# geometrian/simple-spectral

Hardware: AMD Instinct MI355X
Metric: Msamples/s (w*h*spp/s) cornell-srgb 512x512 (higher is better)
Workload: dtype f32

## Files before the change

include/ssx.h:

```cpp
#ifndef SSX_H
#define SSX_H

#include <stddef.h>
#include <stdint.h>

#ifdef __cplusplus
extern "C" {
#endif

#define SSX_ABI_VERSION 2

enum {
	SSX_OK = 0,
	SSX_ERR_DATA = -1,
	SSX_ERR_ARG = -2,
	SSX_ERR_SCENE = -3,
	SSX_ERR_DEVICE = -10,
	SSX_ERR_STATE = -11
};

#define SSX_MAX_DEPTH 10u
#define SSX_TILE_SIZE 8u
#define SSX_SAMPLE_WAVELENGTHS 4u
#define SSX_MAX_TEXTURES 64u
// ... 43 lines not shown
} ssx_meng_grid;

typedef struct ssx_scene_desc {
	uint32_t struct_size;
	uint32_t reserved;
	double pv_inv[16];
	float cam_pos[3];
	float lambda_min;
	float lambda_step;
	uint32_t spec_xbar, spec_ybar, spec_zbar;
	uint32_t spec_basis_r, spec_basis_g, spec_basis_b;
	const ssx_spectrum* spectra;  uint32_t n_spectra;
	const float* samples;         uint32_t n_samples;
	const ssx_material* materials; uint32_t n_materials;
	const ssx_quad* quads;        uint32_t n_quads;
	const uint32_t* lights;       uint32_t n_lights;
	const ssx_texture* textures;  uint32_t n_textures;
	float srgb_to_linear[256];
	uint32_t uplift;
	uint32_t jh_res;
	const float* jh_scale;
	const float* jh_data;
	const ssx_meng_grid* meng;
	float cam_dir[3];
	uint32_t reserved2;
} ssx_scene_desc;

typedef struct ssx_render_params {
	uint32_t struct_size;
	uint32_t width, height;
	uint32_t spp;
	uint32_t indirect_only;
	uint32_t tile_first;
	uint32_t tile_stride;
	uint32_t spp_per_launch;
	uint32_t no_explicit_light_sampling;
	uint32_t no_flat_field_correction;
	uint32_t tile_major;
	uint32_t tile_skew;
	uint64_t seed;
	uint32_t libm;
	uint32_t reserved3;
} ssx_render_params;
enum { SSX_LIBM_BUILD = 0, SSX_LIBM_GLIBC_2_35 = 1 };


typedef struct ssx_ctx ssx_ctx;

int ssx_create(int device, ssx_ctx** out);
void ssx_destroy(ssx_ctx* ctx);

int ssx_upload_scene(ssx_ctx* ctx, const ssx_scene_desc* scene);

int ssx_render_start(ssx_ctx* ctx, const ssx_render_params* params);
int ssx_render_stop(ssx_ctx* ctx);
int ssx_is_rendering(ssx_ctx* ctx);
float ssx_progress(ssx_ctx* ctx);
uint32_t ssx_done_spp(ssx_ctx* ctx);
uint32_t ssx_done_tiles(ssx_ctx* ctx);
int ssx_render_wait(ssx_ctx* ctx, float* xyza_out);

int ssx_render_device(ssx_ctx* ctx, const ssx_render_params* params, void* d_xyza_out, void* hip_stream);
int ssx_render_device_wait(ssx_ctx* ctx);

void* ssx_device_framebuffer(ssx_ctx* ctx);
int ssx_device_index(ssx_ctx* ctx);
int ssx_read_framebuffer(ssx_ctx* ctx, float* xyza_out);
int ssx_accumulate_peer(ssx_ctx* ctx, void* d_dst, int src_device, const void* d_src, uint32_t width, uint32_t height, void* hip_stream);

int ssx_reduce_rccl(ssx_ctx** ctxs, int n, uint32_t width, uint32_t height);
int ssx_rccl_probe(char* report, size_t report_size);
uint64_t ssx_rccl_groups_made(void);

const char* ssx_last_error(const ssx_ctx* ctx);

int ssx_set_timing(ssx_ctx* ctx, int enable);
int ssx_get_timing(ssx_ctx* ctx, float stage_ms[4]);

int ssx_abi_version(void);
int ssx_kernel_info(ssx_ctx* ctx, int* vgprs, int* sgprs, int* lds_bytes, int* scratch_bytes, int* max_blocks_per_cu);
int ssx_plan_info(ssx_ctx* ctx, float* frames_per_sample, int* fold_in_path_kernel);
int ssx_calibration_info(ssx_ctx* ctx, float* frames_per_sample, float* rays_left_per_sample, int* camera_rays_pretraced);
int ssx_scratch_info(ssx_ctx* ctx, uint64_t* sample_bytes, uint64_t* log_bytes);
int ssx_sums_info(ssx_ctx* ctx, uint64_t* units_parked, uint64_t* units_chained);
int ssx_units_info(ssx_ctx* ctx, uint64_t* units_enqueued);
int ssx_kernel_variant(ssx_ctx* ctx);
enum { SSX_JIT_OFF = 0, SSX_JIT_AT_UPLOAD = 1, SSX_JIT_BACKGROUND = 2 };
int ssx_set_jit(ssx_ctx* ctx, int mode);
enum { SSX_JIT_STATE_NONE = 0,
       SSX_JIT_STATE_GENERIC_MEANWHILE = 1,
       SSX_JIT_STATE_SPECIALISED = 2,
       SSX_JIT_STATE_FAILED = -1 };
int ssx_jit_status(ssx_ctx* ctx, int wait_ms, char* message, size_t message_size);
void ssx_jit_counters(uint64_t* compiled, uint64_t* disk_hits);
const char* ssx_kernel_name(ssx_ctx* ctx);


int ssx_render_continue(ssx_ctx* ctx, uint32_t spp_more);

typedef struct ssx_sums_info_t {
	uint32_t struct_size;
	uint32_t width, height;
	uint32_t done_spp;
	uint64_t seed;
	uint32_t indirect_only, no_explicit_light_sampling, no_flat_field_correction, libm;
	uint32_t rgb_mode;
	uint32_t tile_first, tile_stride, tile_skew;
	uint32_t noise_batches;
	uint32_t reserved;
	uint64_t scene_digest;
} ssx_sums_info_t;
uint64_t ssx_scene_digest(ssx_ctx* ctx);
int ssx_sums_export(ssx_ctx* ctx, ssx_sums_info_t* info, double* sums, double* noise_s2);
int ssx_sums_import(ssx_ctx* ctx, const ssx_render_params* params, const ssx_sums_info_t* info, const double* sums, const double* noise_s2);

int ssx_set_noise_estimate(ssx_ctx* ctx, int enable);
int ssx_noise_info(ssx_ctx* ctx, double* v_out, double summary[4]);


int ssx_set_spectral_bins(ssx_ctx* ctx, uint32_t bins);
typedef struct ssx_spectral_info_t {
	uint32_t struct_size;
	uint32_t width, height;
	uint32_t bins;
	uint32_t done_spp;
	uint32_t reserved;
	float lambda_min;
	float bin_width;
} ssx_spectral_info_t;
int ssx_spectral_read(ssx_ctx* ctx, ssx_spectral_info_t* info, float* mean, double* sums, uint32_t* counts);

enum {
	SSX_DBG_FMATH = 1,
	SSX_DBG_SPHTRI = 2,
	SSX_DBG_ARVO = 3,
	SSX_DBG_SAMPLE_LIGHT = 4,
	SSX_DBG_COSHEMI = 5,
	SSX_DBG_TRACE = 6,
	SSX_DBG_RAND_CHOICE = 7,
	SSX_DBG_ALBEDO = 8,
	SSX_DBG_FLUX_TO_XYZ = 9,
	SSX_DBG_RAND_1F = 10,
	SSX_DBG_GLIBC_MATH = 11,
	SSX_DBG_SPHTRI_GLIBC = 12, SSX_DBG_ARVO_GLIBC = 13, SSX_DBG_SAMPLE_LIGHT_GLIBC = 14, SSX_DBG_COSHEMI_GLIBC = 15
};
enum {
	SSX_SWEEP_RCP = 1,
	SSX_SWEEP_SQRT = 2,
	SSX_SWEEP_INVERSESQRT = 3,
	SSX_SWEEP_SIN = 4,
	SSX_SWEEP_COS = 5,
	SSX_SWEEP_ACOS = 6,
	SSX_SWEEP_DIV_PI = 7,
	SSX_SWEEP_RCP64 = 8,
	SSX_SWEEP_DIV_PAIRS = 9,
	SSX_SWEEP_ACOS_SIN = 10,
	SSX_SWEEP_SIN_PROOF = 11, SSX_SWEEP_COS_PROOF = 12, SSX_SWEEP_ACOS_PROOF = 13,
	SSX_SWEEP_GLIBC_SIN = 14, SSX_SWEEP_GLIBC_COS = 15, SSX_SWEEP_GLIBC_ACOS = 16,
	SSX_SWEEP_GLIBC_COS_LDS = 17
};
int ssx_debug_sweep(ssx_ctx* ctx, uint32_t op, uint32_t lo, uint64_t count, uint64_t result[11]);
int ssx_debug_pass1_source(const uint8_t* vid, uint32_t n_quads, const char* name, char* out, size_t out_size);
int ssx_debug_eval(ssx_ctx* ctx, uint32_t op, const void* in, uint32_t in_words, void* out, uint32_t out_words, uint32_t n);
int ssx_debug_samples(ssx_ctx* ctx, const ssx_render_params* params, float* xyza, uint64_t* rng_state, uint32_t* levels);
int ssx_debug_sample_flux(ssx_ctx* ctx, const ssx_render_params* params, float* flux, float* lambda_0);

// ... 5 lines not shown
```

simple_spectral_amd/_capi.py:

```python
import ctypes as C
import os

from . import build as _build


class SsxSpectrum(C.Structure):
    _fields_ = [("offset", C.c_uint32), ("n", C.c_uint32), ("low", C.c_float), ("high", C.c_float),
                ("delta_recip", C.c_float)]


class SsxVertex(C.Structure):
    _fields_ = [("pos", C.c_float * 3), ("st", C.c_float * 2)]


class SsxQuad(C.Structure):
    _fields_ = [("v00", SsxVertex), ("v10", SsxVertex), ("v11", SsxVertex), ("v01", SsxVertex),
                ("normal0", C.c_float * 3), ("normal1", C.c_float * 3),
                ("material", C.c_uint32), ("flags", C.c_uint32)]


class SsxMaterial(C.Structure):
    _fields_ = [("kind", C.c_uint32), ("albedo_mode", C.c_uint32), ("albedo_spectrum", C.c_uint32),
                ("albedo_texture", C.c_uint32), ("emission_spectrum", C.c_uint32)]


class SsxTexture(C.Structure):
    _fields_ = [("width", C.c_uint32), ("height", C.c_uint32), ("rgb", C.POINTER(C.c_uint8))]


class SsxMengGrid(C.Structure):
    _fields_ = [("grid_w", C.c_uint32), ("grid_h", C.c_uint32), ("n_points", C.c_uint32), ("n_samples", C.c_uint32),
                ("sample_min", C.c_float), ("sample_max", C.c_float), ("xy_to_uv", C.c_float * 6),
                ("cells", C.POINTER(C.c_int32)), ("points", C.POINTER(C.c_float))]


class SsxSceneDesc(C.Structure):
    _fields_ = [
        ("struct_size", C.c_uint32), ("reserved", C.c_uint32),
        ("pv_inv", C.c_double * 16), ("cam_pos", C.c_float * 3),
        ("lambda_min", C.c_float), ("lambda_step", C.c_float),
        ("spec_xbar", C.c_uint32), ("spec_ybar", C.c_uint32), ("spec_zbar", C.c_uint32),
        ("spec_basis_r", C.c_uint32), ("spec_basis_g", C.c_uint32), ("spec_basis_b", C.c_uint32),
        ("spectra", C.POINTER(SsxSpectrum)), ("n_spectra", C.c_uint32),
        ("samples", C.POINTER(C.c_float)), ("n_samples", C.c_uint32),
        ("materials", C.POINTER(SsxMaterial)), ("n_materials", C.c_uint32),
        ("quads", C.POINTER(SsxQuad)), ("n_quads", C.c_uint32),
        ("lights", C.POINTER(C.c_uint32)), ("n_lights", C.c_uint32),
        ("textures", C.POINTER(SsxTexture)), ("n_textures", C.c_uint32),
        ("srgb_to_linear", C.c_float * 256),
        ("uplift", C.c_uint32), ("jh_res", C.c_uint32),
        ("jh_scale", C.POINTER(C.c_float)), ("jh_data", C.POINTER(C.c_float)),
        ("meng", C.POINTER(SsxMengGrid)),
        ("cam_dir", C.c_float * 3), ("reserved2", C.c_uint32),
    ]


class SsxRenderParams(C.Structure):
    _fields_ = [("struct_size", C.c_uint32), ("width", C.c_uint32), ("height", C.c_uint32), ("spp", C.c_uint32),
                ("indirect_only", C.c_uint32), ("tile_first", C.c_uint32), ("tile_stride", C.c_uint32),
                ("spp_per_launch", C.c_uint32), ("no_explicit_light_sampling", C.c_uint32), ("no_flat_field_correction", C.c_uint32),
                ("tile_major", C.c_uint32), ("tile_skew", C.c_uint32), ("seed", C.c_uint64), ("libm", C.c_uint32), ("reserved3", C.c_uint32)]


class SsxSumsInfo(C.Structure):
    _fields_ = [("struct_size", C.c_uint32), ("width", C.c_uint32), ("height", C.c_uint32), ("done_spp", C.c_uint32), ("seed", C.c_uint64),
                ("indirect_only", C.c_uint32), ("no_explicit_light_sampling", C.c_uint32), ("no_flat_field_correction", C.c_uint32), ("libm", C.c_uint32),
                ("rgb_mode", C.c_uint32), ("tile_first", C.c_uint32), ("tile_stride", C.c_uint32), ("tile_skew", C.c_uint32),
                ("noise_batches", C.c_uint32), ("reserved", C.c_uint32), ("scene_digest", C.c_uint64)]


class SsxSpectralInfo(C.Structure):
    _fields_ = [("struct_size", C.c_uint32), ("width", C.c_uint32), ("height", C.c_uint32), ("bins", C.c_uint32), ("done_spp", C.c_uint32),
                ("reserved", C.c_uint32), ("lambda_min", C.c_float), ("bin_width", C.c_float)]


SSX_LIBM_BUILD, SSX_LIBM_GLIBC_2_35 = 0, 1
LIBM_MODES = {"build": SSX_LIBM_BUILD, "glibc-2.35": SSX_LIBM_GLIBC_2_35}


SSX_MODE_RGB, SSX_UPLIFT_OURS, SSX_UPLIFT_MENG, SSX_UPLIFT_JH = 0, 1, 2, 3
SSX_PRIM_LIGHT, SSX_PRIM_TRI = 1, 0x100
SSX_OK, SSX_ERR_DATA, SSX_ERR_ARG, SSX_ERR_SCENE, SSX_ERR_DEVICE, SSX_ERR_STATE = 0, -1, -2, -3, -10, -11
SSX_ABI_VERSION = 2
SSX_JIT_OFF, SSX_JIT_AT_UPLOAD, SSX_JIT_BACKGROUND = 0, 1, 2
SSX_JIT_STATE_NONE, SSX_JIT_STATE_GENERIC_MEANWHILE, SSX_JIT_STATE_SPECIALISED, SSX_JIT_STATE_FAILED = 0, 1, 2, -1

HIP_SYMBOLS = ["ssx_create", "ssx_destroy", "ssx_upload_scene", "ssx_render_start", "ssx_render_stop",
               "ssx_is_rendering", "ssx_progress", "ssx_render_wait", "ssx_render_device", "ssx_last_error",
               "ssx_abi_version", "ssx_kernel_info", "ssx_plan_info", "ssx_set_timing", "ssx_get_timing",
               "ssx_device_framebuffer", "ssx_device_index", "ssx_read_framebuffer", "ssx_accumulate_peer",
               "ssx_debug_eval", "ssx_debug_samples", "ssx_debug_sweep", "ssx_kernel_variant", "ssx_kernel_name", "ssx_scratch_info", "ssx_calibration_info", "ssx_set_jit", "ssx_debug_pass1_source", "ssx_done_spp", "ssx_reduce_rccl", "ssx_sums_info", "ssx_rccl_groups_made", "ssx_jit_status", "ssx_jit_counters", "ssx_done_tiles", "ssx_render_device_wait", "ssx_units_info", "ssx_rccl_probe",
               "ssx_render_continue", "ssx_scene_digest", "ssx_sums_export", "ssx_sums_import", "ssx_set_noise_estimate", "ssx_noise_info",
               "ssx_set_spectral_bins", "ssx_spectral_read", "ssx_debug_sample_flux"]
(SSX_SWEEP_RCP, SSX_SWEEP_SQRT, SSX_SWEEP_INVERSESQRT, SSX_SWEEP_SIN, SSX_SWEEP_COS, SSX_SWEEP_ACOS, SSX_SWEEP_DIV_PI,
 SSX_SWEEP_RCP64, SSX_SWEEP_DIV_PAIRS, SSX_SWEEP_ACOS_SIN, SSX_SWEEP_SIN_PROOF, SSX_SWEEP_COS_PROOF, SSX_SWEEP_ACOS_PROOF) = range(1, 14)
(SSX_DBG_FMATH, SSX_DBG_SPHTRI, SSX_DBG_ARVO, SSX_DBG_SAMPLE_LIGHT, SSX_DBG_COSHEMI, SSX_DBG_TRACE, SSX_DBG_RAND_CHOICE,
 SSX_DBG_ALBEDO, SSX_DBG_FLUX_TO_XYZ, SSX_DBG_RAND_1F) = range(1, 11)
(SSX_DBG_GLIBC_MATH, SSX_DBG_SPHTRI_GLIBC, SSX_DBG_ARVO_GLIBC, SSX_DBG_SAMPLE_LIGHT_GLIBC, SSX_DBG_COSHEMI_GLIBC) = range(11, 16)
(SSX_SWEEP_GLIBC_SIN, SSX_SWEEP_GLIBC_COS, SSX_SWEEP_GLIBC_ACOS, SSX_SWEEP_GLIBC_COS_LDS) = range(14, 18)
HOST_SYMBOLS = ["ssh_scene_create", "ssh_scene_create_ex", "ssh_scene_destroy", "ssh_scene_desc", "ssh_xyza_to_srgba", "ssh_save_image",
                "ssh_load_png_rgb8", "ssh_free", "ssh_color_values", "ssh_last_error", "ssh_checkpoint_save", "ssh_checkpoint_load", "ssh_sums_merge", "ssh_save_npy_f32"]

_hip = None
_host = None


def host_lib():
    global _host
    if _host is None:
        path = _build.HOST_LIB
        if not os.path.exists(path):
            _build.build_host()
        lib = C.CDLL(path)
        vp = C.c_void_p
        lib.ssh_last_error.restype = C.c_char_p
        lib.ssh_scene_create.argtypes = [C.c_char_p, C.c_char_p, C.c_int, vp, C.c_uint32, C.c_uint32, C.c_char_p,
                                         C.c_float, C.POINTER(vp)]
        lib.ssh_scene_create_ex.argtypes = [C.c_char_p, C.c_char_p, C.c_int, vp, C.c_uint32, C.c_uint32, C.c_char_p,
                                            C.c_float, C.c_uint32, C.c_char_p, C.c_uint32, C.POINTER(vp)]
        lib.ssh_scene_destroy.argtypes = [vp]
        lib.ssh_scene_desc.restype = C.POINTER(SsxSceneDesc)
        lib.ssh_scene_desc.argtypes = [vp]
        lib.ssh_xyza_to_srgba.argtypes = [vp, vp, vp, C.c_size_t]
        lib.ssh_save_image.argtypes = [C.c_char_p, vp, C.c_uint32, C.c_uint32]
        lib.ssh_load_png_rgb8.argtypes = [C.c_char_p, C.POINTER(C.POINTER(C.c_uint8)), C.POINTER(C.c_uint32),
                                          C.POINTER(C.c_uint32)]
        lib.ssh_free.argtypes = [vp]
        lib.ssh_color_values.argtypes = [vp, C.c_char_p, C.POINTER(C.c_float), C.c_int]
        lib.ssh_checkpoint_save.argtypes = [C.c_char_p, C.POINTER(SsxSumsInfo), C.c_char_p, C.c_char_p, vp, vp]
        lib.ssh_checkpoint_load.argtypes = [C.c_char_p, C.POINTER(SsxSumsInfo), C.c_char_p, C.c_size_t, C.c_char_p, C.c_size_t,
                                            C.POINTER(C.POINTER(C.c_double)), C.POINTER(C.POINTER(C.c_double))]
        lib.ssh_sums_merge.argtypes = [vp, vp, vp, vp, C.POINTER(SsxSumsInfo)]
        lib.ssh_save_npy_f32.argtypes = [C.c_char_p, vp, C.POINTER(C.c_uint32), C.c_uint32]
        _host = lib
    return _host


def mapped_hip_runtimes():
    out = set()
    try:
        for ln in open("/proc/self/maps"):
            f = ln.split(None, 5)
            if len(f) == 6 and "libamdhip64.so" in os.path.basename(f[5].strip()):
                out.add(os.path.realpath(f[5].strip()))
    except OSError:
        pass
    return sorted(out)


def _elf_dynamic(path):
    import struct
    try:
        with open(path, "rb") as f:
            eh = f.read(64)
            if eh[:6] != b"\x7fELF\x02\x01":
                return None, []
            shoff, = struct.unpack_from("<Q", eh, 0x28)
            shentsize, shnum = struct.unpack_from("<HH", eh, 0x3A)
            f.seek(shoff)
            sh = [struct.unpack_from("<IIQQQQIIQQ", f.read(shentsize)) for _ in range(shnum)]
            dyn = next((x for x in sh if x[1] == 6), None)
            if dyn is None:
                return None, []
            strtab = sh[dyn[6]]
            f.seek(strtab[4]); names = f.read(strtab[5])
            f.seek(dyn[4]); raw = f.read(dyn[5])
        soname, needed = None, []
        for k in range(0, len(raw) - 15, 16):
            tag, val = struct.unpack_from("<qQ", raw, k)
            if tag in (1, 14):
                name = names[val:names.index(b"\0", val)].decode()
                if tag == 14:
                    soname = name
                else:
                    needed.append(name)
        return soname, needed
    except Exception:
        return None, []


def _one_hip_runtime_before_load(path):
    if mapped_hip_runtimes():
        return
    try:
        import importlib.util
        wanted = [n for n in _elf_dynamic(path)[1] if n.startswith("libamdhip64.so")]
        spec = importlib.util.find_spec("torch")
        if wanted and spec and spec.submodule_search_locations:
            cand = os.path.join(list(spec.submodule_search_locations)[0], "lib", "libamdhip64.so")
            if os.path.exists(cand) and _elf_dynamic(cand)[0] == wanted[0]:
                C.CDLL(cand, mode=C.RTLD_GLOBAL)
    except Exception:
        pass


def _one_hip_runtime_after_load(path):
    rts = mapped_hip_runtimes()
    if len(rts) > 1:
        raise RuntimeError("two HIP runtimes are mapped into this process (%s) after loading %s: streams and device pointers cannot be "
                           "handed between them.  Import simple_spectral_amd (or torch) before whatever loaded the other one, or "
                           "point LD_LIBRARY_PATH at one of them." % (", ".join(rts), path))


def hip_lib():
    global _hip
    if _hip is None:
        path = (os.environ.get("SSX_HIP_LIB_OVERRIDE") if os.environ.get("SSX_DEBUG_ENV") == "1" else None) or _build.HIP_LIB
        if not os.path.exists(path):
            raise RuntimeError("%s is missing: run `python -m simple_spectral_amd.build` (needs hipcc). "
                               "simple_spectral_amd has no CPU or PyTorch fallback path." % path)
        _one_hip_runtime_before_load(path)
        lib = C.CDLL(path)
        _one_hip_runtime_after_load(path)
        override = path != _build.HIP_LIB
        if not override and lib.ssx_abi_version() != SSX_ABI_VERSION:
            raise RuntimeError("%s implements ABI version %d, this binding version %d (include/ssx.h): rebuild with `python -m simple_spectral_amd.build`"
                               % (path, lib.ssx_abi_version(), SSX_ABI_VERSION))
        vp = C.c_void_p
        lib.ssx_last_error.restype = C.c_char_p
        lib.ssx_last_error.argtypes = [vp]
        lib.ssx_create.argtypes = [C.c_int, C.POINTER(vp)]
        lib.ssx_destroy.argtypes = [vp]
        lib.ssx_destroy.restype = None
        lib.ssx_upload_scene.argtypes = [vp, C.POINTER(SsxSceneDesc)]
        lib.ssx_render_start.argtypes = [vp, C.POINTER(SsxRenderParams)]
        lib.ssx_render_stop.argtypes = [vp]
        lib.ssx_is_rendering.argtypes = [vp]
        lib.ssx_progress.argtypes = [vp]
        lib.ssx_progress.restype = C.c_float
        lib.ssx_render_wait.argtypes = [vp, vp]
        lib.ssx_render_device.argtypes = [vp, C.POINTER(SsxRenderParams), vp, vp]
        lib.ssx_kernel_info.argtypes = [vp] + [C.POINTER(C.c_int)] * 5
        lib.ssx_plan_info.argtypes = [vp, C.POINTER(C.c_float), C.POINTER(C.c_int)]
        lib.ssx_set_timing.argtypes = [vp, C.c_int]
        lib.ssx_get_timing.argtypes = [vp, C.POINTER(C.c_float)]
        lib.ssx_device_framebuffer.argtypes = [vp]
        lib.ssx_device_framebuffer.restype = vp
        lib.ssx_device_index.argtypes = [vp]
        lib.ssx_read_framebuffer.argtypes = [vp, vp]
        lib.ssx_accumulate_peer.argtypes = [vp, vp, C.c_int, vp, C.c_uint32, C.c_uint32, vp]
        lib.ssx_debug_eval.argtypes = [vp, C.c_uint32, vp, C.c_uint32, vp, C.c_uint32, C.c_uint32]
        lib.ssx_debug_samples.argtypes = [vp, C.POINTER(SsxRenderParams), vp, vp, vp]
        lib.ssx_debug_sweep.argtypes = [vp, C.c_uint32, C.c_uint32, C.c_uint64, C.POINTER(C.c_uint64)]
        if not override or hasattr(lib, "ssx_scratch_info"):
            lib.ssx_calibration_info.argtypes = [vp, C.POINTER(C.c_float), C.POINTER(C.c_float), C.POINTER(C.c_int)]
            lib.ssx_scratch_info.argtypes = [vp, C.POINTER(C.c_uint64), C.POINTER(C.c_uint64)]
        if not override or hasattr(lib, "ssx_set_jit"):
            lib.ssx_set_jit.argtypes = [vp, C.c_int]
            lib.ssx_done_spp.argtypes = [vp]
            lib.ssx_done_spp.restype = C.c_uint32
            lib.ssx_reduce_rccl.argtypes = [C.POINTER(vp), C.c_int, C.c_uint32, C.c_uint32]
            lib.ssx_debug_pass1_source.argtypes = [C.POINTER(C.c_uint8), C.c_uint32, C.c_char_p, C.c_char_p, C.c_size_t]
        if not override or hasattr(lib, "ssx_sums_info"):
            lib.ssx_sums_info.argtypes = [vp, C.POINTER(C.c_uint64), C.POINTER(C.c_uint64)]
        if hasattr(lib, "ssx_rccl_probe"):
            lib.ssx_rccl_probe.argtypes = [C.c_char_p, C.c_size_t]
        if hasattr(lib, "ssx_units_info"):
            lib.ssx_units_info.argtypes = [vp, C.POINTER(C.c_uint64)]
        if not override or hasattr(lib, "ssx_jit_status"):
            lib.ssx_jit_status.argtypes = [vp, C.c_int, C.c_char_p, C.c_size_t]
            lib.ssx_jit_counters.argtypes = [C.POINTER(C.c_uint64), C.POINTER(C.c_uint64)]
            lib.ssx_jit_counters.restype = None
            lib.ssx_rccl_groups_made.restype = C.c_uint64
            lib.ssx_render_device_wait.argtypes = [vp]
            lib.ssx_done_tiles.argtypes = [vp]
            lib.ssx_done_tiles.restype = C.c_uint32
        if not override or hasattr(lib, "ssx_render_continue"):
            lib.ssx_render_continue.argtypes = [vp, C.c_uint32]
            lib.ssx_scene_digest.argtypes = [vp]
            lib.ssx_scene_digest.restype = C.c_uint64
            lib.ssx_sums_export.argtypes = [vp, C.POINTER(SsxSumsInfo), vp, vp]
            lib.ssx_sums_import.argtypes = [vp, C.POINTER(SsxRenderParams), C.POINTER(SsxSumsInfo), vp, vp]
            lib.ssx_set_noise_estimate.argtypes = [vp, C.c_int]
            lib.ssx_noise_info.argtypes = [vp, vp, C.POINTER(C.c_double)]
        if not override or hasattr(lib, "ssx_set_spectral_bins"):
            lib.ssx_set_spectral_bins.argtypes = [vp, C.c_uint32]
            lib.ssx_spectral_read.argtypes = [vp, C.POINTER(SsxSpectralInfo), vp, vp, vp]
            lib.ssx_debug_sample_flux.argtypes = [vp, C.POINTER(SsxRenderParams), vp, vp]
        lib.ssx_kernel_variant.argtypes = [vp]
        lib.ssx_kernel_name.argtypes = [vp]
        lib.ssx_kernel_name.restype = C.c_char_p
        _hip = lib
    return _hip
```

simple_spectral_amd/csrc/ssx_api.hip:

```cpp
#include "ssx_kernels.hip"
#include "ssx_debug.hip"

#include "../../include/ssx.h"

#include <chrono>
#include <array>
#include <atomic>
#include <cstdarg>
#include <cstdio>
#include <cstdlib>
#include <cmath>
#include <algorithm>
#include <cstring>
#include <mutex>
#include <string>
#include <thread>
#include <vector>

#include <limits.h>
#include <set>

#include "ssx_jit.h"

namespace {

thread_local std::string g_create_error;

const char* debug_env(const char* name) {
	const char* m = getenv("SSX_DEBUG_ENV");
	if (!m || m[0] != '1' || m[1] != '\0') return nullptr;
	return getenv(name);
}
bool env_on(const char* name) { const char* e = debug_env(name); return e && e[0] != '\0' && e[0] != '0'; }

std::string fmt(const char* f, ...) {
	char buf[512];
	va_list ap; va_start(ap, f); vsnprintf(buf, sizeof buf, f, ap); va_end(ap);
	return buf;
}

struct DeviceBuffer {
	void* ptr = nullptr;
	size_t bytes = 0;
	DeviceBuffer() = default;
	DeviceBuffer(DeviceBuffer&& o) noexcept : ptr(o.ptr), bytes(o.bytes) { o.ptr = nullptr; o.bytes = 0; }
	DeviceBuffer& operator=(DeviceBuffer&& o) noexcept { std::swap(ptr, o.ptr); std::swap(bytes, o.bytes); return *this; }
	~DeviceBuffer() { release(); }
	void release() { if (ptr) (void)hipFree(ptr); ptr = nullptr; bytes = 0; }
	hipError_t reserve(size_t n) {
		if (n <= bytes) return hipSuccess;
		release();
		const hipError_t e = hipMalloc(&ptr, n);
		if (e == hipSuccess) bytes = n; else ptr = nullptr;
		return e;
	}
	template <class T> T* as() const { return static_cast<T*>(ptr); }
};

}

#include "ssx_pack.h"

struct ssx_ctx {
	int device = 0;
	int n_cus = 0;
	hipStream_t stream = nullptr;
	DeviceBuffer d_blob;
	uint32_t blob_words = 0;
	uint32_t path_blob_words = 0;
	uint32_t topology = 0;
	int jit_mode = SSX_JIT_BACKGROUND;
	const ssx_jit::Kernels* jit_kernels[ssx_jit::kVariants] = {};
	uint32_t libm = SSX_LIBM_BUILD;
	uint32_t variant = SSX_LIBM_BUILD;
	bool jit_pending = false, jit_requested = false;
	ssx_jit::VidTable jit_vid;
	DeviceBuffer d_blob_jit; uint32_t blob_jit_words = 0, path_blob_jit_words = 0;
	uint64_t generic_samples = 0;
	int jit_state = SSX_JIT_STATE_NONE; std::string jit_message;
	std::vector<DeviceBuffer> d_textures;
	DeviceBuffer d_jh_data;
	bool rgb_mode = false;
	bool fuse_resolve = true;
	float calib_frames = 0.0f;
	float calib_left = 0.0f;
	bool pre_hits = false;
	DeviceBuffer d_accum;
	DeviceBuffer d_unit_counter;
	int resident_blocks = 0;
	int gen_blocks = 0;
	uint32_t max_wave_slots = 0;
	uint32_t queue_words = SSX_QUEUE_WORDS_WIDE;
	DeviceBuffer d_samples;
	DeviceBuffer d_logs;
	DeviceBuffer d_out;
	DeviceBuffer d_peer;
	bool have_scene = false;
	bool have_cam_dir = false;

	std::thread worker;
	std::atomic<int> rendering{0};
	std::atomic<int> stop_flag{0};
	std::atomic<uint32_t> done_spp{0};
	std::atomic<uint32_t> done_tiles{0};
	uint32_t total_spp = 0;
	int worker_rc = 0;
	std::atomic<uint64_t> units_enqueued{0};
	ssx_render_params cur{};
	struct SumsState { bool continuable = false, noise_valid = false, spectral_valid = false; uint32_t noise_batches = 0; } sums;
	uint32_t k_begin = 0;
	uint64_t scene_digest = 0;
	bool noise_on = false;
	DeviceBuffer d_noise;
	DeviceBuffer d_stage;
	uint32_t spectral_bins = 0;
	DeviceBuffer d_spectral_sums, d_spectral_counts;
	std::string spectral_note;
	float lambda_min = 0.0f, lambda_step = 0.0f;

	bool timing = false;
	std::vector<hipEvent_t> ev_pool;
	size_t ev_used = 0;
	float stage_ms[4] = { 0, 0, 0, 0 };

	hipEvent_t ev_device_done = nullptr;
	bool device_pending = false;

	void* rccl_comm = nullptr; uint64_t rccl_group = 0; int rccl_rank = -1, rccl_size = 0;

	std::mutex error_mutex;
	std::string error;
	std::string error_out;
};

namespace {

void set_error(ssx_ctx* ctx, const std::string& msg) { std::lock_guard<std::mutex> g(ctx->error_mutex); ctx->error = msg; }

#define SSX_HIP(ctx, call)                                                                          \
	do {                                                                                            \
		hipError_t e_ = (call);                                                                     \
		if (e_ != hipSuccess) {                                                                     \
			set_error((ctx), fmt("%s failed: %s", #call, hipGetErrorString(e_)));                   \
			return SSX_ERR_DEVICE;                                                                  \
		}                                                                                           \
	} while (0)

int fail(ssx_ctx* ctx, int code, const std::string& msg) { set_error(ctx, msg); return code; }

int check_params(ssx_ctx* ctx, const ssx_render_params* p) {
	if (!p || p->struct_size != sizeof(ssx_render_params)) return fail(ctx, SSX_ERR_ARG, "ssx_render_params.struct_size mismatch");
	if (p->libm != SSX_LIBM_BUILD && p->libm != SSX_LIBM_GLIBC_2_35) return fail(ctx, SSX_ERR_ARG, "ssx_render_params.libm: unknown value");
	if (!ctx->have_scene) return fail(ctx, SSX_ERR_STATE, "no scene uploaded");
	if (p->width == 0 || p->height == 0 || p->spp == 0) return fail(ctx, SSX_ERR_ARG, "width, height and spp must be positive");
	if ((uint64_t)p->width * p->height > (1ull << 28)) return fail(ctx, SSX_ERR_ARG, "image too large");
	if (p->tile_stride == 0 || p->tile_first >= p->tile_stride) return fail(ctx, SSX_ERR_ARG, "need tile_first < tile_stride");
	if (p->no_flat_field_correction && !ctx->have_cam_dir) return fail(ctx, SSX_ERR_ARG, "no_flat_field_correction needs ssx_scene_desc.cam_dir (caller built against an older ssx.h)");
	return SSX_OK;
}

int take_params(ssx_ctx* ctx, const ssx_render_params* in, ssx_render_params* out) {
	if (!in) return fail(ctx, SSX_ERR_ARG, "ssx_render_params is NULL");
	memset(out, 0, sizeof *out);
	if (in->struct_size == offsetof(ssx_render_params, libm)) { memcpy(out, in, offsetof(ssx_render_params, libm)); out->struct_size = sizeof *out; }
	else memcpy(out, in, in->struct_size == sizeof *out ? sizeof *out : sizeof out->struct_size);
	return check_params(ctx, out);
}
int begin_render(ssx_ctx* ctx, const ssx_render_params* in, ssx_render_params* out, const char* busy) {
	const int rc = take_params(ctx, in, out);
	if (rc) return rc;
	return ctx->rendering.load() ? fail(ctx, SSX_ERR_STATE, busy) : SSX_OK;
}

int wait_device_pending(ssx_ctx* ctx) {
	if (ctx->device_pending) { SSX_HIP(ctx, hipEventSynchronize(ctx->ev_device_done)); ctx->device_pending = false; }
	return SSX_OK;
}

uint32_t tiles_across(uint32_t pixels) { return (pixels + 7u) / 8u; }
size_t accum_bytes(uint32_t width, uint32_t height) { return (size_t)tiles_across(width) * tiles_across(height) * 64u * 4 * sizeof(double); }
size_t image_bytes(uint32_t width, uint32_t height) { return (size_t)width * height * 4 * sizeof(float); }

SsxPixelGrid pixel_grid(const ssx_render_params* p) {
	const uint32_t tx = tiles_across(p->width);
	return SsxPixelGrid{ p->width, p->height, tx, p->tile_first, p->tile_stride, p->tile_skew % tx };
}
dim3 pixel_blocks(const ssx_render_params* p) { return dim3((p->width * p->height + 255u) / 256u); }

int clear_sums(ssx_ctx* ctx, uint32_t width, uint32_t height, hipStream_t stream) {
	SSX_HIP(ctx, hipMemsetAsync(ctx->d_accum.ptr, 0, accum_bytes(width, height), stream));
	return SSX_OK;
}
void sums_invalidate(ssx_ctx* ctx) { ctx->sums = ssx_ctx::SumsState{}; }
void sums_publish(ssx_ctx* ctx, uint32_t done_spp, int64_t noise_batches = -1) {
	if (noise_batches >= 0) { ctx->sums.noise_valid = true; ctx->sums.noise_batches = (uint32_t)noise_batches; }
	ctx->done_spp.store(done_spp); ctx->sums.continuable = true;
}

constexpr size_t kSampleBufferBudget = (size_t)16 << 30;
size_t bytes_per_sample(const ssx_ctx* ctx) { return ctx->spectral_bins ? SSX_BYTES_PER_SAMPLE_FLUX : SSX_BYTES_PER_SAMPLE; }
constexpr size_t kAuxWordsPer64Records = 5;
size_t bytes_per_64_records(const ssx_ctx* ctx) { return 64u * bytes_per_sample(ctx) + kAuxWordsPer64Records * sizeof(uint32_t); }
size_t sample_bytes(const ssx_ctx* ctx, size_t records) { return records / 64u * bytes_per_64_records(ctx); }
size_t sample_slots(const ssx_ctx* ctx) { return ctx->d_samples.bytes / bytes_per_64_records(ctx) * 64u; }
size_t log_records(const ssx_ctx* ctx) { return ctx->d_logs.bytes / SSX_LOG_BYTES_PER_RECORD; }
constexpr uint32_t kMinUnits = 3072;
constexpr uint64_t kSamplesPerSync = (uint64_t)32 << 20;

struct LaunchPlan { SsxKernelArgs args; uint32_t max_spp_per_launch; };

LaunchPlan make_plan(ssx_ctx* ctx, const ssx_render_params* p, bool ask_device = true) {
	LaunchPlan pl{};
	SsxKernelArgs& a = pl.args;
	a.blob = ctx->d_blob.as<uint32_t>(); a.blob_words = ctx->path_blob_words;
	a.width = p->width; a.height = p->height;
	a.inv_width = 1.0 / (double)p->width; a.inv_height = 1.0 / (double)p->height;
	a.tiles_x = tiles_across(p->width);
	a.n_tiles = a.tiles_x * tiles_across(p->height);
	a.tile_first = p->tile_first; a.tile_stride = p->tile_stride; a.tile_skew = p->tile_skew % a.tiles_x;
	a.indirect_only = p->indirect_only ? 1u : 0u;
	a.no_els = p->no_explicit_light_sampling ? 1u : 0u;
	a.no_flat_field = p->no_flat_field_correction ? 1u : 0u;
	a.seed = p->seed;
	a.rgb_mode = ctx->rgb_mode ? 1u : 0u;
	a.fuse_resolve = ctx->fuse_resolve ? 1u : 0u;
	a.pre_hits = ctx->pre_hits ? 1u : 0u;
	a.my_tiles = a.n_tiles > p->tile_first ? (a.n_tiles - p->tile_first + p->tile_stride - 1u) / p->tile_stride : 0u;
	size_t per_spp = (size_t)(a.my_tiles ? a.my_tiles : 1u) * 64u * bytes_per_sample(ctx);
	size_t budget = kSampleBufferBudget, free_b = 0, total_b = 0;
	if (ask_device && hipMemGetInfo(&free_b, &total_b) == hipSuccess) {
		const size_t avail = (size_t)((double)(free_b + sample_slots(ctx) * bytes_per_sample(ctx)) * 0.8);
		if (avail < budget) budget = avail;
	}
	size_t cap = budget / per_spp;
	const size_t idx_cap = (size_t)0xFFFFFFFFu / ((size_t)(a.my_tiles ? a.my_tiles : 1u) * 64u);
	if (cap > idx_cap) cap = idx_cap;
	pl.max_spp_per_launch = (uint32_t)(cap < 1 ? 1 : (cap > 65536 ? 65536 : cap));
	return pl;
}

void cap_to_allocation(const ssx_ctx* ctx, LaunchPlan& pl) {
	const size_t per_spp = (size_t)(pl.args.my_tiles ? pl.args.my_tiles : 1u) * 64u;
	const size_t fit = sample_slots(ctx) / per_spp;
	if (fit >= 1 && fit < pl.max_spp_per_launch) pl.max_spp_per_launch = (uint32_t)fit;
}

int ensure_samples(ssx_ctx* ctx, const LaunchPlan& pl, uint32_t n_k) {
	const size_t need = (size_t)pl.args.my_tiles * 64u * n_k;
	const hipError_t e = ctx->d_samples.reserve(sample_bytes(ctx, need));
	if (e == hipErrorOutOfMemory) { (void)hipGetLastError(); return fail(ctx, SSX_ERR_DEVICE, fmt("out of device memory for %zu samples in flight; lower spp_per_launch", need)); }
	SSX_HIP(ctx, e);
	return SSX_OK;
}

int ensure_logs(ssx_ctx* ctx, uint32_t unit_cohorts) {
	const size_t need = (size_t)ctx->max_wave_slots * 2u * unit_cohorts * SSX_COHORT_RECORDS, bytes = need * SSX_LOG_BYTES_PER_RECORD;
	if (bytes >= ((size_t)1 << 32)) return fail(ctx, SSX_ERR_DEVICE, "level logs beyond 4 GiB: the kernels address them with 32-bit offsets");
	if (ctx->d_logs.bytes >= bytes) return SSX_OK;
	if (ctx->d_logs.ptr) {
		const int rc = wait_device_pending(ctx);
		if (rc) return rc;
		SSX_HIP(ctx, hipStreamSynchronize(ctx->stream));
	}
	const hipError_t e = ctx->d_logs.reserve(bytes);
	if (e == hipErrorOutOfMemory) { (void)hipGetLastError(); return fail(ctx, SSX_ERR_DEVICE, fmt("out of device memory for the level logs (%zu bytes)", bytes)); }
	SSX_HIP(ctx, e);
	return SSX_OK;
}

void bind_arrays(SsxKernelArgs& a, uint8_t* base, uint64_t cap, uint8_t* logs, uint64_t log_cap, bool with_flux) {
	a.ray = reinterpret_cast<float4*>(base);                      base += cap * 16u;
	a.st = reinterpret_cast<uint4*>(base);                        base += cap * 16u;
	a.hit = reinterpret_cast<float4*>(base);                      base += cap * 16u;
	a.flux = with_flux ? reinterpret_cast<float4*>(base) : nullptr;
	a.logs = logs; a.log_cap = (uint32_t)log_cap;
}

int collect_timing(ssx_ctx* ctx) {
	for (size_t b = 0; b + 6 <= ctx->ev_used; b += 6) {
		hipEvent_t* e = &ctx->ev_pool[b];
		SSX_HIP(ctx, hipEventSynchronize(e[2]));
		SSX_HIP(ctx, hipEventSynchronize(e[5]));
		const int pairs[4][2] = { { 0, 1 }, { 1, 2 }, { 3, 4 }, { 4, 5 } };
		for (int k = 0; k < 4; ++k) {
			float ms = 0;
			SSX_HIP(ctx, hipEventElapsedTime(&ms, e[pairs[k][0]], e[pairs[k][1]]));
			ctx->stage_ms[k] += ms;
		}
	}
	ctx->ev_used = 0;
	return SSX_OK;
}

int timing_events(ssx_ctx* ctx, hipEvent_t** out) {
	if (ctx->ev_used + 6 > 6 * 64) { int r = collect_timing(ctx); if (r) return r; }
	while (ctx->ev_pool.size() < ctx->ev_used + 6) {
		hipEvent_t e;
		SSX_HIP(ctx, hipEventCreateWithFlags(&e, hipEventDisableSystemFence));
		ctx->ev_pool.push_back(e);
	}
	*out = &ctx->ev_pool[ctx->ev_used];
	ctx->ev_used += 6;
	return SSX_OK;
}

struct Batch { SsxKernelArgs a; uint32_t units; uint64_t n_rec; hipEvent_t* tev; int rc; };

uint32_t unit_spp_of(const ssx_ctx* ctx) { return ctx->calib_frames >= 2.0f ? SSX_MAX_UNIT_KS / 2u : SSX_MAX_UNIT_KS; }

Batch make_batch(ssx_ctx* ctx, const LaunchPlan& pl, uint32_t k0, uint32_t k1) {
	Batch b{};
	b.a = pl.args;
	SsxKernelArgs& a = b.a;
	const uint32_t n_k = k1 - k0;
	a.k0 = k0; a.k1 = k1;
	a.n_records = (uint64_t)a.my_tiles * n_k * 64u;
	uint32_t g = unit_spp_of(ctx);
	while (g > 1u && (uint64_t)((n_k + g - 1u) / g) * a.my_tiles < kMinUnits) g >>= 1;
	a.group_spp = g;
	if (a.group_spp > n_k) a.group_spp = n_k;
	a.unit_cohorts = (a.group_spp + SSX_COHORT_KS - 1u) / SSX_COHORT_KS;
	a.unit_grab = ctx->calib_frames >= 2.0f ? 1u : 4u;
	if (a.unit_grab < 1u || a.unit_grab > 32u || a.group_spp == 0u || a.unit_cohorts == 0u) {
		b.rc = fail(ctx, SSX_ERR_STATE, fmt("internal: launch with unit_grab = %u (1..32), group_spp = %u, unit_cohorts = %u", a.unit_grab, a.group_spp, a.unit_cohorts));
		return b;
	}
	a.n_groups = (n_k + a.group_spp - 1) / a.group_spp;
	b.units = a.my_tiles * a.n_groups;
	b.n_rec = a.n_records;
	b.rc = ensure_logs(ctx, a.unit_cohorts);
	if (b.rc == SSX_OK) bind_arrays(a, ctx->d_samples.as<uint8_t>(), a.n_records, ctx->d_logs.as<uint8_t>(), log_records(ctx), ctx->spectral_bins != 0u);
	a.accum = ctx->d_accum.as<double>();
	uint32_t* const aux = reinterpret_cast<uint32_t*>(ctx->d_samples.as<uint8_t>() + sample_slots(ctx) * bytes_per_sample(ctx));
	a.unit_state = aux;
	a.tile_mask = aux + b.units;
	if (b.rc == SSX_OK && (size_t)a.my_tiles * 4u + b.units > (sample_slots(ctx) / 64u) * kAuxWordsPer64Records) b.rc = fail(ctx, SSX_ERR_STATE, "internal: launch larger than the sample allocation");
	return b;
}

size_t path_lds_bytes(uint32_t blob_words, uint32_t queue_words) {
	size_t n = ((size_t)blob_words + SSX_LDS_PREFIX_WORDS) * 4 + 4u * ((size_t)SSX_QUEUE_ENTRIES * queue_words + SSX_WAVE_COUNTER_WORDS) * 4u;
#ifdef SSX_REGTIME
	n += 4u * SSX_NTIME * 8u;
#endif
	return n;
}
struct PathKernel { const char* name; void (*host)(SsxKernelArgs); };
#define SSX_PK(k) { #k, k }
static const PathKernel kPathKernels[ssx_jit::kVariants][3][2] = {
	{ { SSX_PK(ssx_render_kernel), SSX_PK(ssx_render_kernel_nq) }, { SSX_PK(ssx_render_kernel_cornell), SSX_PK(ssx_render_kernel_cornell_nq) },
	  { SSX_PK(ssx_render_kernel_plane), SSX_PK(ssx_render_kernel_plane_nq) } },
	{ { SSX_PK(ssx_render_kernel_glibc), SSX_PK(ssx_render_kernel_nq_glibc) }, { SSX_PK(ssx_render_kernel_cornell_glibc), SSX_PK(ssx_render_kernel_cornell_nq_glibc) },
	  { SSX_PK(ssx_render_kernel_plane_glibc), SSX_PK(ssx_render_kernel_plane_nq_glibc) } },
	{ { SSX_PK(ssx_render_kernel_flux), SSX_PK(ssx_render_kernel_nq_flux) }, { SSX_PK(ssx_render_kernel_cornell_flux), SSX_PK(ssx_render_kernel_cornell_nq_flux) },
	  { SSX_PK(ssx_render_kernel_plane_flux), SSX_PK(ssx_render_kernel_plane_nq_flux) } } };
#undef SSX_PK
static const char* const kJitKernelNames[2] = { "ssx_render_kernel_jit", "ssx_render_kernel_jit_nq" };
const PathKernel& path_kernel_of(const ssx_ctx* ctx, bool narrow) { return kPathKernels[ctx->variant][ctx->topology < 3u ? ctx->topology : 0u][narrow]; }
struct KernelRef { const void* host = nullptr; hipFunction_t mod = nullptr; };
KernelRef path_kernel_ref(const ssx_ctx* ctx, bool narrow) {
	KernelRef k;
	const ssx_jit::Kernels* jk = ctx->jit_kernels[ctx->variant];
	if (ctx->topology == 3u && jk) k.mod = narrow ? jk->path_nq : jk->path;
	else k.host = (const void*)path_kernel_of(ctx, narrow).host;
	return k;
}
int occupancy_of(ssx_ctx* ctx, const KernelRef& k, size_t lds, int* per_cu) {
	if (k.mod) SSX_HIP(ctx, hipModuleOccupancyMaxActiveBlocksPerMultiprocessor(per_cu, k.mod, 256, lds));
	else SSX_HIP(ctx, hipOccupancyMaxActiveBlocksPerMultiprocessor(per_cu, k.host, 256, lds));
	return SSX_OK;
}
int blocks_that_fit(ssx_ctx* ctx, const KernelRef& k, size_t lds, int* blocks) {
	int per_cu = 0;
	const int rc = occupancy_of(ctx, k, lds, &per_cu);
	if (rc) return rc;
	*blocks = (per_cu > 0 ? per_cu : 1) * ctx->n_cus;
	return SSX_OK;
}
int launch_kernel(ssx_ctx* ctx, const KernelRef& k, uint32_t blocks, size_t lds, hipStream_t stream, SsxKernelArgs& a) {
	if (k.mod) {
		size_t size = sizeof a;
		void* config[] = { HIP_LAUNCH_PARAM_BUFFER_POINTER, &a, HIP_LAUNCH_PARAM_BUFFER_SIZE, &size, HIP_LAUNCH_PARAM_END };
		SSX_HIP(ctx, hipModuleLaunchKernel(k.mod, blocks, 1, 1, 256, 1, 1, (unsigned)lds, stream, nullptr, config));
	} else {
		void* args[] = { &a };
		SSX_HIP(ctx, hipLaunchKernel(k.host, dim3(blocks), dim3(256), args, lds, stream));
	}
	return SSX_OK;
}
int pick_queue(ssx_ctx* ctx, uint32_t blob_words, uint32_t* queue_words, int* blocks_per_cu) {
	int wide = 0, narrow = 0, rc;
	if (path_lds_bytes(blob_words, SSX_QUEUE_WORDS_WIDE) <= 65536u)
		if ((rc = occupancy_of(ctx, path_kernel_ref(ctx, false), path_lds_bytes(blob_words, SSX_QUEUE_WORDS_WIDE), &wide))) return rc;
	if ((rc = occupancy_of(ctx, path_kernel_ref(ctx, true), path_lds_bytes(blob_words, SSX_QUEUE_WORDS_NARROW), &narrow))) return rc;
	const bool use_narrow = narrow > wide || env_on("SSX_NARROW_QUEUE");
	*queue_words = use_narrow ? SSX_QUEUE_WORDS_NARROW : SSX_QUEUE_WORDS_WIDE;
	if (blocks_per_cu) *blocks_per_cu = use_narrow ? narrow : wide;
	return SSX_OK;
}

bool fuses_generate(const ssx_ctx* ctx, const SsxKernelArgs& a) {
	const char* fuse_env = debug_env("SSX_FUSE_GEN");
	const bool tiles_fit = a.tiles_x <= 0xFFFFu && tiles_across(a.height) <= 0xFFFFu;
	return ctx->topology == 2u && !a.pre_hits && tiles_fit && !(fuse_env && fuse_env[0] == '0');
}

int enqueue_generate(ssx_ctx* ctx, const Batch& b, hipStream_t stream) {
	SsxKernelArgs ga = b.a;
	ga.blob_words = ctx->blob_words;
	if (ga.pre_hits) {
		hipLaunchKernelGGL(ssx_tile_mask_kernel, dim3((ga.my_tiles + 3u) / 4u), dim3(256), 0, stream, ga);
		SSX_HIP(ctx, hipGetLastError());
	}
	const KernelRef gen_kernel{ (const void*)ssx_generate_kernel };
	const size_t gen_lds = ((size_t)ga.blob_words + SSX_LDS_PREFIX_WORDS) * 4;
	if (ctx->gen_blocks == 0) { const int rc = blocks_that_fit(ctx, gen_kernel, gen_lds, &ctx->gen_blocks); if (rc) return rc; }
	const uint64_t want = (b.n_rec + 255u) / 256u;
	return launch_kernel(ctx, gen_kernel, (uint32_t)(want < (uint64_t)ctx->gen_blocks ? want : (uint64_t)ctx->gen_blocks), gen_lds, stream, ga);
}

int enqueue_path(ssx_ctx* ctx, Batch& b, const KernelRef& kernel, uint32_t queue_words, uint32_t blob_words, int resident_blocks, hipStream_t stream) {
	if (!ctx->d_unit_counter.ptr) {
		SSX_HIP(ctx, ctx->d_unit_counter.reserve(4 * sizeof(uint32_t)));
		SSX_HIP(ctx, hipMemsetAsync(ctx->d_unit_counter.ptr, 0, 4 * sizeof(uint32_t), stream));
	}
	b.a.blob_words = blob_words; b.a.queue_words = queue_words;
	SSX_HIP(ctx, hipMemsetAsync(ctx->d_unit_counter.ptr, 0, 2 * sizeof(uint32_t), stream));
	SSX_HIP(ctx, hipMemsetAsync(b.a.unit_state, 0, (size_t)b.units * sizeof(uint32_t), stream));
	b.a.unit_counter = ctx->d_unit_counter.as<uint32_t>();
	const uint32_t want_blocks = (b.units + 3u) / 4u;
	uint32_t blocks = want_blocks < (uint32_t)resident_blocks ? want_blocks : (uint32_t)resident_blocks;
	if (blocks * 4u > ctx->max_wave_slots) blocks = ctx->max_wave_slots / 4u;
	return launch_kernel(ctx, kernel, blocks, path_lds_bytes(blob_words, queue_words), stream, b.a);
}

int launch_batch(ssx_ctx* ctx, Batch& b, hipStream_t stream) {
	if (b.rc) return b.rc;
	int rc;
	if (ctx->timing) { if ((rc = timing_events(ctx, &b.tev))) return rc; SSX_HIP(ctx, hipEventRecord(b.tev[0], stream)); }
	b.a.fuse_gen = fuses_generate(ctx, b.a) ? 1u : 0u;
	if (!b.a.fuse_gen && (rc = enqueue_generate(ctx, b, stream))) return rc;
	if (ctx->timing) SSX_HIP(ctx, hipEventRecord(b.tev[1], stream));
	const bool plan = ctx->resident_blocks == 0;
	if (plan && (rc = pick_queue(ctx, b.a.blob_words, &ctx->queue_words, nullptr))) return rc;
	const KernelRef path_kernel = path_kernel_ref(ctx, ctx->queue_words == SSX_QUEUE_WORDS_NARROW);
	if (plan && (rc = blocks_that_fit(ctx, path_kernel, path_lds_bytes(b.a.blob_words, ctx->queue_words), &ctx->resident_blocks))) return rc;
	if ((rc = enqueue_path(ctx, b, path_kernel, ctx->queue_words, b.a.blob_words, ctx->resident_blocks, stream))) return rc;
	ctx->units_enqueued.fetch_add(b.units);
	if (ctx->timing) for (int k = 2; k < 6; ++k) SSX_HIP(ctx, hipEventRecord(b.tev[k], stream));
	return SSX_OK;
}

constexpr uint64_t kJitAfterSamples = kSamplesPerSync;
void maybe_swap_jit(ssx_ctx* ctx, uint64_t samples) {
	if (!ctx->jit_pending) return;
	std::string err;
	const ssx_jit::Kernels* k = nullptr;
	const ssx_jit::State st = ssx_jit::lookup(ctx->device, ctx->jit_vid, &k, &err, ctx->variant);
	if (st == ssx_jit::State::Ready) {
		std::swap(ctx->d_blob, ctx->d_blob_jit);
		ctx->blob_words = ctx->blob_jit_words; ctx->path_blob_words = ctx->path_blob_jit_words;
		ctx->topology = 3u;
		ctx->jit_kernels[ctx->variant] = k;
		ctx->resident_blocks = 0; ctx->gen_blocks = 0;
		ctx->jit_pending = false; ctx->jit_state = SSX_JIT_STATE_SPECIALISED;
	} else if (st == ssx_jit::State::Failed) {
		ctx->jit_pending = false; ctx->jit_state = SSX_JIT_STATE_FAILED; ctx->jit_message = err;
	} else {
		ctx->generic_samples += samples;
		if (!ctx->jit_requested && ctx->generic_samples >= kJitAfterSamples) { ssx_jit::request(ctx->jit_vid, ctx->variant); ctx->jit_requested = true; }
	}
}

int ensure_libm_kernels(ssx_ctx* ctx, uint32_t libm) {
	const ssx_jit::Kernels*& have = ctx->jit_kernels[libm];
	if (ctx->topology != 3u || have) return SSX_OK;
	std::string err;
	const ssx_jit::Kernels* k = ssx_jit::get(ctx->device, ctx->jit_vid, &err, libm);
	if (!k) return fail(ctx, SSX_ERR_STATE, "the scene's specialised kernels for this libm could not be compiled: " + err);
	have = k;
	return SSX_OK;
}

int ready_to_launch(ssx_ctx* ctx, const ssx_render_params* p, bool need_out) {
	const uint32_t variant = (ctx->spectral_bins && p->libm == SSX_LIBM_BUILD && !ctx->rgb_mode) ? ssx_jit::kVariantFlux : p->libm;
	const int rc = ensure_libm_kernels(ctx, variant);
	if (rc) return rc;
	ctx->libm = p->libm;
	if (ctx->variant != variant) { ctx->variant = variant; ctx->resident_blocks = 0; ctx->jit_requested = false; }
	SSX_HIP(ctx, ctx->d_accum.reserve(accum_bytes(p->width, p->height)));
	if (need_out) SSX_HIP(ctx, ctx->d_out.reserve(image_bytes(p->width, p->height)));
	return SSX_OK;
}

int launch_range(ssx_ctx* ctx, LaunchPlan& pl, uint32_t k0, uint32_t k1, hipStream_t stream) {
	if (pl.args.my_tiles == 0 || k1 <= k0) return SSX_OK;
	Batch b = make_batch(ctx, pl, k0, k1);
	return launch_batch(ctx, b, stream);
}

int launch_batches(ssx_ctx* ctx, LaunchPlan& pl, uint32_t spp, uint32_t batch, hipStream_t stream) {
	for (uint32_t k0 = 0; k0 < spp; k0 += batch) {
		int rc = launch_range(ctx, pl, k0, (spp - k0 < batch) ? spp : k0 + batch, stream);
		if (rc) return rc;
	}
	return SSX_OK;
}

int calibrate(ssx_ctx* ctx) {
	ssx_render_params cp{};
	cp.struct_size = sizeof cp; cp.width = 64; cp.height = 64; cp.spp = 4; cp.tile_stride = 1;
	ctx->fuse_resolve = false;
	ctx->pre_hits = false;
	LaunchPlan pl = make_plan(ctx, &cp);
	int rc = ensure_samples(ctx, pl, cp.spp);
	if (rc) return rc;
	Batch b = make_batch(ctx, pl, 0, cp.spp);
	if (b.rc) return b.rc;
	if ((rc = enqueue_generate(ctx, b, ctx->stream))) return rc;
	const KernelRef kernel{ (const void*)ssx_calibrate_kernel };
	int blocks = 0;
	if ((rc = blocks_that_fit(ctx, kernel, path_lds_bytes(ctx->blob_words, SSX_QUEUE_WORDS_NARROW), &blocks))) return rc;
	if ((rc = enqueue_path(ctx, b, kernel, SSX_QUEUE_WORDS_NARROW, ctx->blob_words, blocks, ctx->stream))) return rc;
	SSX_HIP(ctx, hipStreamSynchronize(ctx->stream));
	std::vector<uint4> recs((size_t)b.n_rec);
	SSX_HIP(ctx, hipMemcpy(recs.data(), b.a.st, recs.size() * sizeof(uint4), hipMemcpyDeviceToHost));
	uint64_t frames = 0;
	for (const uint4& r : recs) frames += (r.y >> 2) & 0xFu;
	ctx->calib_frames = (float)((double)frames / (double)recs.size());
	uint32_t counters[2] = { 0u, 0u };
	SSX_HIP(ctx, hipMemcpy(counters, ctx->d_unit_counter.ptr, sizeof counters, hipMemcpyDeviceToHost));
	ctx->calib_left = (float)((double)counters[1] / (double)recs.size());
	ctx->pre_hits = ctx->calib_left >= 0.3f;
	if (const char* e = debug_env("SSX_PRE_HITS")) { if (e[0] != '\0') ctx->pre_hits = e[0] != '0'; }
	ctx->fuse_resolve = true;
	return ensure_logs(ctx, (unit_spp_of(ctx) + SSX_COHORT_KS - 1u) / SSX_COHORT_KS);
}

int launch_finalize(ssx_ctx* ctx, const ssx_render_params* p, uint32_t spp, float* d_out, hipStream_t stream, uint32_t done_tiles = 0xFFFFFFFFu) {
	hipLaunchKernelGGL(ssx_finalize_kernel, pixel_blocks(p), dim3(256), 0, stream,
	                   ctx->d_accum.as<const double>(), (float4*)d_out, pixel_grid(p), spp, ctx->rgb_mode ? 1u : 0u, done_tiles);
	SSX_HIP(ctx, hipGetLastError());
	return SSX_OK;
}

int noise_begin(ssx_ctx* ctx, const ssx_render_params* p, uint32_t k_begin, bool continuing);
int noise_batch(ssx_ctx* ctx, const ssx_render_params* p, uint32_t n_k, hipStream_t stream);
int spectral_refuses(ssx_ctx* ctx, const ssx_render_params& p, bool tile_walk);
int spectral_begin(ssx_ctx* ctx, uint32_t my_tiles, bool continuing, bool* active);
int spectral_batch(ssx_ctx* ctx, const ssx_render_params* p, const LaunchPlan& pl, uint32_t n_k, hipStream_t stream);

int finish_walk(ssx_ctx* ctx, const ssx_render_params& p, uint32_t spp, uint32_t done_tiles) {
	if (const int rc = launch_finalize(ctx, &p, spp, ctx->d_out.as<float>(), ctx->stream, done_tiles)) return rc;
	SSX_HIP(ctx, hipStreamSynchronize(ctx->stream));
	return SSX_OK;
}

uint32_t sample_walk_chunk(const ssx_render_params& p, uint32_t span, const LaunchPlan& pl) {
	const size_t pixels = (size_t)p.width * p.height;
	const uint64_t min_spp = kSamplesPerSync / (pixels ? pixels : 1) + 1u;
	uint32_t chunk = p.spp_per_launch ? p.spp_per_launch : (span + 31u) / 32u;
	if (!p.spp_per_launch && chunk < min_spp) chunk = (uint32_t)(min_spp < span ? min_spp : span);
	if (chunk == 0) chunk = 1;
	return chunk > pl.max_spp_per_launch ? pl.max_spp_per_launch : chunk;
}

struct TileLaunch { uint32_t tiles, spp; };
TileLaunch tile_walk_launch(const ssx_render_params& p, const LaunchPlan& pl) {
// ... 204 lines not shown
	if (!ctx) return;
	if (ctx->worker.joinable()) { ctx->stop_flag.store(1); ctx->worker.join(); }
	(void)hipSetDevice(ctx->device);
	if (ctx->rccl_comm) { std::lock_guard<std::mutex> g(rccl_api().mutex); drop_rccl_comm(ctx); }
	if (ctx->ev_device_done) (void)hipEventDestroy(ctx->ev_device_done);
	for (hipEvent_t e : ctx->ev_pool) (void)hipEventDestroy(e);
	const hipStream_t stream = ctx->stream;
	delete ctx;
	if (stream) (void)hipStreamDestroy(stream);
}

int ssx_upload_scene(ssx_ctx* ctx, const ssx_scene_desc* s) {
	if (!ctx) return SSX_ERR_ARG;
	ssx_scene_desc local;
	bool have_cam_dir = true;
	if (s && (s->struct_size == offsetof(ssx_scene_desc, meng) || s->struct_size == offsetof(ssx_scene_desc, cam_dir))) {
		memset(&local, 0, sizeof local);
		memcpy(&local, s, s->struct_size);
		local.struct_size = sizeof(ssx_scene_desc);
		have_cam_dir = false;
		s = &local;
	}
	if (!s || s->struct_size != sizeof(ssx_scene_desc)) return fail(ctx, SSX_ERR_ARG, "ssx_scene_desc.struct_size mismatch");
	if (ctx->rendering.load()) return fail(ctx, SSX_ERR_STATE, "render in progress");
	SSX_HIP(ctx, hipSetDevice(ctx->device));
	SSX_HIP(ctx, hipDeviceSynchronize());
	ctx->device_pending = false;
	ctx->d_textures.clear();
	ctx->have_scene = false;
	sums_invalidate(ctx); ctx->scene_digest = 0;
	for (uint32_t i = 0; i < s->n_textures && i < SSX_MAX_TEXTURES; ++i) {
		const ssx_texture& t = s->textures[i];
		if (!t.rgb || t.width == 0 || t.height == 0) return fail(ctx, SSX_ERR_DATA, "Could not load texture");
		const size_t bytes = (size_t)3 * t.width * t.height;
		ctx->d_textures.emplace_back();
		SSX_HIP(ctx, ctx->d_textures.back().reserve(bytes));
		SSX_HIP(ctx, hipMemcpy(ctx->d_textures.back().ptr, t.rgb, bytes, hipMemcpyHostToDevice));
	}
	if (s->uplift != SSX_MODE_RGB && s->uplift != SSX_UPLIFT_OURS && s->uplift != SSX_UPLIFT_JH && s->uplift != SSX_UPLIFT_MENG)
		return fail(ctx, SSX_ERR_SCENE, "unsupported uplift variant (0 = RGB mode, 1 = basis, 2 = Meng et al., 3 = Jakob-Hanika)");
	ctx->rgb_mode = (s->uplift == SSX_MODE_RGB);
	ctx->d_jh_data.release();
	if (s->uplift == SSX_UPLIFT_MENG) {
		const ssx_meng_grid* g = s->meng;
		if (!g || !g->cells || !g->points || g->grid_w == 0 || g->grid_h == 0 || g->grid_w > 4096 || g->grid_h > 4096 ||
		    g->n_points == 0 || g->n_points > (1u << 20) || g->n_samples < 2 || g->n_samples > 4096 || !(g->sample_max > g->sample_min))
			return fail(ctx, SSX_ERR_DATA, "Meng grid missing or invalid");
		const size_t n_cells = (size_t)g->grid_w * g->grid_h;
		for (size_t c = 0; c < n_cells; ++c) {
			const int32_t* cell = g->cells + 8 * c;
			const int32_t inside = cell[0], num = cell[1];
			const bool shape_ok = inside ? (num == 4) : (num == 0 || (num >= 3 && num <= 6));
			if (!shape_ok) return fail(ctx, SSX_ERR_DATA, "Meng grid: cell with an unusable point count");
			for (int32_t k = 0; k < num; ++k) if (cell[2 + k] < 0 || (uint32_t)cell[2 + k] >= g->n_points) return fail(ctx, SSX_ERR_DATA, "Meng grid: point index out of range");
		}
		const size_t words = 16 + n_cells * 8 + (size_t)g->n_points * (4 + (size_t)g->n_samples);
		std::vector<uint32_t> tab(words, 0u);
		tab[0] = g->grid_w; tab[1] = g->grid_h; tab[2] = g->n_points; tab[3] = g->n_samples;
		memcpy(&tab[4], &g->sample_min, 4); memcpy(&tab[5], &g->sample_max, 4);
		memcpy(&tab[6], g->xy_to_uv, 24);
		memcpy(&tab[16], g->cells, n_cells * 32);
		memcpy(&tab[16 + n_cells * 8], g->points, (size_t)g->n_points * (4 + (size_t)g->n_samples) * 4);
		SSX_HIP(ctx, ctx->d_jh_data.reserve(words * 4));
		SSX_HIP(ctx, hipMemcpy(ctx->d_jh_data.ptr, tab.data(), words * 4, hipMemcpyHostToDevice));
	}
	if (s->uplift == SSX_UPLIFT_JH) {
		if (!s->jh_scale || !s->jh_data || s->jh_res < 2 || s->jh_res > 256) return fail(ctx, SSX_ERR_DATA, "Jakob-Hanika model missing or invalid");
		size_t bytes = (size_t)3 * s->jh_res * s->jh_res * s->jh_res * 3 * sizeof(float);
		SSX_HIP(ctx, ctx->d_jh_data.reserve(bytes));
		SSX_HIP(ctx, hipMemcpy(ctx->d_jh_data.ptr, s->jh_data, bytes, hipMemcpyHostToDevice));
	}
	std::vector<uint32_t> blob, blob_jit;
	for (auto& k : ctx->jit_kernels) k = nullptr;
	ctx->jit_pending = ctx->jit_requested = false; ctx->generic_samples = 0; ctx->jit_vid.clear();
	ctx->jit_state = SSX_JIT_STATE_NONE; ctx->jit_message.clear();
	ctx->d_blob_jit.release();
	std::vector<const void*> tex;
	for (const DeviceBuffer& t : ctx->d_textures) tex.push_back(t.ptr);
	PackInfo info;
	std::string pack_err;
	int rc = pack_blob(s, tex, ctx->d_jh_data.ptr, blob, pack_err, -1, &info);
	if (rc) return fail(ctx, rc, pack_err);
	const int jit_mode = env_on("SSX_JIT_PASS1") ? SSX_JIT_AT_UPLOAD : ctx->jit_mode;
	if (info.candidate && jit_mode != SSX_JIT_OFF) {
		std::string err;
		const ssx_jit::Kernels* k = nullptr;
		ssx_jit::State st = ssx_jit::lookup(ctx->device, info.vid, &k, &err);
		if (st != ssx_jit::State::Ready && st != ssx_jit::State::Failed && jit_mode == SSX_JIT_AT_UPLOAD) {
			k = ssx_jit::get(ctx->device, info.vid, &err);
			st = k ? ssx_jit::State::Ready : ssx_jit::State::Failed;
		}
		if (st == ssx_jit::State::Failed) { ctx->jit_state = SSX_JIT_STATE_FAILED; ctx->jit_message = err; }
		else if ((rc = pack_blob(s, tex, ctx->d_jh_data.ptr, blob_jit, pack_err, 3))) return fail(ctx, rc, pack_err);
		else if (st == ssx_jit::State::Ready) { blob.swap(blob_jit); blob_jit.clear(); ctx->jit_kernels[SSX_LIBM_BUILD] = k; ctx->jit_vid = info.vid; ctx->jit_state = SSX_JIT_STATE_SPECIALISED; }
		else { ctx->jit_pending = true; ctx->jit_vid = info.vid; ctx->jit_state = SSX_JIT_STATE_GENERIC_MEANWHILE; ctx->jit_requested = (st == ssx_jit::State::Pending); }
	}
	if (ctx->jit_pending) {
		SSX_HIP(ctx, ctx->d_blob_jit.reserve(blob_jit.size() * 4));
		SSX_HIP(ctx, hipMemcpy(ctx->d_blob_jit.ptr, blob_jit.data(), blob_jit.size() * 4, hipMemcpyHostToDevice));
		const SsxBlobHeader* bh = reinterpret_cast<const SsxBlobHeader*>(blob_jit.data());
		ctx->blob_jit_words = (uint32_t)blob_jit.size(); ctx->path_blob_jit_words = bh->words_without_perm;
	}
	SSX_HIP(ctx, ctx->d_blob.reserve(blob.size() * 4));
	SSX_HIP(ctx, hipMemcpy(ctx->d_blob.ptr, blob.data(), blob.size() * 4, hipMemcpyHostToDevice));
	ctx->blob_words = (uint32_t)blob.size();
	{
		SsxBlobHeader* bh = reinterpret_cast<SsxBlobHeader*>(blob.data());
		ctx->topology = bh->topology;
		ctx->path_blob_words = (bh->topology || bh->perm_hbm) ? bh->words_without_perm : ctx->blob_words;
		if (bh->perm_hbm) {
			const uint64_t at = (uint64_t)(uintptr_t)(ctx->d_blob.as<uint32_t>() + bh->off_perm);
			bh->perm_ptr_lo = (uint32_t)at; bh->perm_ptr_hi = (uint32_t)(at >> 32);
			SSX_HIP(ctx, hipMemcpy(ctx->d_blob.ptr, blob.data(), sizeof(SsxBlobHeader), hipMemcpyHostToDevice));
			ctx->blob_words = bh->words_without_perm;
		}
	}
	ctx->have_cam_dir = have_cam_dir;
	ctx->lambda_min = s->lambda_min; ctx->lambda_step = s->lambda_step;
	ctx->resident_blocks = 0; ctx->gen_blocks = 0;
	ctx->have_scene = true;
	ctx->scene_digest = scene_digest_of(s);
	return calibrate(ctx);
}

static uint32_t device_batch(const ssx_render_params* p, const LaunchPlan& pl) {
	uint32_t batch = p->spp_per_launch ? p->spp_per_launch : p->spp;
	if (batch > p->spp) batch = p->spp;
	if (batch > pl.max_spp_per_launch) {
		const uint32_t n = (p->spp + pl.max_spp_per_launch - 1u) / pl.max_spp_per_launch;
		batch = (p->spp + n - 1u) / n;
	}
	return batch;
}

int ssx_render_device(ssx_ctx* ctx, const ssx_render_params* p_in, void* d_xyza_out, void* hip_stream) {
	if (!ctx) return SSX_ERR_ARG;
	ssx_render_params pp;
	int rc = take_params(ctx, p_in, &pp);
	if (rc) return rc;
	const ssx_render_params* const p = &pp;
	if (!d_xyza_out) return fail(ctx, SSX_ERR_ARG, "d_xyza_out is NULL");
	if (ctx->spectral_bins) return fail(ctx, SSX_ERR_ARG, "spectral output is on (ssx_set_spectral_bins): ssx_render_device does not bin its samples; use ssx_render_start");
	if (ctx->rendering.load()) return fail(ctx, SSX_ERR_STATE, "asynchronous render in progress");
	hipStream_t stream = (hipStream_t)hip_stream;
	SSX_HIP(ctx, hipSetDevice(ctx->device));
	if (!ctx->ev_device_done) SSX_HIP(ctx, hipEventCreateWithFlags(&ctx->ev_device_done, hipEventDisableTiming));
	hipStreamCaptureStatus capture = hipStreamCaptureStatusNone;
	(void)hipStreamIsCapturing(stream, &capture);
	const bool capturing = capture == hipStreamCaptureStatusActive;
	if (ctx->device_pending && capturing) return fail(ctx, SSX_ERR_STATE, "a render of this context may still be queued: ssx_render_device_wait before capturing another into a graph");
	if (capturing && ctx->variant != p->libm) return fail(ctx, SSX_ERR_STATE, "ssx_render_params.libm differs from the context's last render: run it once outside the stream capture first");
	if (ctx->device_pending) SSX_HIP(ctx, hipStreamWaitEvent(stream, ctx->ev_device_done, 0));
	{
		LaunchPlan probe = make_plan(ctx, p, !capturing);
		if (capturing) cap_to_allocation(ctx, probe);
		const uint32_t probe_batch = device_batch(p, probe);
		const size_t need = (size_t)probe.args.my_tiles * 64u * probe_batch;
		const bool grow = ctx->d_accum.bytes < accum_bytes(p->width, p->height) || ctx->d_samples.bytes < sample_bytes(ctx, need);
		if (grow && capturing) return fail(ctx, SSX_ERR_STATE, "the context's buffers have to grow for this render: run it once outside the stream capture first");
		if (grow && (rc = wait_device_pending(ctx))) return rc;
	}
	if ((rc = ready_to_launch(ctx, p, false))) return rc;
	sums_invalidate(ctx);
	if ((rc = clear_sums(ctx, p->width, p->height, stream))) return rc;
	if (!capturing) maybe_swap_jit(ctx, (uint64_t)p->width * p->height * p->spp / p->tile_stride);
	LaunchPlan pl = make_plan(ctx, p, !capturing);
	if (capturing) cap_to_allocation(ctx, pl);
	const uint32_t batch = device_batch(p, pl);
	if ((rc = ensure_samples(ctx, pl, batch))) return rc;
	if ((rc = launch_batches(ctx, pl, p->spp, batch, stream))) return rc;
	if ((rc = launch_finalize(ctx, p, p->spp, (float*)d_xyza_out, stream))) return rc;
	if (!capturing) {
		SSX_HIP(ctx, hipEventRecord(ctx->ev_device_done, stream));
		ctx->device_pending = true;
	}
	return SSX_OK;
}

int ssx_render_device_wait(ssx_ctx* ctx) {
	if (!ctx) return SSX_ERR_ARG;
	if (!ctx->device_pending) return SSX_OK;
	SSX_HIP(ctx, hipSetDevice(ctx->device));
	return wait_device_pending(ctx);
}

int ssx_render_start(ssx_ctx* ctx, const ssx_render_params* p_in) {
	if (!ctx) return SSX_ERR_ARG;
	ssx_render_params pp;
	int rc = begin_render(ctx, p_in, &pp, "render already in progress");
	if (rc) return rc;
	SSX_HIP(ctx, hipSetDevice(ctx->device));
	if ((rc = wait_device_pending(ctx))) return rc;
	return start_worker(ctx, pp, 0, false, pp.spp);
}

int ssx_render_stop(ssx_ctx* ctx) {
	if (!ctx) return SSX_ERR_ARG;
	ctx->stop_flag.store(1);
	return SSX_OK;
}

int ssx_is_rendering(ssx_ctx* ctx) { return ctx ? ctx->rendering.load() : 0; }

float ssx_progress(ssx_ctx* ctx) {
	if (!ctx || ctx->total_spp == 0) return 0.0f;
	const uint32_t done = ctx->done_spp.load();
	return done > ctx->k_begin ? (float)(done - ctx->k_begin) / (float)ctx->total_spp : 0.0f;
}

uint32_t ssx_done_spp(ssx_ctx* ctx) { return ctx ? ctx->done_spp.load() : 0u; }

uint32_t ssx_done_tiles(ssx_ctx* ctx) { return ctx ? ctx->done_tiles.load() : 0u; }

int ssx_render_wait(ssx_ctx* ctx, float* xyza_out) {
	if (!ctx) return SSX_ERR_ARG;
	if (!ctx->worker.joinable()) return fail(ctx, SSX_ERR_STATE, "no render was started");
	ctx->worker.join();
	if (ctx->worker_rc) return ctx->worker_rc;
	if (xyza_out) {
		SSX_HIP(ctx, hipSetDevice(ctx->device));
		SSX_HIP(ctx, hipMemcpy(xyza_out, ctx->d_out.ptr, image_bytes(ctx->cur.width, ctx->cur.height), hipMemcpyDeviceToHost));
	}
	return SSX_OK;
}

int ssx_set_timing(ssx_ctx* ctx, int enable) {
	if (!ctx) return SSX_ERR_ARG;
	ctx->timing = enable != 0;
	for (float& m : ctx->stage_ms) m = 0;
	ctx->ev_used = 0;
	return SSX_OK;
}

int ssx_get_timing(ssx_ctx* ctx, float stage_ms[4]) {
	if (!ctx || !stage_ms) return SSX_ERR_ARG;
	SSX_HIP(ctx, hipSetDevice(ctx->device));
	int rc = collect_timing(ctx);
	if (rc) return rc;
	for (int k = 0; k < 4; ++k) { stage_ms[k] = ctx->stage_ms[k]; ctx->stage_ms[k] = 0; }
	return SSX_OK;
}
// ... 92 lines not shown
	std::vector<float4> ray((size_t)b.n_rec);
	std::vector<uint4> st((size_t)b.n_rec);
	SSX_HIP(ctx, hipMemcpy(ray.data(), b.a.ray, ray.size() * sizeof(float4), hipMemcpyDeviceToHost));
	SSX_HIP(ctx, hipMemcpy(st.data(), b.a.st, st.size() * sizeof(uint4), hipMemcpyDeviceToHost));
	const uint32_t spp = p->spp, tiles_x = tiles_across(p->width);
	for (uint32_t j = 0; j < p->height; ++j) for (uint32_t i = 0; i < p->width; ++i) {
		const uint32_t tile = (j >> 3) * tiles_x + (i >> 3), lane = (j & 7u) * 8u + (i & 7u);
		for (uint32_t k = 0; k < spp; ++k) {
			const size_t r = ((size_t)tile * spp + k) * 64u + lane, o = ((size_t)j * p->width + i) * spp + k;
			if (xyza) { xyza[4 * o + 0] = ray[r].x; xyza[4 * o + 1] = ray[r].y; xyza[4 * o + 2] = ray[r].z; xyza[4 * o + 3] = ray[r].w; }
			if (rng_state) rng_state[o] = ((uint64_t)st[r].w << 32) | st[r].z;
			if (levels) levels[o] = (st[r].y >> 2) & 0xFu;
		}
	}
	return SSX_OK;
}

#ifdef SSX_LANESTAT
int ssx_lanestat(unsigned long long* out, int reset) {
	if (reset) { unsigned long long z[2 * SSX_NSTAT] = {}; return (int)hipMemcpyToSymbol(HIP_SYMBOL(g_lanestat), z, sizeof z); }
	(void)hipDeviceSynchronize();
	return (int)hipMemcpyFromSymbol(out, HIP_SYMBOL(g_lanestat), 2 * SSX_NSTAT * sizeof(unsigned long long));
}
#endif
#ifdef SSX_REGTIME
int ssx_regtime(unsigned long long* out, int reset) {
	if (reset) { unsigned long long z[SSX_NTIME] = {}; return (int)hipMemcpyToSymbol(HIP_SYMBOL(g_regtime), z, sizeof z); }
	(void)hipDeviceSynchronize();
	return (int)hipMemcpyFromSymbol(out, HIP_SYMBOL(g_regtime), SSX_NTIME * sizeof(unsigned long long));
}
#endif

int ssx_set_jit(ssx_ctx* ctx, int mode) {
	if (!ctx || mode < SSX_JIT_OFF || mode > SSX_JIT_BACKGROUND) return SSX_ERR_ARG;
	ctx->jit_mode = mode;
	return SSX_OK;
}

int ssx_jit_status(ssx_ctx* ctx, int wait_ms, char* message, size_t message_size) {
	if (!ctx) return SSX_ERR_ARG;
	if (ctx->rendering.load()) return fail(ctx, SSX_ERR_STATE, "render in progress");
	if (ctx->jit_pending && wait_ms != 0) {
		if (hipSetDevice(ctx->device) != hipSuccess) return fail(ctx, SSX_ERR_DEVICE, "hipSetDevice failed");
		if (!ctx->jit_requested) { ssx_jit::request(ctx->jit_vid, ctx->variant); ctx->jit_requested = true; }
		(void)ssx_jit::wait(ctx->jit_vid, wait_ms < 0 ? 600000 : wait_ms, ctx->variant);
		maybe_swap_jit(ctx, 0);
	}
	copy_text(ctx->jit_message, message, message_size);
	return ctx->jit_state;
}

void ssx_jit_counters(uint64_t* compiled, uint64_t* disk_hits) {
	ssx_jit::Shared& S = ssx_jit::shared();
	std::lock_guard<std::mutex> g(S.m);
	if (compiled) *compiled = S.compiled;
	if (disk_hits) *disk_hits = S.disk_hits;
}

int ssx_debug_pass1_source(const uint8_t* vid, uint32_t n_quads, const char* name, char* out, size_t out_size) {
	if (!vid || !name || n_quads == 0 || n_quads > 32u) return SSX_ERR_ARG;
	ssx_jit::VidTable t(n_quads);
	for (uint32_t q = 0; q < n_quads; ++q) for (int v = 0; v < 4; ++v) t[q][v] = vid[4 * q + v];
	const std::string text = ssx_jit::pass1_source(name, t);
	copy_text(text, out, out_size);
	return (int)text.size();
}

int ssx_calibration_info(ssx_ctx* ctx, float* frames_per_sample, float* rays_left_per_sample, int* camera_rays_pretraced) {
	if (!ctx) return SSX_ERR_ARG;
	if (!ctx->have_scene) return fail(ctx, SSX_ERR_STATE, "no scene uploaded");
	if (frames_per_sample) *frames_per_sample = ctx->calib_frames;
	if (rays_left_per_sample) *rays_left_per_sample = ctx->calib_left;
	if (camera_rays_pretraced) *camera_rays_pretraced = ctx->pre_hits ? 1 : 0;
	return SSX_OK;
}

int ssx_scratch_info(ssx_ctx* ctx, uint64_t* sample_bytes, uint64_t* log_bytes) {
	if (!ctx) return SSX_ERR_ARG;
	if (sample_bytes) *sample_bytes = (uint64_t)sample_slots(ctx) * bytes_per_sample(ctx);
	if (log_bytes) *log_bytes = (uint64_t)ctx->d_logs.bytes;
	return SSX_OK;
}

int ssx_sums_info(ssx_ctx* ctx, uint64_t* units_parked, uint64_t* units_chained) {
	if (!ctx) return SSX_ERR_ARG;
	uint32_t c[4] = { 0u, 0u, 0u, 0u };
	if (ctx->d_unit_counter.ptr) {
		SSX_HIP(ctx, hipSetDevice(ctx->device));
		const int rc = wait_device_pending(ctx);
		if (rc) return rc;
		SSX_HIP(ctx, hipMemcpy(c, ctx->d_unit_counter.ptr, sizeof c, hipMemcpyDeviceToHost));
	}
	if (units_parked) *units_parked = c[2];
	if (units_chained) *units_chained = c[3];
	return SSX_OK;
}

int ssx_units_info(ssx_ctx* ctx, uint64_t* units_enqueued) {
	if (!ctx) return SSX_ERR_ARG;
	if (units_enqueued) *units_enqueued = ctx->units_enqueued.load();
	return SSX_OK;
}

int ssx_kernel_variant(ssx_ctx* ctx) { return (ctx && ctx->have_scene) ? (int)ctx->topology : -1; }

const char* ssx_kernel_name(ssx_ctx* ctx) {
	if (!ctx || !ctx->have_scene) return nullptr;
	if (hipSetDevice(ctx->device) != hipSuccess) return nullptr;
	uint32_t qw = 0;
	if (pick_queue(ctx, ctx->path_blob_words, &qw, nullptr) != SSX_OK) return nullptr;
	const bool narrow = qw == SSX_QUEUE_WORDS_NARROW;
	return ctx->topology == 3u ? kJitKernelNames[narrow] : path_kernel_of(ctx, narrow).name;
}

int ssx_plan_info(ssx_ctx* ctx, float* frames_per_sample, int* fold_in_path_kernel) {
	if (!ctx) return SSX_ERR_ARG;
	if (!ctx->have_scene) return fail(ctx, SSX_ERR_STATE, "no scene uploaded");
	if (frames_per_sample) *frames_per_sample = ctx->calib_frames;
	if (fold_in_path_kernel) *fold_in_path_kernel = ctx->fuse_resolve ? 1 : 0;
	return SSX_OK;
}

int ssx_kernel_info(ssx_ctx* ctx, int* vgprs, int* sgprs, int* lds_bytes, int* scratch_bytes, int* max_blocks_per_cu) {
	if (!ctx) return SSX_ERR_ARG;
	SSX_HIP(ctx, hipSetDevice(ctx->device));
	hipFuncAttributes at;
	uint32_t qw = 0; int nb = 0;
	int r = pick_queue(ctx, ctx->path_blob_words, &qw, &nb);
	if (r) return r;
	const KernelRef k = path_kernel_ref(ctx, qw == SSX_QUEUE_WORDS_NARROW);
	if (k.mod) {
		int v = 0;
		SSX_HIP(ctx, hipFuncGetAttribute(&v, HIP_FUNC_ATTRIBUTE_NUM_REGS, k.mod)); at.numRegs = v;
		SSX_HIP(ctx, hipFuncGetAttribute(&v, HIP_FUNC_ATTRIBUTE_SHARED_SIZE_BYTES, k.mod)); at.sharedSizeBytes = (size_t)v;
		SSX_HIP(ctx, hipFuncGetAttribute(&v, HIP_FUNC_ATTRIBUTE_LOCAL_SIZE_BYTES, k.mod)); at.localSizeBytes = (size_t)v;
	} else SSX_HIP(ctx, hipFuncGetAttributes(&at, k.host));
	if (vgprs) *vgprs = at.numRegs;
	if (sgprs) *sgprs = 0;
	if (lds_bytes) *lds_bytes = (int)at.sharedSizeBytes + (int)path_lds_bytes(ctx->path_blob_words, qw);
	if (scratch_bytes) *scratch_bytes = (int)at.localSizeBytes;
	if (max_blocks_per_cu) *max_blocks_per_cu = nb;
	return SSX_OK;
}

}

#include "ssx_progressive.hip"
#include "ssx_spectral.hip"
```

simple_spectral_amd/csrc/ssx_blob.h:

```cpp
#pragma once
#include <stdint.h>
#include <hip/hip_runtime.h>

#define SSX_QUEUE_ENTRIES 128u
#define SSX_QUEUE_WORDS_WIDE 12u
#define SSX_QUEUE_WORDS_NARROW 8u
#define SSX_LDS_PREFIX_WORDS 80u
#define SSX_BLOB_MAX_BYTES 48576u

#define SSX_PERM_COUNT 3u
#define SSX_PERM_WORDS_PER_QUAD (SSX_PERM_COUNT * 12u)
#define SSX_PERM_AXES { { 1u, 2u }, { 0u, 2u }, { 0u, 1u } }

struct SsxBlobSpectrum {
	uint32_t offset;
	uint32_t n;
	float low, delta_recip;
};

struct SsxBlobQuad {
	float pos[4][3];
	float st[4][2];
	float normal[2][3];
	uint32_t kind;
	uint32_t albedo_mode;
	uint32_t albedo_tex;
	uint32_t is_emissive;
	SsxBlobSpectrum albedo;
	SsxBlobSpectrum emission;
	uint32_t is_tri;
	uint32_t pad[1];
};
static_assert(sizeof(SsxBlobQuad) == 160, "layout");

struct SsxBlobHeader {
	double pv_inv[16];
	float cam_pos[3];
	float lambda_min, lambda_step;
	uint32_t n_quads, n_lights, n_materials, n_spectra;
	uint32_t spec_xbar, spec_ybar, spec_zbar, spec_basis_r, spec_basis_g, spec_basis_b;
	uint32_t off_perm, off_quads, off_lights, off_spectra, off_lut, off_tex;
	uint32_t n_textures;
	uint32_t total_words;
	uint32_t basis_one_grid;
	uint32_t uplift, jh_res, off_jh_scale, jh_data_lo, jh_data_hi;
	uint32_t observer_one_grid;
	uint32_t off_basis4, off_observer4;
	uint32_t topology, n_verts, off_vtab, vtab_stride, off_vid, words_without_perm, off_vtab4, off_triofs;
	uint64_t tri_valid[4];
	uint32_t perm_hbm, perm_ptr_lo, perm_ptr_hi;
	float cam_dir[3];
	uint32_t black_ends_path;
	uint32_t pad4_[1];
	float lambda_steps[4];
	double n_lights_recip;
	double q_const[4];
	double cam_pos_d[3];
};
static_assert(sizeof(SsxBlobHeader) % 16 == 0, "header must keep 16-byte alignment");

struct SsxBlobTexture {
	uint32_t ptr_lo, ptr_hi, w, h;
};

#define SSX_MAX_FRAMES 9u
#define SSX_MAX_LEVELS 10u
#define SSX_NO_SLOT 0x1FFFu
#ifndef SSX_COHORT_KS
#define SSX_COHORT_KS 2u
#endif
#define SSX_COHORT_RECORDS (64u * SSX_COHORT_KS)
#ifndef SSX_MAX_UNIT_KS
#define SSX_MAX_UNIT_KS 8u
#endif
#define SSX_UNIT_COHORTS (SSX_MAX_UNIT_KS / SSX_COHORT_KS)
#define SSX_WAVE_COUNTER_WORDS (4u * SSX_UNIT_COHORTS + 4u)
#define SSX_UNIT_PARKED 1u
#define SSX_UNIT_TURN 2u
#define SSX_BYTES_PER_SAMPLE (16u + 16u + 16u)
#define SSX_BYTES_PER_SAMPLE_FLUX (SSX_BYTES_PER_SAMPLE + 16u)
#define SSX_LOG_BYTES_PER_RECORD ((16u + 8u + 4u) * SSX_MAX_FRAMES + (16u + 16u + 1u) * SSX_MAX_LEVELS)

struct SsxKernelArgs {
	const uint32_t* blob;
	uint32_t blob_words;
	uint32_t width, height;
	uint32_t tiles_x, n_tiles;
	uint32_t tile_first, tile_stride;
	uint32_t tile_skew;
	uint32_t k0, k1;
	uint32_t indirect_only;
	uint32_t no_els;
	uint32_t my_tiles;
	uint32_t group_spp;
	uint32_t n_groups;
	uint64_t seed;
	float4* ray;
	uint4* st;
	float4* hit;
	uint8_t* logs;
	uint32_t log_cap;
	uint64_t n_records;
	uint32_t* unit_counter;
	uint32_t rgb_mode;
	uint32_t fuse_resolve;
	uint32_t unit_cohorts;
	double* accum;
	uint32_t* tile_mask;
	uint32_t* unit_state;
	uint32_t no_flat_field;
	uint32_t keep_samples;
	uint32_t pre_hits;
	uint32_t queue_words;
	uint32_t unit_grab;
	uint32_t pad_grab_;
	double inv_width, inv_height;
	uint32_t fuse_gen;
	float4* flux;
};
```

simple_spectral_amd/csrc/ssx_jit.h:

```cpp
#pragma once
#include <hip/hip_runtime.h>
#include <dlfcn.h>

#include <sys/stat.h>
#include <unistd.h>

#include <algorithm>
#include <array>
#include <chrono>
#include <condition_variable>
#include <cstdint>
#include <cstdio>
#include <cstdlib>
#include <cstring>
#include <deque>
#include <map>
#include <mutex>
#include <set>
#include <string>
#include <thread>
#include <utility>
#include <vector>

#include "ssx_sources_gen.h"
// ... 53 lines not shown
		for (uint32_t k : run.verts) {
			snprintf(b, sizeof b, "\t\tconst float z%u = vz[%u] - rs.okz, x%u = (vt[%u] - rs.okx) - rs.Sx * z%u, y%u = (vt[%u] - rs.oky) - rs.Sy * z%u;", k, k, k, 2u * k, k, k, 2u * k + 1u, k);
			line(b);
		}
		std::set<std::pair<uint32_t, uint32_t>> edges;
		for (uint32_t q = run.first; q < run.first + run.count; ++q) {
			const uint32_t a = vids[q][0], bb = vids[q][1], c = vids[q][2], d = vids[q][3];
			const uint32_t uv[5][2] = { { bb, c }, { c, a }, { a, bb }, { c, d }, { d, a } };
			for (const auto& e : uv) if (e[0] != e[1]) edges.insert({ std::min(e[0], e[1]), std::max(e[0], e[1]) });
		}
		for (const auto& e : edges) { snprintf(b, sizeof b, "\t\tconst float e%u_%u = y%u * x%u - x%u * y%u;", e.first, e.second, e.first, e.second, e.first, e.second); line(b); }
		n_edges += edges.size();
		for (uint32_t q = run.first; q < run.first + run.count; ++q) {
			const uint32_t a = vids[q][0], bb = vids[q][1], c = vids[q][2], d = vids[q][3];
			const char* acc = q < 16u ? "acc0" : "acc1";
			const std::string tri[2][3] = { { edge_expr(bb, c), edge_expr(c, a), edge_expr(a, bb) }, { edge_expr(c, d), edge_expr(d, a), edge_expr(a, c) } };
			for (const auto& t : tri) {
				snprintf(b, sizeof b, "\t\t{ const float u = %s, v = %s, w = %s; %s = __builtin_amdgcn_alignbit(%s, __float_as_uint(__builtin_fmaf(__builtin_fminf(__builtin_fminf(u, v), w), __builtin_fmaxf(__builtin_fmaxf(u, v), w), 0.0f)), 31u); } // quad %u",
				         t[0].c_str(), t[1].c_str(), t[2].c_str(), acc, acc, q);
				line(b);
			}
		}
		line("\t}");
	}
	line("}");
	std::swap(out, body);
	snprintf(b, sizeof b, "// topology \"%s\": %zu quads, %u distinct vertices of %zu corners, %zu distinct edges of %zu", name.c_str(), vids.size(), nv, 4 * vids.size(), n_edges, 5 * vids.size());
	return std::string(b) + "\n" + body;
}

struct Rtc {
	void* lib = nullptr;
	typedef void* Program;
	int (*create)(Program*, const char*, const char*, int, const char**, const char**) = nullptr;
	int (*compile)(Program, int, const char**) = nullptr;
	int (*log_size)(Program, size_t*) = nullptr;
	int (*log)(Program, char*) = nullptr;
	int (*code_size)(Program, size_t*) = nullptr;
	int (*code)(Program, char*) = nullptr;
	int (*destroy)(Program*) = nullptr;
	bool open(std::string* err) {
		if (lib) return true;
		for (const char* name : { "libhiprtc.so.7", "libhiprtc.so", "/opt/rocm/lib/libhiprtc.so" }) if ((lib = dlopen(name, RTLD_NOW | RTLD_LOCAL))) break;
		if (!lib) { const char* why = dlerror(); *err = std::string("hipRTC is not available (") + (why ? why : "dlopen failed") + ")"; return false; }
		bool ok = true;
		auto sym = [&](const char* n) { void* s = dlsym(lib, n); ok = ok && s; return s; };
		create = (decltype(create))sym("hiprtcCreateProgram"); compile = (decltype(compile))sym("hiprtcCompileProgram");
		log_size = (decltype(log_size))sym("hiprtcGetProgramLogSize"); log = (decltype(log))sym("hiprtcGetProgramLog");
		code_size = (decltype(code_size))sym("hiprtcGetCodeSize"); code = (decltype(code))sym("hiprtcGetCode");
		destroy = (decltype(destroy))sym("hiprtcDestroyProgram");
		if (!ok) { *err = "hipRTC lacks an entry point"; dlclose(lib); lib = nullptr; }
		return ok;
	}
};

struct Kernels {
	hipModule_t module = nullptr;
	hipFunction_t path = nullptr, path_nq = nullptr;
};

enum class State { Missing, Pending, Ready, Failed };

inline uint64_t fnv64(const void* data, size_t n, uint64_t h = 0xCBF29CE484222325ull) {
	const unsigned char* p = static_cast<const unsigned char*>(data);
	for (size_t i = 0; i < n; ++i) { h ^= p[i]; h *= 0x100000001B3ull; }
	return h;
}

struct Shared {
	std::mutex m;
	std::condition_variable cv;
	std::map<std::string, std::string> code, errors;
	std::set<std::string> queued;
	std::deque<std::pair<std::string, std::pair<VidTable, uint32_t>>> jobs;
	bool worker_running = false;
	std::map<std::pair<int, std::string>, Kernels> modules;
	std::set<std::string> disk_missed;
	std::mutex rtc_mutex;
	Rtc rtc;
	uint64_t compiled = 0, disk_hits = 0;
};
inline Shared& shared() { static Shared* s = new Shared; return *s; }

constexpr uint32_t kVariantFlux = 2, kVariants = 3;
inline std::string pattern_key(const VidTable& vids, uint32_t libm = 0) {
	std::string key;
	if (libm == 1u) key = "libm=glibc-2.35|";
	if (libm == kVariantFlux) key = "flux|";
	for (const auto& r : vids) key.append(reinterpret_cast<const char*>(r.data()), 4);
	return key;
}
inline const char* libm_flag(uint32_t libm) { return libm == kVariantFlux ? "-DSSX_JIT_FLUX=1" : libm ? "-DSSX_JIT_GLIBC=1" : nullptr; }

inline const char* const* compile_flags(size_t* n) {
	static const char* const flags[] = { "--offload-arch=gfx950", "-O3", "-std=c++17", "-ffp-contract=off", "-fno-slp-vectorize", "-DSSX_JIT_BUILD",
#ifdef SSX_ACCUM_FORMAL
		"-DSSX_ACCUM_FORMAL",
#endif
	};
	*n = sizeof flags / sizeof flags[0];
	return flags;
}

inline std::string cache_dir_name() {
	if (const char* e = getenv("SSX_CACHE_DIR")) return e;
	if (const char* x = getenv("XDG_CACHE_HOME")) if (x[0]) return std::string(x) + "/ssx";
	if (const char* h = getenv("HOME")) if (h[0]) return std::string(h) + "/.cache/ssx";
	return "";
}
inline std::string cache_dir() {
	const std::string dir = cache_dir_name();
	if (dir.empty()) return dir;
	struct stat st;
	if (lstat(dir.c_str(), &st) != 0) return dir;
	if (!S_ISDIR(st.st_mode) || st.st_uid != geteuid() || (st.st_mode & (S_IWGRP | S_IWOTH))) return "";
	return dir;
}
inline void cache_id(const std::string& key, const VidTable& vids, uint32_t libm, uint64_t id[2]) {
	static const std::pair<uint64_t, uint64_t> base = [] {
		uint64_t a = 0xCBF29CE484222325ull, b = 0x9E3779B97F4A7C15ull;
		const char* texts[] = { ssx_src_kernels_hip, ssx_src_blob_h, ssx_src_exact_h, ssx_src_lanestat_h, ssx_src_fmath_h, ssx_src_pass1_gen_h, ssx_src_glibc_math_h };
		for (const char* t : texts) { a = fnv64(t, strlen(t), a); b = fnv64(t, strlen(t), b); }
		size_t nf = 0; const char* const* flags = compile_flags(&nf);
		for (size_t i = 0; i < nf; ++i) { a = fnv64(flags[i], strlen(flags[i]) + 1, a); b = fnv64(flags[i], strlen(flags[i]) + 1, b); }
		int ver = 0;
		(void)hipRuntimeGetVersion(&ver);
		a = fnv64(&ver, sizeof ver, a); b = fnv64(&ver, sizeof ver, b);
		return std::make_pair(a, b);
	}();
	const std::string pass1 = pass1_source("jit", vids);
	uint64_t a = fnv64(key.data(), key.size(), base.first), b = fnv64(key.data(), key.size(), base.second);
	a = fnv64(pass1.data(), pass1.size(), a); b = fnv64(pass1.data(), pass1.size(), b);
	if (const char* lf = libm_flag(libm)) { a = fnv64(lf, strlen(lf) + 1, a); b = fnv64(lf, strlen(lf) + 1, b); }
	id[0] = a; id[1] = b;
}
inline std::string cache_file(const std::string& dir, const uint64_t id[2]) {
	char name[64];
	snprintf(name, sizeof name, "/pass1-%016llx%016llx.co", (unsigned long long)id[0], (unsigned long long)id[1]);
	return dir + name;
}
inline bool disk_load(const std::string& key, const VidTable& vids, uint32_t libm, std::string* obj) {
	const std::string dir = cache_dir();
	if (dir.empty()) return false;
	uint64_t id[2]; cache_id(key, vids, libm, id);
	FILE* f = fopen(cache_file(dir, id).c_str(), "rb");
	if (!f) return false;
	char magic[8]; uint64_t head[2] = { 0, 0 }, sum = 0;
	bool ok = fread(magic, 1, 8, f) == 8 && memcmp(magic, "SSXJIT01", 8) == 0 && fread(head, 8, 2, f) == 2 && head[0] == id[0] && head[1] > 0 && head[1] < ((uint64_t)64 << 20);
	if (ok) { obj->resize((size_t)head[1]); ok = fread(&(*obj)[0], 1, obj->size(), f) == obj->size() && fread(&sum, 8, 1, f) == 1 && sum == fnv64(obj->data(), obj->size()); }
	fclose(f);
	if (!ok) obj->clear();
	return ok;
}
inline void disk_store(const std::string& key, const VidTable& vids, uint32_t libm, const std::string& obj) {
	std::string dir = cache_dir();
	if (dir.empty()) return;
	const size_t slash = dir.rfind('/');
	if (slash != std::string::npos && slash > 0) (void)mkdir(dir.substr(0, slash).c_str(), 0700);
	(void)mkdir(dir.c_str(), 0700);
	dir = cache_dir();
	struct stat st;
	if (dir.empty() || lstat(dir.c_str(), &st) != 0) return;
	uint64_t id[2]; cache_id(key, vids, libm, id);
	const std::string path = cache_file(dir, id);
	char suffix[48]; snprintf(suffix, sizeof suffix, ".tmp.%ld.%llx", (long)getpid(), (unsigned long long)(uintptr_t)&suffix);
	const std::string tmp = path + suffix;
	FILE* f = fopen(tmp.c_str(), "wb");
	if (!f) return;
	const uint64_t head[2] = { id[0], (uint64_t)obj.size() }, sum = fnv64(obj.data(), obj.size());
	const bool ok = fwrite("SSXJIT01", 1, 8, f) == 8 && fwrite(head, 8, 2, f) == 2 && fwrite(obj.data(), 1, obj.size(), f) == obj.size() && fwrite(&sum, 8, 1, f) == 1;
	if (fclose(f) != 0 || !ok || rename(tmp.c_str(), path.c_str()) != 0) (void)remove(tmp.c_str());
}

inline bool compile(const VidTable& vids, uint32_t libm, std::string* obj, std::string* err) {
	Shared& S = shared();
// ... 136 lines not shown
```

simple_spectral_amd/csrc/ssx_kernels.hip:

```cpp
#include <hip/hip_runtime.h>
#ifndef __HIPCC_RTC__
#include <stdint.h>
#endif

#include "ssx_blob.h"
#include "ssx_exact.h"
#include "ssx_lanestat.h"
extern __shared__ __attribute__((aligned(16))) uint32_t ssx_lds[];
#define SSX_FM_TABLE (reinterpret_cast<const double*>(ssx_lds))
#ifdef SSX_JIT_BUILD
#include "ssx_fmath.h"
#else
#include "../../include/ssx_fmath.h"
#endif
#define SSX_GM_TABLE (SSX_FM_TABLE + SSX_FM_I_A11)
#ifdef SSX_JIT_BUILD
#include "ssx_glibc_math.h"
#else
#include "../../include/ssx_glibc_math.h"
#endif
__device__ const double ssx_fm_coeff_values[SSX_FM_N_COEFF] = SSX_FM_COEFF_INIT;
__device__ const double ssx_gm_coeff_values[SSX_GM_N_COEFF] = SSX_GM_COEFF_INIT;
static_assert(2 * SSX_FM_N_COEFF <= SSX_LDS_PREFIX_WORDS, "coefficient table");
static_assert(SSX_FM_I_A11 + SSX_GM_N_COEFF <= SSX_FM_N_COEFF, "glibc coefficients in the arc-cosine slots");
// ... 720 lines not shown
	int ignore;
	uint32_t depth;
	uint32_t rec_index;
	uint32_t prev_slot;
	int hit_tri;
	float hit_dist;
	float hit_st_x, hit_st_y;
};

__device__ __forceinline__ float4& log_fs(const SsxKernelArgs& a, uint32_t i) { return *reinterpret_cast<float4*>(a.logs + i * 16u); }
__device__ __forceinline__ float4& log_nee(const SsxKernelArgs& a, uint32_t i) { return *reinterpret_cast<float4*>(a.logs + (a.log_cap * (16u * SSX_MAX_FRAMES) + i * 16u)); }
__device__ __forceinline__ float4& log_direct(const SsxKernelArgs& a, uint32_t i) { return *reinterpret_cast<float4*>(a.logs + (a.log_cap * (16u * SSX_MAX_FRAMES + 16u * SSX_MAX_LEVELS) + i * 16u)); }
__device__ __forceinline__ float2& log_np(const SsxKernelArgs& a, uint32_t i) { return *reinterpret_cast<float2*>(a.logs + (a.log_cap * (16u * SSX_MAX_FRAMES + 32u * SSX_MAX_LEVELS) + i * 8u)); }
__device__ __forceinline__ uint32_t& log_link(const SsxKernelArgs& a, uint32_t i) { return *reinterpret_cast<uint32_t*>(a.logs + (a.log_cap * (24u * SSX_MAX_FRAMES + 32u * SSX_MAX_LEVELS) + i * 4u)); }
__device__ __forceinline__ uint8_t& log_vis(const SsxKernelArgs& a, uint32_t i) { return a.logs[a.log_cap * (28u * SSX_MAX_FRAMES + 32u * SSX_MAX_LEVELS) + i]; }

struct LogRef {
	uint32_t* cnt;
	uint32_t wave_base;
	uint32_t tagw;
	__device__ __forceinline__ uint32_t group() const { return tagw & (2u * SSX_UNIT_COHORTS - 1u); }
	__device__ __forceinline__ uint32_t log_rec() const { return (wave_base + ((tagw >> 3) & 7u)) * SSX_COHORT_RECORDS; }
	__device__ __forceinline__ uint32_t rc(uint32_t rec_index) const { return ((tagw >> 8) << 6) | (rec_index & 63u); }
};
__device__ __forceinline__ uint32_t log_region(const SsxKernelArgs& a, uint32_t wave_slot, uint32_t tag, uint32_t cohort) {
	return ((wave_slot * 2u + tag) * a.unit_cohorts + cohort) * SSX_COHORT_RECORDS;
}
__device__ __forceinline__ void wave_release(uint32_t* cnt) { (void)__hip_atomic_fetch_add(cnt + 4u * SSX_UNIT_COHORTS, 1u, __ATOMIC_RELEASE, __HIP_MEMORY_SCOPE_WAVEFRONT); }
__device__ __forceinline__ void wave_acquire(uint32_t* cnt) { (void)__hip_atomic_load(cnt + 4u * SSX_UNIT_COHORTS, __ATOMIC_ACQUIRE, __HIP_MEMORY_SCOPE_WAVEFRONT); }
__device__ __forceinline__ uint32_t log_append(const LogRef& lg, uint32_t which) {
	return __hip_atomic_fetch_add(lg.cnt + 2u * lg.group() + which, 1u, __ATOMIC_RELAXED, __HIP_MEMORY_SCOPE_WAVEFRONT);
}

template <typename Args>
__device__ __forceinline__ void camera_dir(const SsxBlobHeader& h, const Args& a, double x, double y, double& dx, double& dy, double& dz) {
	const bool pow2 = ((a.width & (a.width - 1u)) | (a.height & (a.height - 1u))) == 0u;
	double st_x, st_y;
	if (pow2) { st_x = x * a.inv_width; st_y = y * a.inv_height; }
	else { st_x = x / (double)a.width; st_y = y / (double)a.height; }
	double ndc_x = st_x * 2.0 - 1.0, ndc_y = st_y * 2.0 - 1.0;
	double q[4];
#pragma unroll
	for (int r = 0; r < 4; ++r)
		q[r] = (h.pv_inv[0 * 4 + r] * ndc_x + h.pv_inv[1 * 4 + r] * ndc_y) + h.q_const[r];
	double w = q[3];
	double px = q[0] / w, py = q[1] / w, pz = q[2] / w;
	dx = px - h.cam_pos_d[0]; dy = py - h.cam_pos_d[1]; dz = pz - h.cam_pos_d[2];
}
template <typename Args>
__device__ __forceinline__ void generate_sample(const SsxBlobHeader& h, const Args& a, uint32_t i, uint32_t j, uint32_t k, float4& ray, uint4& st) {
	const uint64_t pixel = (uint64_t)j * (uint64_t)a.width + (uint64_t)i;
	const uint64_t pa = mix64(a.seed + 0x9E3779B97F4A7C15ull * (pixel + 1ull));
	const uint64_t b = mix64(pa + 0x9E3779B97F4A7C15ull * ((uint64_t)k + 1ull));
	Rng rng;
	rng.state = b;
	rng.inc = mix64(b ^ 0xDA3E39CB94B95BDBull) | 1ull;
	double sub_y = rand_1d(rng);
	double sub_x = rand_1d(rng);
	double dx, dy, dz;
	camera_dir(h, a, (double)i + sub_x, (double)j + sub_y, dx, dy, dz);
	double inv = 1.0 / __builtin_sqrt((dx * dx + dy * dy) + dz * dz);
	const float lambda_0 = a.rgb_mode ? 0.0f : h.lambda_min + rand_1f(rng) * h.lambda_step;
	ray = make_float4((float)(dx * inv), (float)(dy * inv), (float)(dz * inv), lambda_0);
	st = make_uint4((uint32_t)rng.state, (uint32_t)(rng.state >> 32), (uint32_t)rng.inc, (uint32_t)(rng.inc >> 32));
}

#define SSX_SQ_FLUSH_AT 64u
#define SSX_SQ_CAPACITY 128u
struct ShadowQ {
	float4* e;
	uint32_t count;
	uint32_t* cnt;
};

__device__ __forceinline__ void hit_st(const SsxBlobQuad& Q, uint32_t which, const HitInfo& hit, float& st_x, float& st_y) {
	float bx = hit.U * hit.det_recip, by = hit.V * hit.det_recip, bz = hit.W * hit.det_recip;
	const float* s0 = Q.st[0];
	const float* s1 = which ? Q.st[2] : Q.st[1];
	const float* s2 = which ? Q.st[3] : Q.st[2];
	st_x = (bx * s0[0] + by * s1[0]) + bz * s2[0];
	st_y = (bx * s0[1] + by * s1[1]) + bz * s2[1];
}

template <bool NARROW, bool BLACK, bool GLIBC = false>
__device__ __forceinline__ bool path_step(const Lds& L, const ShadowQ& q, const SsxKernelArgs& a, const LogRef& lg, Path& p, bool& pushed, uint32_t& level_word) {
	const SsxBlobHeader& h = L.hdr();
	level_word = SSX_NO_SLOT << 13;
	SSX_STAT(4);
	const uint32_t hq = (uint32_t)p.hit_tri >> 1, which = (uint32_t)p.hit_tri & 1u;
	const SsxBlobQuad& Q = L.quad(hq);
	const SsxBlobQuad& M = Q;
	V3 N = mk(Q.normal[which][0], Q.normal[which][1], Q.normal[which][2]);

	float direct[4] = { 0.0f, 0.0f, 0.0f, 0.0f };
	const bool els = a.no_els == 0u;
	if ((els ? (p.depth == 0u && !a.indirect_only) : true) && M.is_emissive != 0u) {
		SSX_STAT(5);
		Hero em = spectrum_hero(L, M.emission, p.lambda_0, h.lambda_step);
#pragma unroll
		for (int k = 0; k < 4; ++k) direct[k] += em.v[k];
		log_direct(a, lg.log_rec() * SSX_MAX_LEVELS + p.depth * SSX_COHORT_RECORDS + lg.rc(p.rec_index)) = make_float4(direct[0], direct[1], direct[2], direct[3]);
		level_word |= 1u << 26;
	}
	if (p.depth + 1u >= SSX_MAX_DEPTH_) return false;
	const V3 hit_pos = add(p.orig, scl(p.hit_dist, p.dir));
	p.orig = hit_pos;
	if (M.albedo_mode != 0u) { SSX_STAT(6); } else { SSX_STAT(7); }
	Hero alb = material_albedo(L, Q, p.hit_st_x, p.hit_st_y, p.lambda_0);
	float f_lamb[4];
#pragma unroll
	for (int k = 0; k < 4; ++k) f_lamb[k] = SSX_DIV_CONST(alb.v[k], SSX_PI_F);

	if (BLACK && M.kind == 0u && h.black_ends_path != 0u && f_lamb[0] == 0.0f && f_lamb[1] == 0.0f && f_lamb[2] == 0.0f && f_lamb[3] == 0.0f) {
		SSX_STAT(18);
		if (els && (!a.indirect_only || p.depth > 0u)) skip_light_draws(L, p.rng);
		skip_coshemi_draws(p.rng);
		return false;
	}
	if (els && (!a.indirect_only || p.depth > 0u)) {
		V3 sdir; uint32_t light; float spdf;
		SSX_STAT(8);
		sample_light<GLIBC>(L, p.rng, hit_pos, sdir, light, spdf);
		float n_dot_l = dot3(sdir, N);
		if (n_dot_l > 0.0f) {
			SSX_STAT(9);
			Hero emitted = spectrum_hero(L, L.quad(light).emission, p.lambda_0, h.lambda_step);
			float c[4];
			const double spdf_recip = ssx_exact::div64_rcp_any(spdf);
#pragma unroll
			for (int k = 0; k < 4; ++k) {
				float fs = (M.kind == 0u) ? f_lamb[k] : 0.0f;
				c[k] = ssx_exact::div64_by((emitted.v[k] * n_dot_l) * fs, spdf_recip);
			}
			if (c[0] != 0.0f || c[1] != 0.0f || c[2] != 0.0f || c[3] != 0.0f) {
				SSX_STAT(10);
				const uint64_t pushing = __ballot(1);
				const uint32_t slot = q.count + __builtin_amdgcn_mbcnt_hi((uint32_t)(pushing >> 32), __builtin_amdgcn_mbcnt_lo((uint32_t)pushing, 0u));
				const uint32_t nslot = log_append(lg, 1u);
				const uint32_t ni = lg.log_rec() * SSX_MAX_LEVELS + nslot;
				if (NARROW) {
					log_nee(a, ni) = make_float4(c[0], c[1], c[2], c[3]);
					float4* E = q.e + 2u * slot;
					E[0] = make_float4(hit_pos.x, hit_pos.y, hit_pos.z, sdir.x);
					E[1] = make_float4(sdir.y, sdir.z, __uint_as_float((light << 8) | hq), __uint_as_float(ni));
				} else {
					float4* E = q.e + 3u * slot;
					E[0] = make_float4(hit_pos.x, hit_pos.y, hit_pos.z, sdir.x);
					E[1] = make_float4(sdir.y, sdir.z, c[0], c[1]);
					E[2] = make_float4(c[2], c[3], __uint_as_float((light << 8) | hq), __uint_as_float(ni));
				}
				level_word = (level_word & ~(SSX_NO_SLOT << 13)) | (nslot << 13);
				pushed = true;
			}
		}
	}

	V3 w_i; float pdf_w_i; float f_s[4];
	if (M.kind == 0u) {
		SSX_STAT(11);
		w_i = rand_coshemi<GLIBC>(p.rng, pdf_w_i);
		w_i = get_rotated_to(w_i, N);
#pragma unroll
		for (int k = 0; k < 4; ++k) f_s[k] = f_lamb[k];
	} else {
		w_i = reflect3(mk(-p.dir.x, -p.dir.y, -p.dir.z), N);
		pdf_w_i = __builtin_inff();
#pragma unroll
		for (int k = 0; k < 4; ++k) f_s[k] = alb.v[k];
	}
	bool cont = false;
	float n_dot_l = 0.0f;
	float dotfs = (f_s[0] * f_s[0] + f_s[1] * f_s[1]) + (f_s[2] * f_s[2] + f_s[3] * f_s[3]);
	if (dotfs > 0.0f) {
		if (__builtin_isfinite(pdf_w_i)) n_dot_l = dot3(w_i, N);
		else { n_dot_l = 1.0f; pdf_w_i = 1.0f; }
		cont = n_dot_l > 0.0f;
	}
	if (!cont || (els && p.depth + 2u >= SSX_MAX_DEPTH_)) return false;
	SSX_STAT(12);
	const uint32_t slot = log_append(lg, 0u);
	const uint32_t entry = lg.log_rec() * SSX_MAX_FRAMES + slot;
	log_fs(a, entry) = make_float4(f_s[0], f_s[1], f_s[2], f_s[3]);
	log_np(a, entry) = make_float2(n_dot_l, pdf_w_i);
	log_link(a, entry) = p.prev_slot | level_word;
	wave_release(lg.cnt);
	p.prev_slot = slot;
	p.dir = w_i; p.ignore = (int)hq;
	++p.depth;
	return true;
}

template <int TOPO, bool NARROW>
__device__ __forceinline__ void shadow_flush(const Lds& L, const SsxKernelArgs& a, const ShadowQ& q, uint32_t first, uint32_t n, SsxTimer& tm) {
	const uint32_t lane = threadIdx.x & 63u;
	const bool have = lane < n;
	const bool narrow = NARROW;
	float4 e0 = make_float4(0.0f, 0.0f, 0.0f, 0.0f), e1 = make_float4(0.0f, 1.0f, 0.0f, 0.0f), e2 = e0;
	if (have) {
		if (narrow) { const float4* E = q.e + 2u * (first + lane); e0 = E[0]; e1 = E[1]; e2.z = e1.z; e2.w = e1.w; }
		else { const float4* E = q.e + 3u * (first + lane); e0 = E[0]; e1 = E[1]; e2 = E[2]; }
	}
	const uint32_t tag = __float_as_uint(e2.z);
	HitInfo sh;
	trace<TOPO>(L, mk(e0.x, e0.y, e0.z), mk(e0.w, e1.x, e1.y), (int)(tag & 0xFFu), have, sh, 2, nullptr, &tm);
	if (have) {
		const bool visible = sh.tri >= 0 && ((uint32_t)sh.tri >> 1) == (tag >> 8);
		if (narrow) log_vis(a, __float_as_uint(e2.w)) = visible ? (uint8_t)1 : (uint8_t)0;
		else log_nee(a, __float_as_uint(e2.w)) = visible ? make_float4(e1.z, e1.w, e2.x, e2.y) : make_float4(0.0f, 0.0f, 0.0f, 0.0f);
		wave_release(q.cnt);
	}
}

__device__ __forceinline__ const __attribute__((address_space(4))) SsxKernelArgs& cold_args() {
	auto p = __builtin_amdgcn_kernarg_segment_ptr();
	asm volatile("" : "+s"(p));
	return *(const __attribute__((address_space(4))) SsxKernelArgs*)p;
}
__device__ __forceinline__ double ld_agent(const double* p) { return __hip_atomic_load(p, __ATOMIC_RELAXED, __HIP_MEMORY_SCOPE_AGENT); }
__device__ __forceinline__ void st_agent(double* p, double v) { __hip_atomic_store(p, v, __ATOMIC_RELAXED, __HIP_MEMORY_SCOPE_AGENT); }
__device__ __forceinline__ void add_sample(bool rgb_mode, double acc[4], float x, float y, float z, float alpha) {
	if (rgb_mode) { acc[0] += (double)x; acc[1] += (double)y; acc[2] += (double)z; acc[3] += (double)alpha; }
	else { acc[0] += (double)(x * 0.001f); acc[1] += (double)(y * 0.001f); acc[2] += (double)(z * 0.001f); acc[3] += (double)(alpha * 0.001f); }
}
__device__ __forceinline__ void stage_sample(float4* rec, float x, float y, float z, float alpha) {
	uint64_t* const q = reinterpret_cast<uint64_t*>(rec);
	__hip_atomic_store(q, (uint64_t)__float_as_uint(x) | ((uint64_t)__float_as_uint(y) << 32), __ATOMIC_RELAXED, __HIP_MEMORY_SCOPE_AGENT);
	__hip_atomic_store(q + 1, (uint64_t)__float_as_uint(z) | ((uint64_t)__float_as_uint(alpha) << 32), __ATOMIC_RELAXED, __HIP_MEMORY_SCOPE_AGENT);
}
__device__ __forceinline__ void add_staged_sample(bool rgb_mode, double acc[4], const float4* rec) {
	const uint64_t* const q = reinterpret_cast<const uint64_t*>(rec);
	const uint64_t lo = __hip_atomic_load(q, __ATOMIC_RELAXED, __HIP_MEMORY_SCOPE_AGENT), hi = __hip_atomic_load(q + 1, __ATOMIC_RELAXED, __HIP_MEMORY_SCOPE_AGENT);
	add_sample(rgb_mode, acc, __uint_as_float((uint32_t)lo), __uint_as_float((uint32_t)(lo >> 32)), __uint_as_float((uint32_t)hi), __uint_as_float((uint32_t)(hi >> 32)));
}
template <bool NARROW>
__device__ __forceinline__ float4 nee_term(const SsxKernelArgs& a, uint32_t i, bool has) {
	uint32_t v = 1u;
	float4 c = make_float4(0.0f, 0.0f, 0.0f, 0.0f);
	if (has) {
		if (NARROW) v = log_vis(a, i);
		c = log_nee(a, i);
	}
	if (!NARROW) return c;
	return make_float4(v ? c.x : 0.0f, v ? c.y : 0.0f, v ? c.z : 0.0f, v ? c.w : 0.0f);
}
template <uint32_t WAYS, bool NARROW, bool FLUX = false>
__device__ __forceinline__ void resolve_records(const Lds& L, const SsxKernelArgs& a, uint32_t r0, uint32_t stride, uint32_t count, uint32_t fs_base, uint32_t nee_base, uint32_t rc0, double acc[4], bool stage) {
	float rad[WAYS][4];
	uint32_t depth[WAYS];
	uint32_t K[WAYS];
	uint32_t at[WAYS];
	uint32_t top = 0;
	const float4 zero4 = make_float4(0.0f, 0.0f, 0.0f, 0.0f);
#pragma unroll
	for (uint32_t s = 0; s < WAYS; ++s) {
		depth[s] = 0; K[s] = 0; at[s] = 0;
		rad[s][0] = rad[s][1] = rad[s][2] = rad[s][3] = 0.0f;
		if (s < count) {
			const uint32_t y = a.st[r0 + s * stride].y;
			const uint32_t dep = (y >> 2) & 0xFu;
			depth[s] = dep | ((y & 1u) << 4);
			at[s] = (y >> 6) & SSX_NO_SLOT;
			const uint32_t ns = y >> 19;
			float4 last = zero4;
			if ((y >> 1) & 1u) last = log_direct(a, nee_base + dep * SSX_COHORT_RECORDS + rc0 + s * 64u);
			const float4 ne = nee_term<NARROW>(a, nee_base + ns, ns != SSX_NO_SLOT);
			if (dep) K[s] = log_link(a, fs_base + at[s]);
			rad[s][0] = last.x + ne.x; rad[s][1] = last.y + ne.y; rad[s][2] = last.z + ne.z; rad[s][3] = last.w + ne.w;
			top = max(top, dep);
		}
	}
	for (uint32_t d = top; d-- > 0u;) {
		float4 D[WAYS], F[WAYS]; float2 NP[WAYS];
#pragma unroll
		for (uint32_t s = 0; s < WAYS; ++s)
			if (d < (depth[s] & 0xFu)) {
				const uint32_t i = fs_base + at[s];
				F[s] = log_fs(a, i); NP[s] = log_np(a, i);
				const uint32_t ns = (K[s] >> 13) & SSX_NO_SLOT;
				const bool has_ne = ns != SSX_NO_SLOT;
				D[s] = nee_term<NARROW>(a, nee_base + ns, has_ne);
				if ((K[s] >> 26) & 1u) {
					const float4 em = log_direct(a, nee_base + d * SSX_COHORT_RECORDS + rc0 + s * 64u);
					D[s] = has_ne ? make_float4(em.x + D[s].x, em.y + D[s].y, em.z + D[s].z, em.w + D[s].w) : em;
				}
				at[s] = K[s] & SSX_NO_SLOT;
				if (d) K[s] = log_link(a, fs_base + at[s]);
			}
#pragma unroll
		for (uint32_t s = 0; s < WAYS; ++s)
			if (d < (depth[s] & 0xFu)) {
				SSX_STAT(14);
				const double pdf_recip = ssx_exact::div64_rcp_any(NP[s].y);
				rad[s][0] = D[s].x + ssx_exact::div64_by((rad[s][0] * NP[s].x) * F[s].x, pdf_recip);
				rad[s][1] = D[s].y + ssx_exact::div64_by((rad[s][1] * NP[s].x) * F[s].y, pdf_recip);
				rad[s][2] = D[s].z + ssx_exact::div64_by((rad[s][2] * NP[s].x) * F[s].z, pdf_recip);
				rad[s][3] = D[s].w + ssx_exact::div64_by((rad[s][3] * NP[s].x) * F[s].w, pdf_recip);
			}
	}
	const __attribute__((address_space(4))) SsxKernelArgs& c = cold_args();
	const bool rgb_mode = c.rgb_mode != 0u, keep_samples = c.keep_samples != 0u, no_flat_field = c.no_flat_field != 0u;
#pragma unroll
	for (uint32_t s = 0; s < WAYS; ++s)
		if (s < count) {
			SSX_STAT(15);
			if (no_flat_field) {
				const float4 cr = a.ray[r0 + s * stride];
				const SsxBlobHeader& hh = L.hdr();
				const float d = dot3(mk(cr.x, cr.y, cr.z), mk(hh.cam_dir[0], hh.cam_dir[1], hh.cam_dir[2]));
				rad[s][0] *= d; rad[s][1] *= d; rad[s][2] *= d; rad[s][3] *= d;
			}
			Hero flux; flux.v[0] = rad[s][0]; flux.v[1] = rad[s][1]; flux.v[2] = rad[s][2]; flux.v[3] = rad[s][3];
			if (FLUX) c.flux[r0 + s * stride] = make_float4(rad[s][0], rad[s][1], rad[s][2], rad[s][3]);
			float xyz[3];
			if (rgb_mode) { xyz[0] = rad[s][0]; xyz[1] = rad[s][1]; xyz[2] = rad[s][2]; }
			else flux_to_xyz(L, flux, __uint_as_float(a.st[r0 + s * stride].x), xyz);
			const float alpha = (depth[s] >> 4) ? 1.0f : 0.0f;
			if (stage) stage_sample(a.ray + (r0 + s * stride), xyz[0], xyz[1], xyz[2], alpha);
			else {
				add_sample(rgb_mode, acc, xyz[0], xyz[1], xyz[2], alpha);
				if (keep_samples) a.ray[r0 + s * stride] = make_float4(xyz[0], xyz[1], xyz[2], alpha);
			}
		}
}

}

template <typename Args>
__device__ __forceinline__ uint32_t tile_of_slot(const Args& a, uint32_t slot, uint32_t& tx, uint32_t& ty) {
	const uint32_t t = a.tile_first + slot * a.tile_stride;
	ty = t / a.tiles_x;
	const uint32_t txr = t - ty * a.tiles_x, rot = (ty * a.tile_skew) % a.tiles_x;
	tx = txr >= rot ? txr - rot : txr + a.tiles_x - rot;
	return ty * a.tiles_x + tx;
}
__device__ __forceinline__ void generate_body(const SsxKernelArgs& a) {
	Lds L; L.w = stage_lds(a);
	const SsxBlobHeader& h = L.hdr();
	const V3 cam = mk(h.cam_pos[0], h.cam_pos[1], h.cam_pos[2]);
	const uint32_t n_k = a.k1 - a.k0;
	const uint32_t lane = threadIdx.x & 63u;
	const uint64_t n_waves = a.n_records >> 6;
	for (uint64_t sk = (uint64_t)blockIdx.x * (blockDim.x >> 6) + (threadIdx.x >> 6); sk < n_waves; sk += (uint64_t)gridDim.x * (blockDim.x >> 6)) {
		const uint32_t slot = (uint32_t)(sk / n_k), kk = a.k0 + (uint32_t)(sk % n_k);
		uint32_t tx, ty;
		(void)tile_of_slot(a, slot, tx, ty);
		const uint32_t i = tx * 8u + (lane & 7u), j = ty * 8u + (lane >> 3);
		const bool inside = i < a.width && j < a.height;
		float4 ray = make_float4(0.0f, 0.0f, 1.0f, 0.0f); uint4 st = make_uint4(0u, 0u, 0u, 0u);
		if (inside) generate_sample(h, a, i, j, kk, ray, st);
		const uint64_t r = sk * 64u + lane;
		if (!a.pre_hits) {
			if (inside) { a.ray[r] = ray; a.st[r] = st; }
			continue;
		}
		HitInfo hit;
		trace<0>(L, cam, mk(ray.x, ray.y, ray.z), -1, inside, hit, 16, a.tile_mask + 4u * slot);
		if (inside) {
			float st_x = 0.0f, st_y = 0.0f;
			if (hit.tri >= 0) {
				const SsxBlobQuad& Q = L.quad((uint32_t)hit.tri >> 1);
				if (Q.albedo_mode != 0u) hit_st(Q, (uint32_t)hit.tri & 1u, hit, st_x, st_y);
			} else {
				st = make_uint4(__float_as_uint(ray.w), (SSX_NO_SLOT << 6) | (SSX_NO_SLOT << 19), st.x, st.y);
			}
			a.ray[r] = ray;
			a.st[r] = st;
			a.hit[r] = make_float4(hit.dist, st_x, st_y, __int_as_float(hit.tri));
		}
	}
}
#ifndef SSX_JIT_BUILD
extern "C" __global__ void __launch_bounds__(256) ssx_generate_kernel(SsxKernelArgs a) { generate_body(a); }

extern "C" __global__ void __launch_bounds__(256) ssx_tile_mask_kernel(SsxKernelArgs a) {
	const SsxBlobHeader& h = *reinterpret_cast<const SsxBlobHeader*>(a.blob);
	const uint32_t slot = blockIdx.x * 4u + (threadIdx.x >> 6), lane = threadIdx.x & 63u;
	if (slot >= a.my_tiles) return;
	uint32_t tx, ty;
	(void)tile_of_slot(a, slot, tx, ty);
	const double x0 = (double)(tx * 8u), y0 = (double)(ty * 8u);
	double d[4][3], c[3];
	camera_dir(h, a, x0, y0, d[0][0], d[0][1], d[0][2]);
	camera_dir(h, a, x0 + 8.0, y0, d[1][0], d[1][1], d[1][2]);
	camera_dir(h, a, x0 + 8.0, y0 + 8.0, d[2][0], d[2][1], d[2][2]);
	camera_dir(h, a, x0, y0 + 8.0, d[3][0], d[3][1], d[3][2]);
	camera_dir(h, a, x0 + 4.0, y0 + 4.0, c[0], c[1], c[2]);
	double n[4][3];
#pragma unroll
	for (int k = 0; k < 4; ++k) {
		const double* p = d[k]; const double* q = d[(k + 1) & 3];
		double nx = p[1] * q[2] - p[2] * q[1], ny = p[2] * q[0] - p[0] * q[2], nz = p[0] * q[1] - p[1] * q[0];
		const double inv = 1.0 / __builtin_sqrt(nx * nx + ny * ny + nz * nz);
		const double sgn = (nx * c[0] + ny * c[1] + nz * c[2]) < 0.0 ? -inv : inv;
		n[k][0] = nx * sgn; n[k][1] = ny * sgn; n[k][2] = nz * sgn;
	}
	const SsxBlobQuad* quads = reinterpret_cast<const SsxBlobQuad*>(a.blob + h.off_quads);
	for (uint32_t g = 0; g < 2u; ++g) {
		const uint32_t q = g * 64u + lane;
		bool keep = false;
		if (q < h.n_quads) {
			keep = true;
#pragma unroll
			for (int k = 0; k < 4; ++k) {
				bool all_out = true;
#pragma unroll
				for (int v = 0; v < 4; ++v) {
					const double vx = (double)quads[q].pos[v][0] - (double)h.cam_pos[0], vy = (double)quads[q].pos[v][1] - (double)h.cam_pos[1], vz = (double)quads[q].pos[v][2] - (double)h.cam_pos[2];
					const double dist = __builtin_sqrt(vx * vx + vy * vy + vz * vz);
					const double sd = n[k][0] * vx + n[k][1] * vy + n[k][2] * vz;
					all_out = all_out && (sd < -1.0e-4 * dist);
				}
				if (all_out) keep = false;
			}
		}
		const uint64_t m = __ballot(keep);
		if (lane == 0u) { a.tile_mask[4u * slot + 2u * g] = (uint32_t)m; a.tile_mask[4u * slot + 2u * g + 1u] = (uint32_t)(m >> 32); }
	}
}
#endif

struct WorkUnit {
	uint32_t slot, grp;
	uint32_t tile;
	uint32_t txy;
	uint32_t dims;
	__device__ __forceinline__ uint32_t tw() const { return dims & 15u; }
	__device__ __forceinline__ uint32_t th() const { return (dims >> 4) & 15u; }
	__device__ __forceinline__ uint32_t n_kq() const { return dims >> 8; }
	__device__ __forceinline__ uint32_t npx() const { return tw() * th(); }
	__device__ __forceinline__ uint32_t n_items() const { return npx() * n_kq(); }
	__device__ __forceinline__ uint32_t k_off(const SsxKernelArgs& a) const { return grp * a.group_spp; }
	__device__ __forceinline__ uint32_t rec_base(const SsxKernelArgs& a) const { return (slot * (a.k1 - a.k0) + grp * a.group_spp) * 64u; }
};
// ... 30 lines not shown
}
#ifdef SSX_ACCUM_FORMAL
#define SSX_SUMS_ACQ __ATOMIC_ACQUIRE
#define SSX_SUMS_ACQ_REL __ATOMIC_ACQ_REL
#else
#define SSX_SUMS_ACQ __ATOMIC_RELAXED
#define SSX_SUMS_ACQ_REL __ATOMIC_RELAXED
#endif
__device__ __forceinline__ void sums_chain(uint32_t slot, uint32_t grp, uint32_t lane, uint32_t* cnt) {
	const __attribute__((address_space(4))) SsxKernelArgs& a = cold_args();
	uint32_t tx, ty;
	const uint32_t tile = tile_of_slot(a, slot, tx, ty);
	const bool has_px = (lane & 7u) < min(8u, a.width - tx * 8u) && (lane >> 3) < min(8u, a.height - ty * 8u);
	double* const px = a.accum + (size_t)tile * 256u + lane;
	uint32_t* state = a.unit_state + (slot * a.n_groups + grp);
	uint32_t rec_at = (slot * (a.k1 - a.k0) + grp * a.group_spp) * 64u;
	double acc[4] = { 0.0, 0.0, 0.0, 0.0 };
	if (has_px) { acc[0] = ld_agent(px); acc[1] = ld_agent(px + 64); acc[2] = ld_agent(px + 128); acc[3] = ld_agent(px + 192); }
	for (;;) {
		const uint32_t n = min(a.group_spp, (a.k1 - a.k0) - grp * a.group_spp);
		if (has_px) {
			for (uint32_t kq = 0; kq < n; ++kq) add_staged_sample(a.rgb_mode != 0u, acc, a.ray + (rec_at + kq * 64u + lane));
			st_agent(px, acc[0]); st_agent(px + 64, acc[1]); st_agent(px + 128, acc[2]); st_agent(px + 192, acc[3]);
		}
		if (++grp >= a.n_groups) return;
		sums_release(cnt);
		++state; rec_at += a.group_spp * 64u;
		uint32_t was = 0u;
		if (lane == 0u) was = __hip_atomic_fetch_or(state, SSX_UNIT_TURN, SSX_SUMS_ACQ_REL, __HIP_MEMORY_SCOPE_AGENT);
		was = (uint32_t)__builtin_amdgcn_readfirstlane((int)was);
		sums_acquire(cnt);
		if (was != SSX_UNIT_PARKED) return;
		if (lane == 0u) atomicAdd(a.unit_counter + 3, 1u);
	}
}
template <bool NARROW, bool FLUX = false>
__device__ __forceinline__ void unit_fold(const Lds& L, const SsxKernelArgs& a, const WorkUnit& u, uint32_t wave_slot, uint32_t tag, uint32_t* cnt) {
	wave_acquire(cnt);
	__builtin_amdgcn_fence(__ATOMIC_RELEASE, "workgroup");
	__builtin_amdgcn_fence(__ATOMIC_ACQUIRE, "agent");
	const uint32_t lane = threadIdx.x & 63u;
	const bool has_px = (lane & 7u) < u.tw() && (lane >> 3) < u.th();
	const __attribute__((address_space(4))) SsxKernelArgs& c = cold_args();
	uint32_t* const state = c.unit_state + (u.slot * c.n_groups + u.grp);
	double* const px = c.accum + (size_t)u.tile * 256u + lane;
	bool mine = true;
	if (u.grp) {
		mine = ((uint32_t)__builtin_amdgcn_readfirstlane((int)__hip_atomic_load(state, SSX_SUMS_ACQ, __HIP_MEMORY_SCOPE_AGENT)) & SSX_UNIT_TURN) != 0u;
		sums_acquire(cnt);
	}
	double acc[4] = { 0.0, 0.0, 0.0, 0.0 };
	if (mine && has_px) { acc[0] = ld_agent(px); acc[1] = ld_agent(px + 64); acc[2] = ld_agent(px + 128); acc[3] = ld_agent(px + 192); }
	if (has_px)
		for (uint32_t kq = 0, n_kq = u.n_kq(), rec_base = u.rec_base(a); kq < n_kq; kq += SSX_COHORT_KS) {
			const uint32_t log_rec = log_region(a, wave_slot, tag, kq / SSX_COHORT_KS);
			resolve_records<SSX_COHORT_KS, NARROW, FLUX>(L, a, rec_base + kq * 64u + lane, 64u, min(SSX_COHORT_KS, n_kq - kq), log_rec * SSX_MAX_FRAMES, log_rec * SSX_MAX_LEVELS, lane, acc, !mine);
		}
	if (mine) {
		if (has_px) { st_agent(px, acc[0]); st_agent(px + 64, acc[1]); st_agent(px + 128, acc[2]); st_agent(px + 192, acc[3]); }
		if (u.grp + 1u >= c.n_groups) return;
		sums_release(cnt);
		uint32_t was = 0u;
		if (lane == 0u) was = __hip_atomic_fetch_or(state + 1, SSX_UNIT_TURN, SSX_SUMS_ACQ_REL, __HIP_MEMORY_SCOPE_AGENT);
		was = (uint32_t)__builtin_amdgcn_readfirstlane((int)was);
		sums_acquire(cnt);
		if (was != SSX_UNIT_PARKED) return;
		if (lane == 0u) atomicAdd(c.unit_counter + 3, 1u);
		sums_chain(u.slot, u.grp + 1u, lane, cnt);
	} else {
		sums_release(cnt);
		uint32_t was = 0u;
		if (lane == 0u) {
			atomicAdd(c.unit_counter + 2, 1u);
			uint32_t expected = 0u;
			(void)__hip_atomic_compare_exchange_strong(state, &expected, SSX_UNIT_PARKED, SSX_SUMS_ACQ_REL, SSX_SUMS_ACQ, __HIP_MEMORY_SCOPE_AGENT);
			was = expected;
		}
		was = (uint32_t)__builtin_amdgcn_readfirstlane((int)was);
		sums_acquire(cnt);
		if (was == SSX_UNIT_TURN) sums_chain(u.slot, u.grp, lane, cnt);
	}
}

template <int TOPO, bool NARROW, bool CALIB = false, bool GLIBC = false, bool FLUX = false>
__device__ __forceinline__ void render_body(const SsxKernelArgs& a) {
	constexpr bool FUSE_GEN = TOPO == 2;
	uint32_t* const lds_words = stage_lds<GLIBC>(a);
	Lds L; L.w = lds_words;

	const uint32_t wave = (uint32_t)__builtin_amdgcn_readfirstlane((int)(threadIdx.x >> 6)), lane = threadIdx.x & 63u;
	const uint32_t wave_slot = blockIdx.x * 4u + wave;
	const SsxBlobHeader& hg = *reinterpret_cast<const SsxBlobHeader*>(a.blob);
	const V3 cam = mk(hg.cam_pos[0], hg.cam_pos[1], hg.cam_pos[2]);

	Path p;
	p.orig = mk(0.0f, 0.0f, 0.0f); p.dir = mk(0.0f, 0.0f, 1.0f); p.ignore = -1; p.depth = 0; p.rec_index = 0; p.lambda_0 = 0.0f; p.prev_slot = SSX_NO_SLOT;
	p.hit_tri = 0; p.hit_dist = 0.0f; p.hit_st_x = p.hit_st_y = 0.0f;
	p.rng.state = 0; p.rng.inc = 1;
	bool active = false;
	uint32_t p_tag = 0;
	constexpr uint32_t queue_words = SSX_QUEUE_ENTRIES * (NARROW ? SSX_QUEUE_WORDS_NARROW : SSX_QUEUE_WORDS_WIDE);
	uint32_t* const log_cnt = lds_words + a.blob_words + 4u * queue_words + wave * SSX_WAVE_COUNTER_WORDS;
	SsxTimer tm;
#ifdef SSX_REGTIME
	tm.acc = reinterpret_cast<unsigned long long*>(lds_words + a.blob_words + 4u * queue_words + 4u * SSX_WAVE_COUNTER_WORDS) + wave * SSX_NTIME;
	if (lane < (uint32_t)SSX_NTIME) tm.acc[lane] = 0ull;
	tm.last = __builtin_amdgcn_s_memtime();
#endif
	ShadowQ sq;
	sq.e = reinterpret_cast<float4*>(lds_words + a.blob_words + wave * queue_words);
	sq.count = 0; sq.cnt = log_cnt;
	WorkUnit cur, old;
	bool cur_valid = false, old_pending = false, more = true;
	uint32_t cur_tag = 0, old_tag = 0;
	uint32_t next_item = 0;
	uint32_t grab = 0;
	auto end_path = [&](uint32_t level_word, uint32_t hit_anything) {
		const uint32_t tail = hit_anything | ((level_word >> 26) << 1) | (p.depth << 2) | (p.prev_slot << 6) | ((level_word >> 13) << 19);
		a.st[p.rec_index] = make_uint4(__float_as_uint(p.lambda_0), tail, (uint32_t)p.rng.state, (uint32_t)(p.rng.state >> 32));
		wave_release(log_cnt);
		active = false;
	};
	auto refill = [&](bool with_hit) {
		const uint32_t n_items = cur.n_items();
		if (!(cur_valid && next_item < n_items)) return;
		const uint64_t idle = __ballot(!active);
		if (!active) {
			const uint32_t item = next_item + __builtin_amdgcn_mbcnt_hi((uint32_t)(idle >> 32), __builtin_amdgcn_mbcnt_lo((uint32_t)idle, 0u));
			if (item < n_items) {
				SSX_STAT(19);
				uint32_t in_tile, kq;
				const uint32_t npx = cur.npx(), tw = cur.tw();
				if (npx == 64u) { in_tile = item & 63u; kq = item >> 6; }
				else { const uint32_t r = item % npx; kq = item / npx; in_tile = (r / tw) * 8u + r % tw; }
				p.rec_index = cur.rec_base(a) + kq * 64u + in_tile;
				float4 ray; uint4 st;
				if (FUSE_GEN && a.fuse_gen) {
					const __attribute__((address_space(4))) SsxKernelArgs& c = cold_args();
					generate_sample(L.hdr(), c, (cur.txy & 0xFFFFu) * 8u + (in_tile & 7u), (cur.txy >> 16) * 8u + (in_tile >> 3), c.k0 + cur.grp * c.group_spp + kq, ray, st);
					if (c.no_flat_field) c.ray[p.rec_index] = ray;
				} else {
					ray = a.ray[p.rec_index];
					st = a.st[p.rec_index];
				}
				p.dir = mk(ray.x, ray.y, ray.z);
				p.lambda_0 = ray.w;
				p.rng.state = ((uint64_t)st.y << 32) | st.x;
				p.rng.inc = ((uint64_t)st.w << 32) | st.z;
				p.orig = cam;
				p.ignore = -1;
				p.depth = 0;
				p.prev_slot = SSX_NO_SLOT;
				const uint32_t cohort = kq / SSX_COHORT_KS;
				p_tag = cohort | (cur_tag << 2) | ((cur_tag * a.unit_cohorts + cohort) << 3) | ((kq % SSX_COHORT_KS) << 8);
				active = true;
				if (with_hit) {
					const float4 ht = a.hit[p.rec_index];
					p.hit_dist = ht.x; p.hit_st_x = ht.y; p.hit_st_y = ht.z; p.hit_tri = __float_as_int(ht.w);
					active = p.hit_tri >= 0;
				}
			}
		}
		next_item = min(n_items, next_item + (uint32_t)__popcll(idle));
	};
	auto flush_fold = [&]() {
		const bool busy = __any(active);
		const bool fold_old = old_pending && !__any(active && ((p_tag >> 2) & 1u) == old_tag);
		const bool drain = (fold_old && a.fuse_resolve) || !busy;
		while (sq.count >= SSX_SQ_FLUSH_AT || (drain && sq.count)) {
			const uint32_t take = min(sq.count, 64u);
			sq.count -= take;
			shadow_flush<TOPO, NARROW>(L, a, sq, sq.count, take, tm);
			SSX_TIME(tm, 5);
		}
		if (fold_old) {
			if (a.fuse_resolve) unit_fold<NARROW, FLUX>(L, a, old, wave_slot, old_tag, log_cnt);
			old_pending = false;
			SSX_TIME(tm, 6);
		}
	};
	auto rotate_fetch = [&]() {
		if (cur_valid && next_item >= cur.n_items() && !old_pending) {
			old = cur; old_tag = cur_tag; old_pending = true;
			cur_valid = false;
		}
		if (!cur_valid && more) {
			const __attribute__((address_space(4))) SsxKernelArgs& c = cold_args();
			uint32_t u = 0;
			const uint32_t total = c.my_tiles * c.n_groups;
			if (TOPO != 1 && ((grab >> 26) & 31u)) { u = grab & 0x3FFFFFFu; grab += 1u - (1u << 26); }
			else {
				const uint32_t single = TOPO != 1 ? grab >> 31 : 1u, want = single ? 1u : c.unit_grab;
				if (lane == 0u) u = atomicAdd(c.unit_counter, want);
				u = (uint32_t)__builtin_amdgcn_readfirstlane((int)u);
				if (u < total) {
					const uint32_t got = min(want, total - u);
					if (TOPO != 1) grab = (u + 1u) | ((got - 1u) << 26) | ((single | (total - u < gridDim.x * 4u * want * 4u ? 1u : 0u)) << 31);
				}
			}
			if (u < total) {
				unit_setup(a, u, cur); cur_tag ^= 1u; next_item = 0; cur_valid = true;
				if (lane < 2u * SSX_UNIT_COHORTS) log_cnt[2u * SSX_UNIT_COHORTS * cur_tag + lane] = 0u;
			}
			else more = false;
		}
	};
	for (;;) {
		{
			bool pushed = false;
			if (active) {
				SSX_STAT(13);
				LogRef lg;
				lg.cnt = log_cnt; lg.wave_base = wave_slot * 2u * a.unit_cohorts; lg.tagw = p_tag;
				uint32_t level_word;
				if (!path_step<NARROW, TOPO != 1, GLIBC>(L, sq, a, lg, p, pushed, level_word)) end_path(level_word, 1u);
			}
			sq.count += (uint32_t)__popcll(__ballot(pushed));
		}
		SSX_TIME(tm, 3);
		rotate_fetch();
		if (!a.pre_hits) refill(false);
		SSX_TIME(tm, 4);
		flush_fold();
		SSX_TIME(tm, 14);
		if (__any(active)) {
			HitInfo hit;
			trace<TOPO>(L, p.orig, p.dir, p.ignore, active, hit, 0, nullptr, &tm);
			p.hit_tri = hit.tri; p.hit_dist = hit.dist;
			float st_x = 0.0f, st_y = 0.0f;
			if (CALIB) { const uint32_t left = (uint32_t)__popcll(__ballot(active && hit.tri < 0)); if (lane == 0u && left) atomicAdd(a.unit_counter + 1, left); }
			if (active) {
				if (hit.tri < 0) end_path(SSX_NO_SLOT << 13, p.depth ? 1u : 0u);
				else {
					const SsxBlobQuad& Q = L.quad((uint32_t)hit.tri >> 1);
					if (Q.albedo_mode != 0u) hit_st(Q, (uint32_t)hit.tri & 1u, hit, st_x, st_y);
				}
			}
			p.hit_st_x = st_x; p.hit_st_y = st_y;
		}
		SSX_TIME(tm, 9);
		if (a.pre_hits) refill(true);
		SSX_TIME(tm, 10);
		if (!__any(active) && !cur_valid && !more && !old_pending && sq.count == 0u) break;
	}
#ifdef SSX_REGTIME
	if (lane < (uint32_t)SSX_NTIME) atomicAdd(&g_regtime[lane], tm.acc[lane]);
#endif
}

#ifndef SSX_WAVES_PER_EU
#define SSX_WAVES_PER_EU 4
#endif
#ifndef SSX_JIT_GLIBC
#define SSX_JIT_GLIBC 0
#endif
#ifndef SSX_JIT_FLUX
#define SSX_JIT_FLUX 0
#endif
#define SSX_PATH_KERNEL(name, topo, narrow, glibc, flux) \
	extern "C" __global__ void __launch_bounds__(256) __attribute__((amdgpu_waves_per_eu(SSX_WAVES_PER_EU))) name(SsxKernelArgs a) { render_body<topo, narrow, false, glibc, flux>(a); }
#ifdef SSX_JIT_BUILD
SSX_PATH_KERNEL(ssx_render_kernel_jit, 3, false, SSX_JIT_GLIBC, SSX_JIT_FLUX)
SSX_PATH_KERNEL(ssx_render_kernel_jit_nq, 3, true, SSX_JIT_GLIBC, SSX_JIT_FLUX)
#else
SSX_PATH_KERNEL(ssx_render_kernel, 0, false, false, false)
SSX_PATH_KERNEL(ssx_render_kernel_cornell, 1, false, false, false)
#ifndef SSX_PROBE_BUILD
SSX_PATH_KERNEL(ssx_render_kernel_plane, 2, false, false, false)
SSX_PATH_KERNEL(ssx_render_kernel_nq, 0, true, false, false)
SSX_PATH_KERNEL(ssx_render_kernel_cornell_nq, 1, true, false, false)
SSX_PATH_KERNEL(ssx_render_kernel_plane_nq, 2, true, false, false)
SSX_PATH_KERNEL(ssx_render_kernel_glibc, 0, false, true, false)
SSX_PATH_KERNEL(ssx_render_kernel_cornell_glibc, 1, false, true, false)
SSX_PATH_KERNEL(ssx_render_kernel_plane_glibc, 2, false, true, false)
SSX_PATH_KERNEL(ssx_render_kernel_nq_glibc, 0, true, true, false)
SSX_PATH_KERNEL(ssx_render_kernel_cornell_nq_glibc, 1, true, true, false)
SSX_PATH_KERNEL(ssx_render_kernel_plane_nq_glibc, 2, true, true, false)
SSX_PATH_KERNEL(ssx_render_kernel_flux, 0, false, false, true)
SSX_PATH_KERNEL(ssx_render_kernel_cornell_flux, 1, false, false, true)
SSX_PATH_KERNEL(ssx_render_kernel_plane_flux, 2, false, false, true)
SSX_PATH_KERNEL(ssx_render_kernel_nq_flux, 0, true, false, true)
SSX_PATH_KERNEL(ssx_render_kernel_cornell_nq_flux, 1, true, false, true)
SSX_PATH_KERNEL(ssx_render_kernel_plane_nq_flux, 2, true, false, true)
#endif
extern "C" __global__ void __launch_bounds__(256) __attribute__((amdgpu_waves_per_eu(3))) ssx_calibrate_kernel(SsxKernelArgs a) { render_body<0, true, true>(a); }
#endif

#ifndef SSX_JIT_BUILD
#include "ssx_pixel_grid.h"
extern "C" __global__ void __launch_bounds__(256) ssx_finalize_kernel(const double* accum, float4* out, SsxPixelGrid g, uint32_t spp, uint32_t rgb_mode, uint32_t done_tiles) {
	const uint32_t p = blockIdx.x * blockDim.x + threadIdx.x;
	if (p >= g.width * g.height) return;
	const uint32_t i = p % g.width, j = p / g.width;
	const uint32_t tile = ssx_shared_tile(g, i, j);
	float4 o = make_float4(0.0f, 0.0f, 0.0f, 0.0f);
	if (tile % g.tile_stride == g.tile_first && tile / g.tile_stride < done_tiles) {
		const double* const px = accum + ssx_sum_slot(i, j, g.tiles_x);
		if (rgb_mode) {
			const double n = (double)spp;
			o.x = (float)(px[0] / n);
			o.y = (float)(px[64] / n);
			o.z = (float)(px[128] / n);
			o.w = (float)(px[192] / n);
		} else {
			const double sc = 1000.0 / (double)spp;
			o.x = (float)(px[0] * sc);
			o.y = (float)(px[64] * sc);
			o.z = (float)(px[128] * sc);
			o.w = (float)(px[192] * sc);
		}
	}
	out[p] = o;
}

extern "C" __global__ void __launch_bounds__(256) ssx_sum_kernel(float4* dst, const float4* src, uint32_t n) {
	const uint32_t p = blockIdx.x * blockDim.x + threadIdx.x;
	if (p >= n) return;
	const float4 a = dst[p], b = src[p];
	dst[p] = make_float4(a.x + b.x, a.y + b.y, a.z + b.z, a.w + b.w);
}
#endif
```

simple_spectral_amd/csrc/ssx_pack.h:

```cpp
#pragma once

namespace {

uint32_t align4(uint32_t words) { return (words + 3u) & ~3u; }

const uint32_t kPermAxes[3][2] = SSX_PERM_AXES;

int validate_scene(const ssx_scene_desc* s, std::string& err) {
	auto bad = [&](int code, const std::string& msg) { err = msg; return code; };
	if (s->n_quads == 0 || s->n_quads > SSX_MAX_QUADS) return bad(SSX_ERR_SCENE, fmt("n_quads=%u outside 1..%u", s->n_quads, SSX_MAX_QUADS));
	if (s->n_lights == 0) return bad(SSX_ERR_SCENE, "scene has no lights (reference asserts !lights.empty(), scene.cpp:30)");
	if (s->n_textures > SSX_MAX_TEXTURES) return bad(SSX_ERR_SCENE, "too many textures");
	const uint32_t spec_ids[6] = { s->spec_xbar, s->spec_ybar, s->spec_zbar, s->spec_basis_r, s->spec_basis_g, s->spec_basis_b };
	for (uint32_t id : spec_ids) if (id >= s->n_spectra) return bad(SSX_ERR_ARG, "observer/basis spectrum index out of range");
	for (uint32_t i = 0; i < s->n_spectra; ++i) {
		const ssx_spectrum& sp = s->spectra[i];
		if (sp.n < 2) return bad(SSX_ERR_DATA, "Must have at-least two elements in sampled spectrum!");
		if ((uint64_t)sp.offset + sp.n > s->n_samples) return bad(SSX_ERR_ARG, "spectrum samples out of range");
	}
	if (s->uplift == SSX_MODE_RGB) {
		if (s->lambda_min != 0.0f || s->lambda_step != 1.0f) return bad(SSX_ERR_ARG, "RGB mode needs lambda_min = 0, lambda_step = 1");
		for (uint32_t i = 0; i < s->n_spectra; ++i)
			if (s->spectra[i].n != 4u || s->spectra[i].low != 0.0f || s->spectra[i].delta_recip != 1.0f || s->samples[s->spectra[i].offset + 3u] != 0.0f)
				return bad(SSX_ERR_ARG, "RGB mode needs every spectrum as {r,g,b,0} with low = 0, delta_recip = 1");
	}
	for (uint32_t i = 0; i < s->n_materials; ++i) {
		const ssx_material& m = s->materials[i];
		if (m.kind > SSX_MTL_MIRROR || m.albedo_mode > SSX_ALBEDO_TEXTURE) return bad(SSX_ERR_ARG, "bad material kind/mode");
		if (m.emission_spectrum >= s->n_spectra) return bad(SSX_ERR_ARG, "material emission spectrum out of range");
		if (m.albedo_mode == SSX_ALBEDO_CONSTANT && m.albedo_spectrum >= s->n_spectra) return bad(SSX_ERR_ARG, "material albedo spectrum out of range");
		if (m.albedo_mode == SSX_ALBEDO_TEXTURE && m.albedo_texture >= s->n_textures) return bad(SSX_ERR_ARG, "material texture out of range");
	}
	for (uint32_t i = 0; i < s->n_quads; ++i) if (s->quads[i].material >= s->n_materials) return bad(SSX_ERR_ARG, "quad material out of range");
	for (uint32_t i = 0; i < s->n_quads; ++i) if (s->quads[i].flags & ~(uint32_t)(SSX_PRIM_LIGHT | SSX_PRIM_TRI)) return bad(SSX_ERR_ARG, "unknown primitive flags");
	for (uint32_t i = 0; i < s->n_quads; ++i) {
		const ssx_vertex* vs[4] = { &s->quads[i].v00, &s->quads[i].v10, &s->quads[i].v11, &s->quads[i].v01 };
		const int nv = (s->quads[i].flags & SSX_PRIM_TRI) ? 3 : 4;
		for (int v = 0; v < nv; ++v) for (float c : vs[v]->pos) if (!(std::fabs(c) <= 0x1p30f)) return bad(SSX_ERR_SCENE, "vertex coordinate beyond 2^30 (or not a number)");
	}
	for (float c : s->cam_pos) if (!(std::fabs(c) <= 0x1p30f)) return bad(SSX_ERR_SCENE, "camera position beyond 2^30 (or not a number)");
	for (uint32_t i = 0; i < s->n_lights; ++i) if (s->lights[i] >= s->n_quads) return bad(SSX_ERR_ARG, "light index out of range");
	return SSX_OK;
}

struct PackInfo { bool candidate = false; ssx_jit::VidTable vid; };

struct BlobLayout {
	SsxBlobHeader h{};
	std::vector<uint32_t> sample_pos;
	ssx_jit::VidTable vid;
	std::vector<const float*> distinct;
};

void scene_constants(const ssx_scene_desc* s, SsxBlobHeader& h) {
	memcpy(h.pv_inv, s->pv_inv, sizeof h.pv_inv);
	memcpy(h.cam_pos, s->cam_pos, sizeof h.cam_pos);
	std::memcpy(h.cam_dir, s->cam_dir, sizeof h.cam_dir);
	h.lambda_min = s->lambda_min; h.lambda_step = s->lambda_step;
	h.n_quads = s->n_quads; h.n_lights = s->n_lights; h.n_materials = s->n_materials; h.n_spectra = s->n_spectra;
	h.spec_xbar = s->spec_xbar; h.spec_ybar = s->spec_ybar; h.spec_zbar = s->spec_zbar;
	h.spec_basis_r = s->spec_basis_r; h.spec_basis_g = s->spec_basis_g; h.spec_basis_b = s->spec_basis_b;
	h.n_textures = s->n_textures;
	h.uplift = s->uplift;
	h.n_lights_recip = 1.0 / (double)(float)s->n_lights;
	for (int r = 0; r < 4; ++r) { volatile double z = 0.0, one = 1.0; h.q_const[r] = h.pv_inv[2 * 4 + r] * z + h.pv_inv[3 * 4 + r] * one; }
	for (int k = 0; k < 3; ++k) h.cam_pos_d[k] = (double)s->cam_pos[k];
	h.black_ends_path = 1u;
	for (uint32_t i = 0; i < s->n_lights; ++i) {
		const ssx_spectrum& es = s->spectra[s->materials[s->quads[s->lights[i]].material].emission_spectrum];
		for (uint32_t k = 0; k < es.n; ++k) if (!(std::fabs(s->samples[es.offset + k]) <= 0x1p60f)) h.black_ends_path = 0u;
	}
	if (const char* e = debug_env("SSX_BLACK_SHORTCUT")) { if (e[0] == '0') h.black_ends_path = 0u; }
	for (int i = 0; i < 4; ++i) { volatile float fi = (float)i; h.lambda_steps[i] = fi * s->lambda_step; }
	const ssx_spectrum &r = s->spectra[s->spec_basis_r], &g = s->spectra[s->spec_basis_g], &b = s->spectra[s->spec_basis_b];
	const ssx_spectrum &ox = s->spectra[s->spec_xbar], &oy = s->spectra[s->spec_ybar], &oz = s->spectra[s->spec_zbar];
	h.observer_one_grid = (ox.n == oy.n && ox.n == oz.n && ox.low == oy.low && ox.low == oz.low && ox.delta_recip == oy.delta_recip && ox.delta_recip == oz.delta_recip) ? 1u : 0u;
	h.basis_one_grid = (r.n == g.n && r.n == b.n && r.low == g.low && r.low == b.low && r.delta_recip == g.delta_recip && r.delta_recip == b.delta_recip) ? 1u : 0u;
	for (uint32_t q = 0; q < s->n_quads; ++q) h.tri_valid[q >> 5] |= ((s->quads[q].flags & SSX_PRIM_TRI) ? 1ull : 3ull) << (2u * (q & 31u));
}

int layout_blob(const ssx_scene_desc* s, const void* d_jh, int force_topology, PackInfo* info, BlobLayout& L, std::string& err) {
	SsxBlobHeader& h = L.h;
	scene_constants(s, h);

	L.vid.assign(s->n_quads, std::array<uint8_t, 4>{});
	bool any_tri = false;
	for (uint32_t q = 0; q < s->n_quads; ++q) any_tri = any_tri || (s->quads[q].flags & SSX_PRIM_TRI);
	const bool topo_candidate = s->n_quads <= 32u && !any_tri;
	for (uint32_t q = 0; topo_candidate && q < s->n_quads; ++q) {
		const ssx_vertex* vs[4] = { &s->quads[q].v00, &s->quads[q].v10, &s->quads[q].v11, &s->quads[q].v01 };
		for (int v = 0; v < 4; ++v) {
			size_t k = 0;
			while (k < L.distinct.size() && memcmp(L.distinct[k], vs[v]->pos, 12) != 0) ++k;
			if (k == L.distinct.size()) L.distinct.push_back(vs[v]->pos);
			L.vid[q][v] = (uint8_t)k;
		}
	}
	h.topology = 0; h.n_verts = (uint32_t)L.distinct.size();
	for (const SsxTopology& t : ssx_topologies) {
		if (!topo_candidate || t.n_quads != s->n_quads || t.n_verts != L.distinct.size()) continue;
		bool same = true;
		for (uint32_t q = 0; q < s->n_quads && same; ++q) for (int v = 0; v < 4; ++v) same = same && t.vid[q][v] == L.vid[q][v];
		if (same) h.topology = t.id;
	}
	if (env_on("SSX_GENERIC_KERNEL")) h.topology = 0;
	if (info) { info->candidate = topo_candidate && h.topology == 0 && !env_on("SSX_GENERIC_KERNEL"); info->vid = L.vid; }
	if (force_topology == 3 && topo_candidate) h.topology = 3;

	uint32_t off = (uint32_t)(sizeof(SsxBlobHeader) / 4);
	h.off_quads = off;     off = align4(off + s->n_quads * (uint32_t)(sizeof(SsxBlobQuad) / 4));
	h.off_lights = off;    off = align4(off + s->n_lights);
	h.off_spectra = off;   off = align4(off + s->n_spectra * (uint32_t)(sizeof(SsxBlobSpectrum) / 4));
	std::vector<uint8_t> table_needed(s->n_spectra, 0);
	for (uint32_t i = 0; i < s->n_materials; ++i) {
		table_needed[s->materials[i].emission_spectrum] = 1;
		if (s->materials[i].albedo_mode == SSX_ALBEDO_CONSTANT) table_needed[s->materials[i].albedo_spectrum] = 1;
	}
	if (!h.basis_one_grid) table_needed[s->spec_basis_r] = table_needed[s->spec_basis_g] = table_needed[s->spec_basis_b] = 1;
	if (!h.observer_one_grid) table_needed[s->spec_xbar] = table_needed[s->spec_ybar] = table_needed[s->spec_zbar] = 1;
	L.sample_pos.assign(s->n_spectra, 0u);
	for (uint32_t i = 0; i < s->n_spectra; ++i) if (table_needed[i]) { L.sample_pos[i] = off + 2u; off += s->spectra[i].n + 4u; }
	off = align4(off);
	auto one_grid4 = [&](uint32_t ia, uint32_t flag) -> uint32_t {
		if (!flag) return 0u;
		const uint32_t at = off + 8u;
		off = align4(off + 4u * (s->spectra[ia].n + 4u));
		return at;
	};
	h.off_basis4 = one_grid4(s->spec_basis_r, h.basis_one_grid);
	h.off_observer4 = one_grid4(s->spec_xbar, h.observer_one_grid);
	h.off_lut = off;       off = align4(off + 256u);
	h.off_tex = off;       off = align4(off + s->n_textures * (uint32_t)(sizeof(SsxBlobTexture) / 4));
	if (s->uplift == SSX_UPLIFT_JH) {
		h.jh_res = s->jh_res;
		h.off_jh_scale = off;  off = align4(off + s->jh_res);
	}
	if (s->uplift == SSX_UPLIFT_JH || s->uplift == SSX_UPLIFT_MENG) {
		h.jh_data_lo = (uint32_t)(uintptr_t)d_jh; h.jh_data_hi = (uint32_t)((uint64_t)(uintptr_t)d_jh >> 32);
	}
	if (h.topology) {
		h.vtab_stride = (3u * h.n_verts + 1u) & ~1u;
		h.off_vtab = off;  off = align4(off + SSX_PERM_COUNT * h.vtab_stride);
		h.off_vid = off;   off = align4(off + s->n_quads);
		h.off_vtab4 = off; off = align4(off + SSX_PERM_COUNT * 4u * h.n_verts);
		h.off_triofs = off; off = align4(off + 4u * s->n_quads);
	}
	h.words_without_perm = off;
	h.off_perm = off;      off = align4(off + s->n_quads * SSX_PERM_WORDS_PER_QUAD);
	h.total_words = off;
	h.perm_hbm = ((size_t)off * 4 > SSX_BLOB_MAX_BYTES) ? 1u : 0u;
	const uint32_t staged = h.perm_hbm ? h.words_without_perm : off;
	if ((size_t)staged * 4 > SSX_BLOB_MAX_BYTES) { err = fmt("scene tables need %u bytes of LDS (max %u)", staged * 4, SSX_BLOB_MAX_BYTES); return SSX_ERR_SCENE; }
	return SSX_OK;
}

// ... 92 lines not shown
```

simple_spectral_amd/renderer.py:

```python
import ctypes as C
import os
from dataclasses import dataclass, field
from typing import Optional, Tuple

import numpy as np

from . import _capi

ROOT = os.path.dirname(os.path.dirname(os.path.abspath(__file__)))
DEFAULT_DATA_DIR = os.path.join(ROOT, "data")


class SsxError(RuntimeError):
    def __init__(self, code, message):
        super().__init__("ssx error %d: %s" % (code, message))
        self.code = code


@dataclass
class Options:
    scene_name: str = "cornell-srgb"
    res: Tuple[int, int] = (512, 512)
    spp: int = 16
    indirect_only: bool = False
# ... 285 lines not shown
        info = _capi.SsxSpectralInfo()
        self._check(self._lib.ssx_spectral_read(self._ctx, C.byref(info), None, None, None))
        H, W, B = info.height, info.width, info.bins
        mean = np.zeros((H, W, B), dtype=np.float32)
        counts = np.zeros((H, W, B // 4), dtype=np.uint32)
        s = np.zeros((H, W, B), dtype=np.float64) if sums else None
        self._check(self._lib.ssx_spectral_read(self._ctx, C.byref(info), mean.ctypes.data, None if s is None else s.ctypes.data, counts.ctypes.data))
        return info, mean, counts, s

    def spectral_image(self):
        info, mean, counts, _ = self.spectral_read()
        centres = np.float32(info.lambda_min) + (np.arange(info.bins, dtype=np.float32) + np.float32(0.5)) * np.float32(info.bin_width)
        return mean, counts, centres.astype(np.float32)

    def debug_sample_flux(self, **over):
        p = self.params(**over)
        flux = np.zeros((p.height, p.width, p.spp, 4), dtype=np.float32)
        lambda_0 = np.zeros((p.height, p.width, p.spp), dtype=np.float32)
        self._check(self._lib.ssx_debug_sample_flux(self._ctx, C.byref(p), flux.ctypes.data, lambda_0.ctypes.data))
        return flux, lambda_0

    def render_device(self, d_ptr, stream=0, **over):
        p = self.params(**over)
        self._check(self._lib.ssx_render_device(self._ctx, C.byref(p), C.c_void_p(d_ptr), C.c_void_p(stream)))

    def render_device_wait(self):
        self._check(self._lib.ssx_render_device_wait(self._ctx))

    def set_jit(self, mode=_capi.SSX_JIT_AT_UPLOAD):
        self._check(self._lib.ssx_set_jit(self._ctx, int(mode)))

    def jit_status(self, wait_ms=0):
        buf = C.create_string_buffer(1024)
        st = self._lib.ssx_jit_status(self._ctx, int(wait_ms), buf, len(buf))
        if st < -1:
            self._check(st)
        return st, buf.value.decode(errors="replace")

    def upload_scene_desc(self, desc):
        self._check(self._lib.ssx_upload_scene(self._ctx, C.byref(desc) if not hasattr(desc, "contents") else desc))

    def debug_eval(self, op, inputs, out_words):
        x = np.ascontiguousarray(inputs)
        assert x.ndim == 2 and x.dtype.itemsize == 4
        out = np.zeros((x.shape[0], out_words), dtype=np.uint32)
        self._check(self._lib.ssx_debug_eval(self._ctx, op, x.ctypes.data, x.shape[1], out.ctypes.data, out_words, x.shape[0]))
        return out

    def debug_sweep(self, op, lo=0, count=1 << 32):
        res = (C.c_uint64 * 11)()
        self._check(self._lib.ssx_debug_sweep(self._ctx, op, lo, count, res))
        return int(res[0]), int(res[1]), [int(res[3 + k]) for k in range(min(int(res[2]), 8))]

    def debug_samples(self, **over):
        p = self.params(**over)
        xyza = np.zeros((p.height, p.width, p.spp, 4), dtype=np.float32)
        state = np.zeros((p.height, p.width, p.spp), dtype=np.uint64)
        levels = np.zeros((p.height, p.width, p.spp), dtype=np.uint32)
        self._check(self._lib.ssx_debug_samples(self._ctx, C.byref(p), xyza.ctypes.data, state.ctypes.data, levels.ctypes.data))
        return xyza, state, levels

    def set_timing(self, enable=True):
        self._check(self._lib.ssx_set_timing(self._ctx, int(enable)))

    def get_timing(self):
        ms = (C.c_float * 4)()
        self._check(self._lib.ssx_get_timing(self._ctx, ms))
        return dict(zip(("generate", "path", "resolve", "accumulate"), [float(x) for x in ms]))

    def kernel_info(self):
        v = [C.c_int() for _ in range(5)]
        self._check(self._lib.ssx_kernel_info(self._ctx, *[C.byref(x) for x in v]))
        return dict(zip(("vgprs", "sgprs", "lds_bytes", "scratch_bytes", "max_blocks_per_cu"), [x.value for x in v]))

    def plan_info(self):
        f, k = C.c_float(), C.c_int()
        self._check(self._lib.ssx_plan_info(self._ctx, C.byref(f), C.byref(k)))
        variant = {0: "generic", 1: "cornell topology", 2: "plane topology", 3: "scene topology (compiled at upload)"}.get(self._lib.ssx_kernel_variant(self._ctx), "?")
        name = self._lib.ssx_kernel_name(self._ctx)
        left, pre = C.c_float(), C.c_int()
        if hasattr(self._lib, "ssx_calibration_info"):
            self._check(self._lib.ssx_calibration_info(self._ctx, None, C.byref(left), C.byref(pre)))
        fused = (not pre.value) and variant == "plane topology" and not (os.environ.get("SSX_DEBUG_ENV") == "1" and os.environ.get("SSX_FUSE_GEN", "")[:1] == "0")
        return {"frames_per_sample": round(f.value, 3), "fold": "path kernel", "pass1": variant,
                "rays_left_per_sample": round(left.value, 3), "camera_rays": "pre-traced (generate kernel)" if pre.value else "path loop",
                "samples_made_in": "path kernel (refill)" if fused else "generate kernel",
                "kernel": name.decode() if name else None}

    def scratch_info(self):
        a, b = C.c_uint64(), C.c_uint64()
        if hasattr(self._lib, "ssx_scratch_info"):
            self._check(self._lib.ssx_scratch_info(self._ctx, C.byref(a), C.byref(b)))
        return {"sample_bytes": a.value, "log_bytes": b.value}

    def sums_info(self):
        a, b = C.c_uint64(), C.c_uint64()
        if hasattr(self._lib, "ssx_sums_info"):
            self._check(self._lib.ssx_sums_info(self._ctx, C.byref(a), C.byref(b)))
        u = C.c_uint64()
        if hasattr(self._lib, "ssx_units_info"):
            self._check(self._lib.ssx_units_info(self._ctx, C.byref(u)))
        return {"units_parked": a.value, "units_chained": b.value, "units": u.value}

    def save(self, path):
        fb = np.ascontiguousarray(self.framebuffer, dtype=np.float32)
        rc = _capi.host_lib().ssh_save_image(path.encode(), fb.ctypes.data, fb.shape[1], fb.shape[0])
        if rc != 0:
            raise SsxError(rc, _capi.host_lib().ssh_last_error().decode())

    def close(self):
        if self._ctx:
            self._lib.ssx_destroy(self._ctx)
            self._ctx = C.c_void_p()

    def __del__(self):
        try:
            self.close()
        except Exception:
            pass
```

Baseline: 3191.

## Precompute light emission spectrum per sample in generate kernel when lights share emission

When every light uses the same emission spectrum, the generate kernel evaluates the emission hero-wavelength values once per sample and stores them in a new per-sample float4 array. The path kernel then loads these values at each explicit light connection instead of re-evaluating the spectrum. A new 'plain' kernel variant keeps the old path for non-uniform emission scenes, and the plane topology is excluded. This trades repeated spectrum lookups and interpolation for an extra 16 bytes per sample of memory traffic and allocation.

Result: slower. 3141 (-1.6%).

```diff
diff --git a/include/ssx.h b/include/ssx.h
--- a/include/ssx.h
+++ b/include/ssx.h
@@ -149,6 +149,7 @@
 int ssx_plan_info(ssx_ctx* ctx, float* frames_per_sample, int* fold_in_path_kernel);
 int ssx_calibration_info(ssx_ctx* ctx, float* frames_per_sample, float* rays_left_per_sample, int* camera_rays_pretraced);
 int ssx_scratch_info(ssx_ctx* ctx, uint64_t* sample_bytes, uint64_t* log_bytes);
+int ssx_path_invariants_info(ssx_ctx* ctx, int* on, uint64_t* invariant_bytes);
 int ssx_sums_info(ssx_ctx* ctx, uint64_t* units_parked, uint64_t* units_chained);
 int ssx_units_info(ssx_ctx* ctx, uint64_t* units_enqueued);
 int ssx_kernel_variant(ssx_ctx* ctx);
diff --git a/simple_spectral_amd/_capi.py b/simple_spectral_amd/_capi.py
--- a/simple_spectral_amd/_capi.py
+++ b/simple_spectral_amd/_capi.py
@@ -91,7 +91,7 @@
                "ssx_device_framebuffer", "ssx_device_index", "ssx_read_framebuffer", "ssx_accumulate_peer",
                "ssx_debug_eval", "ssx_debug_samples", "ssx_debug_sweep", "ssx_kernel_variant", "ssx_kernel_name", "ssx_scratch_info", "ssx_calibration_info", "ssx_set_jit", "ssx_debug_pass1_source", "ssx_done_spp", "ssx_reduce_rccl", "ssx_sums_info", "ssx_rccl_groups_made", "ssx_jit_status", "ssx_jit_counters", "ssx_done_tiles", "ssx_render_device_wait", "ssx_units_info", "ssx_rccl_probe",
                "ssx_render_continue", "ssx_scene_digest", "ssx_sums_export", "ssx_sums_import", "ssx_set_noise_estimate", "ssx_noise_info",
-               "ssx_set_spectral_bins", "ssx_spectral_read", "ssx_debug_sample_flux"]
+               "ssx_set_spectral_bins", "ssx_spectral_read", "ssx_debug_sample_flux", "ssx_path_invariants_info"]
 (SSX_SWEEP_RCP, SSX_SWEEP_SQRT, SSX_SWEEP_INVERSESQRT, SSX_SWEEP_SIN, SSX_SWEEP_COS, SSX_SWEEP_ACOS, SSX_SWEEP_DIV_PI,
  SSX_SWEEP_RCP64, SSX_SWEEP_DIV_PAIRS, SSX_SWEEP_ACOS_SIN, SSX_SWEEP_SIN_PROOF, SSX_SWEEP_COS_PROOF, SSX_SWEEP_ACOS_PROOF) = range(1, 14)
 (SSX_DBG_FMATH, SSX_DBG_SPHTRI, SSX_DBG_ARVO, SSX_DBG_SAMPLE_LIGHT, SSX_DBG_COSHEMI, SSX_DBG_TRACE, SSX_DBG_RAND_CHOICE,
@@ -255,6 +255,8 @@
             lib.ssx_sums_info.argtypes = [vp, C.POINTER(C.c_uint64), C.POINTER(C.c_uint64)]
         if hasattr(lib, "ssx_rccl_probe"):
             lib.ssx_rccl_probe.argtypes = [C.c_char_p, C.c_size_t]
+        if hasattr(lib, "ssx_path_invariants_info"):
+            lib.ssx_path_invariants_info.argtypes = [vp, C.POINTER(C.c_int), C.POINTER(C.c_uint64)]
         if hasattr(lib, "ssx_units_info"):
             lib.ssx_units_info.argtypes = [vp, C.POINTER(C.c_uint64)]
         if not override or hasattr(lib, "ssx_jit_status"):
diff --git a/simple_spectral_amd/csrc/ssx_api.hip b/simple_spectral_amd/csrc/ssx_api.hip
--- a/simple_spectral_amd/csrc/ssx_api.hip
+++ b/simple_spectral_amd/csrc/ssx_api.hip
@@ -73,6 +73,7 @@
 	const ssx_jit::Kernels* jit_kernels[ssx_jit::kVariants] = {};
 	uint32_t libm = SSX_LIBM_BUILD;
 	uint32_t variant = SSX_LIBM_BUILD;
+	bool uniform_emission = false;
 	bool jit_pending = false, jit_requested = false;
 	ssx_jit::VidTable jit_vid;
 	DeviceBuffer d_blob_jit; uint32_t blob_jit_words = 0, path_blob_jit_words = 0;
@@ -92,6 +93,7 @@
 	uint32_t max_wave_slots = 0;
 	uint32_t queue_words = SSX_QUEUE_WORDS_WIDE;
 	DeviceBuffer d_samples;
+	DeviceBuffer d_inv;
 	DeviceBuffer d_logs;
 	DeviceBuffer d_out;
 	DeviceBuffer d_peer;
@@ -199,6 +201,13 @@
 
 constexpr size_t kSampleBufferBudget = (size_t)16 << 30;
 size_t bytes_per_sample(const ssx_ctx* ctx) { return ctx->spectral_bins ? SSX_BYTES_PER_SAMPLE_FLUX : SSX_BYTES_PER_SAMPLE; }
+uint32_t variant_of(const ssx_ctx* ctx, uint32_t libm) {
+	if (ctx->spectral_bins && libm == SSX_LIBM_BUILD && !ctx->rgb_mode) return ssx_jit::kVariantFlux;
+	if (libm == SSX_LIBM_BUILD && !ctx->uniform_emission && ctx->topology != 2u) return ssx_jit::kVariantPlain;
+	return libm;
+}
+bool path_invariants_on(const ssx_ctx* ctx, uint32_t variant) { return variant == SSX_LIBM_BUILD && ctx->uniform_emission && ctx->topology != 2u; }
+size_t inv_bytes_per_sample(const ssx_ctx* ctx) { return (ctx->fuse_resolve && path_invariants_on(ctx, ctx->variant)) ? SSX_BYTES_PER_SAMPLE_INV : 0u; }
 constexpr size_t kAuxWordsPer64Records = 5;
 size_t bytes_per_64_records(const ssx_ctx* ctx) { return 64u * bytes_per_sample(ctx) + kAuxWordsPer64Records * sizeof(uint32_t); }
 size_t sample_bytes(const ssx_ctx* ctx, size_t records) { return records / 64u * bytes_per_64_records(ctx); }
@@ -226,10 +235,10 @@
 	a.fuse_resolve = ctx->fuse_resolve ? 1u : 0u;
 	a.pre_hits = ctx->pre_hits ? 1u : 0u;
 	a.my_tiles = a.n_tiles > p->tile_first ? (a.n_tiles - p->tile_first + p->tile_stride - 1u) / p->tile_stride : 0u;
-	size_t per_spp = (size_t)(a.my_tiles ? a.my_tiles : 1u) * 64u * bytes_per_sample(ctx);
+	size_t per_spp = (size_t)(a.my_tiles ? a.my_tiles : 1u) * 64u * (bytes_per_sample(ctx) + inv_bytes_per_sample(ctx));
 	size_t budget = kSampleBufferBudget, free_b = 0, total_b = 0;
 	if (ask_device && hipMemGetInfo(&free_b, &total_b) == hipSuccess) {
-		const size_t avail = (size_t)((double)(free_b + sample_slots(ctx) * bytes_per_sample(ctx)) * 0.8);
+		const size_t avail = (size_t)((double)(free_b + sample_slots(ctx) * bytes_per_sample(ctx) + ctx->d_inv.bytes) * 0.8);
 		if (avail < budget) budget = avail;
 	}
 	size_t cap = budget / per_spp;
@@ -241,13 +250,15 @@
 
 void cap_to_allocation(const ssx_ctx* ctx, LaunchPlan& pl) {
 	const size_t per_spp = (size_t)(pl.args.my_tiles ? pl.args.my_tiles : 1u) * 64u;
-	const size_t fit = sample_slots(ctx) / per_spp;
+	size_t fit = sample_slots(ctx) / per_spp;
+	if (inv_bytes_per_sample(ctx)) fit = std::min(fit, ctx->d_inv.bytes / SSX_BYTES_PER_SAMPLE_INV / per_spp);
 	if (fit >= 1 && fit < pl.max_spp_per_launch) pl.max_spp_per_launch = (uint32_t)fit;
 }
 
 int ensure_samples(ssx_ctx* ctx, const LaunchPlan& pl, uint32_t n_k) {
 	const size_t need = (size_t)pl.args.my_tiles * 64u * n_k;
-	const hipError_t e = ctx->d_samples.reserve(sample_bytes(ctx, need));
+	hipError_t e = ctx->d_samples.reserve(sample_bytes(ctx, need));
+	if (e == hipSuccess) e = ctx->d_inv.reserve(need * inv_bytes_per_sample(ctx));
 	if (e == hipErrorOutOfMemory) { (void)hipGetLastError(); return fail(ctx, SSX_ERR_DEVICE, fmt("out of device memory for %zu samples in flight; lower spp_per_launch", need)); }
 	SSX_HIP(ctx, e);
 	return SSX_OK;
@@ -268,11 +279,12 @@
 	return SSX_OK;
 }
 
-void bind_arrays(SsxKernelArgs& a, uint8_t* base, uint64_t cap, uint8_t* logs, uint64_t log_cap, bool with_flux) {
+void bind_arrays(SsxKernelArgs& a, uint8_t* base, uint64_t cap, uint8_t* logs, uint64_t log_cap, bool with_flux, float4* inv = nullptr) {
 	a.ray = reinterpret_cast<float4*>(base);                      base += cap * 16u;
 	a.st = reinterpret_cast<uint4*>(base);                        base += cap * 16u;
 	a.hit = reinterpret_cast<float4*>(base);                      base += cap * 16u;
 	a.flux = with_flux ? reinterpret_cast<float4*>(base) : nullptr;
+	a.inv = inv;
 	a.logs = logs; a.log_cap = (uint32_t)log_cap;
 }
 
@@ -329,7 +341,9 @@
 	b.units = a.my_tiles * a.n_groups;
 	b.n_rec = a.n_records;
 	b.rc = ensure_logs(ctx, a.unit_cohorts);
-	if (b.rc == SSX_OK) bind_arrays(a, ctx->d_samples.as<uint8_t>(), a.n_records, ctx->d_logs.as<uint8_t>(), log_records(ctx), ctx->spectral_bins != 0u);
+	if (b.rc == SSX_OK) bind_arrays(a, ctx->d_samples.as<uint8_t>(), a.n_records, ctx->d_logs.as<uint8_t>(), log_records(ctx), ctx->spectral_bins != 0u,
+	                            inv_bytes_per_sample(ctx) ? ctx->d_inv.as<float4>() : nullptr);
+	if (b.rc == SSX_OK && a.inv && (size_t)a.n_records * SSX_BYTES_PER_SAMPLE_INV > ctx->d_inv.bytes) b.rc = fail(ctx, SSX_ERR_STATE, "internal: launch larger than the invariants array");
 	a.accum = ctx->d_accum.as<double>();
 	uint32_t* const aux = reinterpret_cast<uint32_t*>(ctx->d_samples.as<uint8_t>() + sample_slots(ctx) * bytes_per_sample(ctx));
 	a.unit_state = aux;
@@ -353,7 +367,9 @@
 	{ { SSX_PK(ssx_render_kernel_glibc), SSX_PK(ssx_render_kernel_nq_glibc) }, { SSX_PK(ssx_render_kernel_cornell_glibc), SSX_PK(ssx_render_kernel_cornell_nq_glibc) },
 	  { SSX_PK(ssx_render_kernel_plane_glibc), SSX_PK(ssx_render_kernel_plane_nq_glibc) } },
 	{ { SSX_PK(ssx_render_kernel_flux), SSX_PK(ssx_render_kernel_nq_flux) }, { SSX_PK(ssx_render_kernel_cornell_flux), SSX_PK(ssx_render_kernel_cornell_nq_flux) },
-	  { SSX_PK(ssx_render_kernel_plane_flux), SSX_PK(ssx_render_kernel_plane_nq_flux) } } };
+	  { SSX_PK(ssx_render_kernel_plane_flux), SSX_PK(ssx_render_kernel_plane_nq_flux) } },
+	{ { SSX_PK(ssx_render_kernel_plain), SSX_PK(ssx_render_kernel_nq_plain) }, { SSX_PK(ssx_render_kernel_cornell_plain), SSX_PK(ssx_render_kernel_cornell_nq_plain) },
+	  { SSX_PK(ssx_render_kernel_plane), SSX_PK(ssx_render_kernel_plane_nq) } } };
 #undef SSX_PK
 static const char* const kJitKernelNames[2] = { "ssx_render_kernel_jit", "ssx_render_kernel_jit_nq" };
 const PathKernel& path_kernel_of(const ssx_ctx* ctx, bool narrow) { return kPathKernels[ctx->variant][ctx->topology < 3u ? ctx->topology : 0u][narrow]; }
@@ -483,7 +499,7 @@
 }
 
 int ready_to_launch(ssx_ctx* ctx, const ssx_render_params* p, bool need_out) {
-	const uint32_t variant = (ctx->spectral_bins && p->libm == SSX_LIBM_BUILD && !ctx->rgb_mode) ? ssx_jit::kVariantFlux : p->libm;
+	const uint32_t variant = variant_of(ctx, p->libm);
 	const int rc = ensure_libm_kernels(ctx, variant);
 	if (rc) return rc;
 	ctx->libm = p->libm;
@@ -854,17 +870,20 @@
 	int rc = pack_blob(s, tex, ctx->d_jh_data.ptr, blob, pack_err, -1, &info);
 	if (rc) return fail(ctx, rc, pack_err);
 	const int jit_mode = env_on("SSX_JIT_PASS1") ? SSX_JIT_AT_UPLOAD : ctx->jit_mode;
+	ctx->uniform_emission = reinterpret_cast<const SsxBlobHeader*>(blob.data())->uniform_emission != 0u;
+	const uint32_t v0 = ctx->uniform_emission ? (uint32_t)SSX_LIBM_BUILD : ssx_jit::kVariantPlain;
+	if (ctx->variant == SSX_LIBM_BUILD || ctx->variant == ssx_jit::kVariantPlain) ctx->variant = v0;
 	if (info.candidate && jit_mode != SSX_JIT_OFF) {
 		std::string err;
 		const ssx_jit::Kernels* k = nullptr;
-		ssx_jit::State st = ssx_jit::lookup(ctx->device, info.vid, &k, &err);
+		ssx_jit::State st = ssx_jit::lookup(ctx->device, info.vid, &k, &err, v0);
 		if (st != ssx_jit::State::Ready && st != ssx_jit::State::Failed && jit_mode == SSX_JIT_AT_UPLOAD) {
-			k = ssx_jit::get(ctx->device, info.vid, &err);
+			k = ssx_jit::get(ctx->device, info.vid, &err, v0);
 			st = k ? ssx_jit::State::Ready : ssx_jit::State::Failed;
 		}
 		if (st == ssx_jit::State::Failed) { ctx->jit_state = SSX_JIT_STATE_FAILED; ctx->jit_message = err; }
 		else if ((rc = pack_blob(s, tex, ctx->d_jh_data.ptr, blob_jit, pack_err, 3))) return fail(ctx, rc, pack_err);
-		else if (st == ssx_jit::State::Ready) { blob.swap(blob_jit); blob_jit.clear(); ctx->jit_kernels[SSX_LIBM_BUILD] = k; ctx->jit_vid = info.vid; ctx->jit_state = SSX_JIT_STATE_SPECIALISED; }
+		else if (st == ssx_jit::State::Ready) { blob.swap(blob_jit); blob_jit.clear(); ctx->jit_kernels[v0] = k; ctx->jit_vid = info.vid; ctx->jit_state = SSX_JIT_STATE_SPECIALISED; }
 		else { ctx->jit_pending = true; ctx->jit_vid = info.vid; ctx->jit_state = SSX_JIT_STATE_GENERIC_MEANWHILE; ctx->jit_requested = (st == ssx_jit::State::Pending); }
 	}
 	if (ctx->jit_pending) {
@@ -879,6 +898,7 @@
 	{
 		SsxBlobHeader* bh = reinterpret_cast<SsxBlobHeader*>(blob.data());
 		ctx->topology = bh->topology;
+		if (ctx->topology == 2u && ctx->variant == ssx_jit::kVariantPlain) ctx->variant = SSX_LIBM_BUILD;
 		ctx->path_blob_words = (bh->topology || bh->perm_hbm) ? bh->words_without_perm : ctx->blob_words;
 		if (bh->perm_hbm) {
 			const uint64_t at = (uint64_t)(uintptr_t)(ctx->d_blob.as<uint32_t>() + bh->off_perm);
@@ -921,14 +941,15 @@
 	(void)hipStreamIsCapturing(stream, &capture);
 	const bool capturing = capture == hipStreamCaptureStatusActive;
 	if (ctx->device_pending && capturing) return fail(ctx, SSX_ERR_STATE, "a render of this context may still be queued: ssx_render_device_wait before capturing another into a graph");
-	if (capturing && ctx->variant != p->libm) return fail(ctx, SSX_ERR_STATE, "ssx_render_params.libm differs from the context's last render: run it once outside the stream capture first");
+	if (capturing && ctx->variant != variant_of(ctx, p->libm)) return fail(ctx, SSX_ERR_STATE, "ssx_render_params.libm differs from the context's last render: run it once outside the stream capture first");
 	if (ctx->device_pending) SSX_HIP(ctx, hipStreamWaitEvent(stream, ctx->ev_device_done, 0));
 	{
 		LaunchPlan probe = make_plan(ctx, p, !capturing);
 		if (capturing) cap_to_allocation(ctx, probe);
 		const uint32_t probe_batch = device_batch(p, probe);
 		const size_t need = (size_t)probe.args.my_tiles * 64u * probe_batch;
-		const bool grow = ctx->d_accum.bytes < accum_bytes(p->width, p->height) || ctx->d_samples.bytes < sample_bytes(ctx, need);
+		const bool grow = ctx->d_accum.bytes < accum_bytes(p->width, p->height) || ctx->d_samples.bytes < sample_bytes(ctx, need) ||
+		                  (path_invariants_on(ctx, variant_of(ctx, p->libm)) && ctx->d_inv.bytes < need * SSX_BYTES_PER_SAMPLE_INV);
 		if (grow && capturing) return fail(ctx, SSX_ERR_STATE, "the context's buffers have to grow for this render: run it once outside the stream capture first");
 		if (grow && (rc = wait_device_pending(ctx))) return rc;
 	}
@@ -1187,6 +1208,15 @@
 	return SSX_OK;
 }
 
+int ssx_path_invariants_info(ssx_ctx* ctx, int* on, uint64_t* invariant_bytes) {
+	if (!ctx) return SSX_ERR_ARG;
+	if (!ctx->have_scene) return fail(ctx, SSX_ERR_STATE, "no scene uploaded");
+	const bool is_on = path_invariants_on(ctx, ctx->variant);
+	if (on) *on = is_on ? 1 : 0;
+	if (invariant_bytes) *invariant_bytes = is_on ? (uint64_t)ctx->d_inv.bytes : 0u;
+	return SSX_OK;
+}
+
 int ssx_sums_info(ssx_ctx* ctx, uint64_t* units_parked, uint64_t* units_chained) {
 	if (!ctx) return SSX_ERR_ARG;
 	uint32_t c[4] = { 0u, 0u, 0u, 0u };
diff --git a/simple_spectral_amd/csrc/ssx_blob.h b/simple_spectral_amd/csrc/ssx_blob.h
--- a/simple_spectral_amd/csrc/ssx_blob.h
+++ b/simple_spectral_amd/csrc/ssx_blob.h
@@ -51,7 +51,7 @@
 	uint32_t perm_hbm, perm_ptr_lo, perm_ptr_hi;
 	float cam_dir[3];
 	uint32_t black_ends_path;
-	uint32_t pad4_[1];
+	uint32_t uniform_emission;
 	float lambda_steps[4];
 	double n_lights_recip;
 	double q_const[4];
@@ -79,6 +79,7 @@
 #define SSX_UNIT_TURN 2u
 #define SSX_BYTES_PER_SAMPLE (16u + 16u + 16u)
 #define SSX_BYTES_PER_SAMPLE_FLUX (SSX_BYTES_PER_SAMPLE + 16u)
+#define SSX_BYTES_PER_SAMPLE_INV 16u
 #define SSX_LOG_BYTES_PER_RECORD ((16u + 8u + 4u) * SSX_MAX_FRAMES + (16u + 16u + 1u) * SSX_MAX_LEVELS)
 
 struct SsxKernelArgs {
@@ -117,4 +118,5 @@
 	double inv_width, inv_height;
 	uint32_t fuse_gen;
 	float4* flux;
+	float4* inv;
 };
diff --git a/simple_spectral_amd/csrc/ssx_jit.h b/simple_spectral_amd/csrc/ssx_jit.h
--- a/simple_spectral_amd/csrc/ssx_jit.h
+++ b/simple_spectral_amd/csrc/ssx_jit.h
@@ -159,15 +159,16 @@
 };
 inline Shared& shared() { static Shared* s = new Shared; return *s; }
 
-constexpr uint32_t kVariantFlux = 2, kVariants = 3;
+constexpr uint32_t kVariantFlux = 2, kVariantPlain = 3, kVariants = 4;
 inline std::string pattern_key(const VidTable& vids, uint32_t libm = 0) {
 	std::string key;
 	if (libm == 1u) key = "libm=glibc-2.35|";
 	if (libm == kVariantFlux) key = "flux|";
+	if (libm == kVariantPlain) key = "plain|";
 	for (const auto& r : vids) key.append(reinterpret_cast<const char*>(r.data()), 4);
 	return key;
 }
-inline const char* libm_flag(uint32_t libm) { return libm == kVariantFlux ? "-DSSX_JIT_FLUX=1" : libm ? "-DSSX_JIT_GLIBC=1" : nullptr; }
+inline const char* libm_flag(uint32_t libm) { return libm == kVariantPlain ? "-DSSX_JIT_INV=0" : libm == kVariantFlux ? "-DSSX_JIT_FLUX=1" : libm ? "-DSSX_JIT_GLIBC=1" : nullptr; }
 
 inline const char* const* compile_flags(size_t* n) {
 	static const char* const flags[] = { "--offload-arch=gfx950", "-O3", "-std=c++17", "-ffp-contract=off", "-fno-slp-vectorize", "-DSSX_JIT_BUILD",
diff --git a/simple_spectral_amd/csrc/ssx_kernels.hip b/simple_spectral_amd/csrc/ssx_kernels.hip
--- a/simple_spectral_amd/csrc/ssx_kernels.hip
+++ b/simple_spectral_amd/csrc/ssx_kernels.hip
@@ -826,7 +826,13 @@
 	st_y = (bx * s0[1] + by * s1[1]) + bz * s2[1];
 }
 
-template <bool NARROW, bool BLACK, bool GLIBC = false>
+__device__ __forceinline__ const __attribute__((address_space(4))) SsxKernelArgs& cold_args() {
+	auto p = __builtin_amdgcn_kernarg_segment_ptr();
+	asm volatile("" : "+s"(p));
+	return *(const __attribute__((address_space(4))) SsxKernelArgs*)p;
+}
+
+template <bool NARROW, bool BLACK, bool GLIBC = false, bool INV = false>
 __device__ __forceinline__ bool path_step(const Lds& L, const ShadowQ& q, const SsxKernelArgs& a, const LogRef& lg, Path& p, bool& pushed, uint32_t& level_word) {
 	const SsxBlobHeader& h = L.hdr();
 	level_word = SSX_NO_SLOT << 13;
@@ -868,7 +874,11 @@
 		float n_dot_l = dot3(sdir, N);
 		if (n_dot_l > 0.0f) {
 			SSX_STAT(9);
-			Hero emitted = spectrum_hero(L, L.quad(light).emission, p.lambda_0, h.lambda_step);
+			Hero emitted;
+			if (INV) {
+				const float4 e = cold_args().inv[p.rec_index];
+				emitted.v[0] = e.x; emitted.v[1] = e.y; emitted.v[2] = e.z; emitted.v[3] = e.w;
+			} else emitted = spectrum_hero(L, L.quad(light).emission, p.lambda_0, h.lambda_step);
 			float c[4];
 			const double spdf_recip = ssx_exact::div64_rcp_any(spdf);
 #pragma unroll
@@ -955,11 +965,6 @@
 	}
 }
 
-__device__ __forceinline__ const __attribute__((address_space(4))) SsxKernelArgs& cold_args() {
-	auto p = __builtin_amdgcn_kernarg_segment_ptr();
-	asm volatile("" : "+s"(p));
-	return *(const __attribute__((address_space(4))) SsxKernelArgs*)p;
-}
 __device__ __forceinline__ double ld_agent(const double* p) { return __hip_atomic_load(p, __ATOMIC_RELAXED, __HIP_MEMORY_SCOPE_AGENT); }
 __device__ __forceinline__ void st_agent(double* p, double v) { __hip_atomic_store(p, v, __ATOMIC_RELAXED, __HIP_MEMORY_SCOPE_AGENT); }
 __device__ __forceinline__ void add_sample(bool rgb_mode, double acc[4], float x, float y, float z, float alpha) {
@@ -1093,6 +1098,10 @@
 		float4 ray = make_float4(0.0f, 0.0f, 1.0f, 0.0f); uint4 st = make_uint4(0u, 0u, 0u, 0u);
 		if (inside) generate_sample(h, a, i, j, kk, ray, st);
 		const uint64_t r = sk * 64u + lane;
+		if (a.inv && inside) {
+			const Hero em = spectrum_hero(L, L.quad(L.light(0u)).emission, ray.w, h.lambda_step);
+			a.inv[r] = make_float4(em.v[0], em.v[1], em.v[2], em.v[3]);
+		}
 		if (!a.pre_hits) {
 			if (inside) { a.ray[r] = ray; a.st[r] = st; }
 			continue;
@@ -1289,7 +1298,7 @@
 	}
 }
 
-template <int TOPO, bool NARROW, bool CALIB = false, bool GLIBC = false, bool FLUX = false>
+template <int TOPO, bool NARROW, bool CALIB = false, bool GLIBC = false, bool FLUX = false, bool INV = false>
 __device__ __forceinline__ void render_body(const SsxKernelArgs& a) {
 	constexpr bool FUSE_GEN = TOPO == 2;
 	uint32_t* const lds_words = stage_lds<GLIBC>(a);
@@ -1420,7 +1429,7 @@
 				LogRef lg;
 				lg.cnt = log_cnt; lg.wave_base = wave_slot * 2u * a.unit_cohorts; lg.tagw = p_tag;
 				uint32_t level_word;
-				if (!path_step<NARROW, TOPO != 1, GLIBC>(L, sq, a, lg, p, pushed, level_word)) end_path(level_word, 1u);
+				if (!path_step<NARROW, TOPO != 1, GLIBC, INV>(L, sq, a, lg, p, pushed, level_word)) end_path(level_word, 1u);
 			}
 			sq.count += (uint32_t)__popcll(__ballot(pushed));
 		}
@@ -1464,31 +1473,38 @@
 #ifndef SSX_JIT_FLUX
 #define SSX_JIT_FLUX 0
 #endif
-#define SSX_PATH_KERNEL(name, topo, narrow, glibc, flux) \
-	extern "C" __global__ void __launch_bounds__(256) __attribute__((amdgpu_waves_per_eu(SSX_WAVES_PER_EU))) name(SsxKernelArgs a) { render_body<topo, narrow, false, glibc, flux>(a); }
+#ifndef SSX_JIT_INV
+#define SSX_JIT_INV 1
+#endif
+#define SSX_PATH_KERNEL(name, topo, narrow, glibc, flux, inv) \
+	extern "C" __global__ void __launch_bounds__(256) __attribute__((amdgpu_waves_per_eu(SSX_WAVES_PER_EU))) name(SsxKernelArgs a) { render_body<topo, narrow, false, glibc, flux, inv>(a); }
 #ifdef SSX_JIT_BUILD
-SSX_PATH_KERNEL(ssx_render_kernel_jit, 3, false, SSX_JIT_GLIBC, SSX_JIT_FLUX)
-SSX_PATH_KERNEL(ssx_render_kernel_jit_nq, 3, true, SSX_JIT_GLIBC, SSX_JIT_FLUX)
+SSX_PATH_KERNEL(ssx_render_kernel_jit, 3, false, SSX_JIT_GLIBC, SSX_JIT_FLUX, SSX_JIT_INV && !SSX_JIT_GLIBC && !SSX_JIT_FLUX)
+SSX_PATH_KERNEL(ssx_render_kernel_jit_nq, 3, true, SSX_JIT_GLIBC, SSX_JIT_FLUX, SSX_JIT_INV && !SSX_JIT_GLIBC && !SSX_JIT_FLUX)
 #else
-SSX_PATH_KERNEL(ssx_render_kernel, 0, false, false, false)
-SSX_PATH_KERNEL(ssx_render_kernel_cornell, 1, false, false, false)
+SSX_PATH_KERNEL(ssx_render_kernel, 0, false, false, false, true)
+SSX_PATH_KERNEL(ssx_render_kernel_cornell, 1, false, false, false, true)
 #ifndef SSX_PROBE_BUILD
-SSX_PATH_KERNEL(ssx_render_kernel_plane, 2, false, false, false)
-SSX_PATH_KERNEL(ssx_render_kernel_nq, 0, true, false, false)
-SSX_PATH_KERNEL(ssx_render_kernel_cornell_nq, 1, true, false, false)
-SSX_PATH_KERNEL(ssx_render_kernel_plane_nq, 2, true, false, false)
-SSX_PATH_KERNEL(ssx_render_kernel_glibc, 0, false, true, false)
-SSX_PATH_KERNEL(ssx_render_kernel_cornell_glibc, 1, false, true, false)
-SSX_PATH_KERNEL(ssx_render_kernel_plane_glibc, 2, false, true, false)
-SSX_PATH_KERNEL(ssx_render_kernel_nq_glibc, 0, true, true, false)
-SSX_PATH_KERNEL(ssx_render_kernel_cornell_nq_glibc, 1, true, true, false)
-SSX_PATH_KERNEL(ssx_render_kernel_plane_nq_glibc, 2, true, true, false)
-SSX_PATH_KERNEL(ssx_render_kernel_flux, 0, false, false, true)
-SSX_PATH_KERNEL(ssx_render_kernel_cornell_flux, 1, false, false, true)
-SSX_PATH_KERNEL(ssx_render_kernel_plane_flux, 2, false, false, true)
-SSX_PATH_KERNEL(ssx_render_kernel_nq_flux, 0, true, false, true)
-SSX_PATH_KERNEL(ssx_render_kernel_cornell_nq_flux, 1, true, false, true)
-SSX_PATH_KERNEL(ssx_render_kernel_plane_nq_flux, 2, true, false, true)
+SSX_PATH_KERNEL(ssx_render_kernel_plane, 2, false, false, false, false)
+SSX_PATH_KERNEL(ssx_render_kernel_nq, 0, true, false, false, true)
+SSX_PATH_KERNEL(ssx_render_kernel_cornell_nq, 1, true, false, false, true)
+SSX_PATH_KERNEL(ssx_render_kernel_plane_nq, 2, true, false, false, false)
+SSX_PATH_KERNEL(ssx_render_kernel_plain, 0, false, false, false, false)
+SSX_PATH_KERNEL(ssx_render_kernel_cornell_plain, 1, false, false, false, false)
+SSX_PATH_KERNEL(ssx_render_kernel_nq_plain, 0, true, false, false, false)
+SSX_PATH_KERNEL(ssx_render_kernel_cornell_nq_plain, 1, true, false, false, false)
+SSX_PATH_KERNEL(ssx_render_kernel_glibc, 0, false, true, false, false)
+SSX_PATH_KERNEL(ssx_render_kernel_cornell_glibc, 1, false, true, false, false)
+SSX_PATH_KERNEL(ssx_render_kernel_plane_glibc, 2, false, true, false, false)
+SSX_PATH_KERNEL(ssx_render_kernel_nq_glibc, 0, true, true, false, false)
+SSX_PATH_KERNEL(ssx_render_kernel_cornell_nq_glibc, 1, true, true, false, false)
+SSX_PATH_KERNEL(ssx_render_kernel_plane_nq_glibc, 2, true, true, false, false)
+SSX_PATH_KERNEL(ssx_render_kernel_flux, 0, false, false, true, false)
+SSX_PATH_KERNEL(ssx_render_kernel_cornell_flux, 1, false, false, true, false)
+SSX_PATH_KERNEL(ssx_render_kernel_plane_flux, 2, false, false, true, false)
+SSX_PATH_KERNEL(ssx_render_kernel_nq_flux, 0, true, false, true, false)
+SSX_PATH_KERNEL(ssx_render_kernel_cornell_nq_flux, 1, true, false, true, false)
+SSX_PATH_KERNEL(ssx_render_kernel_plane_nq_flux, 2, true, false, true, false)
 #endif
 extern "C" __global__ void __launch_bounds__(256) __attribute__((amdgpu_waves_per_eu(3))) ssx_calibrate_kernel(SsxKernelArgs a) { render_body<0, true, true>(a); }
 #endif
diff --git a/simple_spectral_amd/csrc/ssx_pack.h b/simple_spectral_amd/csrc/ssx_pack.h
--- a/simple_spectral_amd/csrc/ssx_pack.h
+++ b/simple_spectral_amd/csrc/ssx_pack.h
@@ -71,6 +71,12 @@
 		for (uint32_t k = 0; k < es.n; ++k) if (!(std::fabs(s->samples[es.offset + k]) <= 0x1p60f)) h.black_ends_path = 0u;
 	}
 	if (const char* e = debug_env("SSX_BLACK_SHORTCUT")) { if (e[0] == '0') h.black_ends_path = 0u; }
+	h.uniform_emission = s->n_lights ? 1u : 0u;
+	for (uint32_t i = 1; i < s->n_lights; ++i) {
+		const ssx_spectrum &e0 = s->spectra[s->materials[s->quads[s->lights[0]].material].emission_spectrum], &ei = s->spectra[s->materials[s->quads[s->lights[i]].material].emission_spectrum];
+		if (!(e0.offset == ei.offset && e0.n == ei.n && memcmp(&e0.low, &ei.low, 4) == 0 && memcmp(&e0.delta_recip, &ei.delta_recip, 4) == 0)) h.uniform_emission = 0u;
+	}
+	if (const char* e = debug_env("SSX_PATH_INVARIANTS")) { if (e[0] == '0') h.uniform_emission = 0u; }
 	for (int i = 0; i < 4; ++i) { volatile float fi = (float)i; h.lambda_steps[i] = fi * s->lambda_step; }
 	const ssx_spectrum &r = s->spectra[s->spec_basis_r], &g = s->spectra[s->spec_basis_g], &b = s->spectra[s->spec_basis_b];
 	const ssx_spectrum &ox = s->spectra[s->spec_xbar], &oy = s->spectra[s->spec_ybar], &oz = s->spectra[s->spec_zbar];
diff --git a/simple_spectral_amd/renderer.py b/simple_spectral_amd/renderer.py
--- a/simple_spectral_amd/renderer.py
+++ b/simple_spectral_amd/renderer.py
@@ -391,7 +391,11 @@
         if hasattr(self._lib, "ssx_calibration_info"):
             self._check(self._lib.ssx_calibration_info(self._ctx, None, C.byref(left), C.byref(pre)))
         fused = (not pre.value) and variant == "plane topology" and not (os.environ.get("SSX_DEBUG_ENV") == "1" and os.environ.get("SSX_FUSE_GEN", "")[:1] == "0")
+        inv = C.c_int()
+        if hasattr(self._lib, "ssx_path_invariants_info"):
+            self._check(self._lib.ssx_path_invariants_info(self._ctx, C.byref(inv), None))
         return {"frames_per_sample": round(f.value, 3), "fold": "path kernel", "pass1": variant,
+                "path_invariants": "generate kernel (per-sample record)" if inv.value else "path kernel (every level)",
                 "rays_left_per_sample": round(left.value, 3), "camera_rays": "pre-traced (generate kernel)" if pre.value else "path loop",
                 "samples_made_in": "path kernel (refill)" if fused else "generate kernel",
                 "kernel": name.decode() if name else None}
@@ -400,7 +404,13 @@
         a, b = C.c_uint64(), C.c_uint64()
         if hasattr(self._lib, "ssx_scratch_info"):
             self._check(self._lib.ssx_scratch_info(self._ctx, C.byref(a), C.byref(b)))
-        return {"sample_bytes": a.value, "log_bytes": b.value}
+        out = {"sample_bytes": a.value, "log_bytes": b.value}
+        on, n = C.c_int(), C.c_uint64()
+        if hasattr(self._lib, "ssx_path_invariants_info"):
+            self._check(self._lib.ssx_path_invariants_info(self._ctx, C.byref(on), C.byref(n)))
+        if on.value:
+            out["invariant_bytes"] = n.value
+        return out
 
     def sums_info(self):
         a, b = C.c_uint64(), C.c_uint64()
```
